# OSOceanAcoustics/echopype

Measured on AMD Instinct MI355X. Metric: range-samples/sec through compute_Sv->compute_MVBS, higher is better.
Workload: dtype f64; 1 GPU; cfg5: EK60 CW 4x2000000x4096 in ping_time tiles, compute_Sv -> compute_MVBS(20s x 1m), Sv+MVBS out; tiles=8 x 250000 pings over 1 rank(s), route=compute_Sv -> compute_MVBS('1m','20s') per tile, collective=none at 1 rank, tile_streams=2

## Files before the change

### echopype_amd/_lib.py

```python
import ctypes
import os

import torch

_HERE = os.path.dirname(os.path.abspath(__file__))
LIB_PATH = os.environ.get("ECHOPYPE_AMD_LIB") or os.path.join(_HERE, "lib", "libechopype_amd.so")

EPA_OK, EPA_EINVAL, EPA_EHIP, EPA_ENOMEM, EPA_EUNSUPPORTED = range(5)
F32, F64 = 0, 1
I8 = 2
CAL_SV, CAL_TS = 0, 1
SONAR_EK60, SONAR_EK80 = 0, 1
PM_SCALAR, PM_CHANNEL, PM_CHANNEL_PING, PM_PULSE_TABLE = range(4)
NCOEF = 8
CF_RA, CF_RB, CF_R0, CF_SHIFT, CF_ALPHA2, CF_A0, CF_G, CF_D = range(8)
NCCOEF = 8
CC_RA, CC_RB, CC_SHIFT, CC_ALPHA2, CC_A, CC_PSCALE = range(6)
FLAG_GUARD_POS, FLAG_MASK_RANGE = 1, 2
BIN_SKIPNA, BIN_CLOSED_RIGHT, BIN_RANGE_AS_STORED = 1, 2, 4
POOL_NANMEAN, POOL_NANMEDIAN = 0, 1
CMP_GT, CMP_LT, CMP_LE, CMP_GE, CMP_EQ = range(5)
CCP = ("sample_interval", "tau_nominal", "transmit_power", "sound_speed", "absorption", "gain", "freq_center", "psi",
       "sa_correction", "z_er", "z_et", "angle_offset_alongship", "angle_offset_athwartship", "beamwidth_alongship",
       "beamwidth_athwartship")
EK80_NFFT = 2048
APPLY_MASKS_WS_DOUBLES = 131072
SEAFLOOR_STATE_WORDS = 16
SHOAL_STATE_WORDS = 8
SHOAL_QUEUE_BOXES = 4096


class EpaError(RuntimeError):
    """A C-ABI call returned a non-zero status."""


def _load():
    if not os.path.exists(LIB_PATH):
        raise ImportError(
            f"{LIB_PATH} not found: build it with `python echopype_amd/build.py` "
            "(hipcc --offload-arch=gfx950).  echopype_amd has no CPU fallback."
        )
    return ctypes.CDLL(LIB_PATH)


lib = _load()

_vp, _i, _u, _d, _sz = ctypes.c_void_p, ctypes.c_int, ctypes.c_uint, ctypes.c_double, ctypes.c_size_t
_i64 = ctypes.c_int64

SIGNATURES = {
    "epa_version": [],
    "epa_source_digest": [],
    "epa_last_error": [],
    "epa_launch_trace": [_i],
    "epa_last_range_stats_filled": [],
    "epa_launch_seen": [],
    "epa_device_count": [ctypes.POINTER(_i)],
    "epa_set_device": [_i],
    "epa_device_name": [_i, ctypes.c_char_p, _sz],
    "epa_malloc": [ctypes.POINTER(_vp), _sz],
    "epa_free": [_vp],
    "epa_memset": [_vp, _i, _sz, _vp],
    "epa_memcpy_h2d": [_vp, _vp, _sz, _vp],
    "epa_memcpy_d2h": [_vp, _vp, _sz, _vp],
    "epa_stream_synchronize": [_vp],
    "epa_timer_create": [ctypes.POINTER(_vp)],
    "epa_timer_destroy": [_vp],
    "epa_timer_start": [_vp, _vp],
    "epa_timer_stop": [_vp, _vp],
    "epa_timer_elapsed_ms": [_vp, ctypes.POINTER(ctypes.c_float)],
    "epa_power_coef_ek": [_i, _i, _vp, _vp, _vp, _vp, _i, _vp, _i, _vp, _i, _vp, _i, _vp, _i, _vp, _i, _vp,
                          _vp, _i, _vp, _i, _i, _vp, _vp],
    "epa_pulse_table_lookup": [_vp, _vp, _vp, _i, _i, _i, _vp, _vp],
    "epa_sv_power": [_vp, _vp, _i, _i, _i, _i, _u, _vp, _vp, _i, _vp],
    "epa_sv_power_stats": [_vp, _vp, _i, _i, _i, _i, _u, _vp, _vp, _i, _vp, _vp, _vp],
    "epa_range_power": [_vp, _vp, _i, _i, _i, _u, _vp, _i, _vp],
    "epa_range_complex": [_vp, _i, _vp, _i, _i, _i, _i, _vp, _i, _vp],
    "epa_sv_complex_cw_stats": [_vp, _vp, _i, _vp, _i, _i, _i, _i, _i, _vp, _vp, _vp, _i, _vp, _vp, _vp],
    "epa_time_bin_offsets": [_vp, _i, _i64, _i64, _i, _u, _vp, _vp],
    "epa_sv_mvbs_fused": [_vp, _vp, _i, _i, _i, _i, _u, _vp, _vp, _i, _d, _i, _u, _d, _vp, _vp, _vp,
                          _vp, _vp, _vp, _vp, _i, _vp],
    "epa_sv_mvbs_fused_i16": [_vp, _vp, _vp, _i, _i, _i, _i, _vp, _i, _d, _i, _d, _vp, _vp, _vp, _vp, _vp, _i, _vp],
    "epa_sv_mvbs_fused_depth": [_vp, _vp, _vp, _vp, _i, _i, _i, _i, _vp, _i, _d, _i, _d, _vp, _vp, _vp, _vp, _vp, _vp, _i,
                                _vp],
    "epa_mvbs": [_vp, _vp, _vp, _i, _i, _i, _vp, _vp, _i, _d, _i, _u, _d, _vp, _vp, _vp, _i, _vp],
    "epa_selftest_lin_from_db": [_vp, _vp, _sz, _vp],
    "epa_selftest_log10": [_vp, _vp, _sz, _vp],
    "epa_selftest_log10_inline": [_vp, _vp, _sz, _vp],
    "epa_selftest_correlate": [_vp, _i, _vp, _vp, _i, _vp, _vp, _vp],
    "epa_mvbs_finalize": [_vp, _vp, _sz, _d, _vp, _i, _vp],
    "epa_edge_pack": [_vp, _vp, _vp, _vp, _i, _i, _i, _i, _i, _i, _vp, _vp],
    "epa_edge_prepare_max": [_vp, _i, _vp],
    "epa_edge_gather": [_vp, _i, _vp, _vp, _i, _i, _i, _vp, _vp, _vp, _i, _vp],
    "epa_edge_finalize_mvbs": [_vp, _i, _vp, _vp, _vp, _vp, _vp, _i, _i, _i, _d, _i, _vp],
    "epa_affine_rows": [_vp, _vp, _vp, _i, _i, _i, _vp, _i, _vp],
    "epa_depth_rows": [_vp, _vp, _vp, _vp, _vp, _i, _i, _i, _vp, _i, _vp, _vp, _vp],
    "epa_nanminmax": [_vp, _sz, _i, _vp, _vp, _vp],
    "epa_mvbs_index": [_vp, _vp, _i, _i, _i, _i, _i, _vp, _vp, _i, _vp],
    "epa_noise_estimate": [_vp, _vp, _vp, _vp, _i, _i, _i, _i, _i, _i, _d, _vp, _vp, _vp, _i, _vp],
    "epa_noise_finalize": [_vp, _vp, _i, _i, _d, _vp, _vp],
    "epa_noise_apply": [_vp, _vp, _vp, _vp, _vp, _i, _i, _i, _i, _i, _d, _vp, _vp, _vp, _i, _vp],
    "epa_noise_apply_rows": [_vp, _vp, _vp, _vp, _vp, _i, _i, _i, _i, _i, _d, _vp, _vp, _vp, _i, _vp],
    "epa_complex_coef_ek80": [_i, _i, _vp, _vp, _vp, _i, _vp, _i, _i, _i, _vp, _vp],
    "epa_sv_complex": [_vp, _vp, _i, _vp, _vp, _i, _vp, _i, _i, _i, _i, _i, _vp, _vp, _vp, _i, _vp],
    "epa_sv_complex_indexed": [_vp, _vp, _i, _vp, _vp, _vp, _i, _i, _vp, _i, _i, _i, _i, _i, _vp, _vp, _vp, _i, _vp],
    "epa_sv_complex_fft": [_vp, _vp, _i, _vp, _vp, _i, _vp, _i, _i, _i, _i, _i, _vp, _vp, _vp, _i, _i, _vp, _vp, _vp],
    "epa_sv_complex_fft_indexed": [_vp, _vp, _i, _vp, _vp, _vp, _i, _i, _vp, _i, _i, _i, _i, _i, _vp, _vp, _vp, _i, _i,
                                   _vp, _vp, _vp],
    "epa_range_bin_smooth": [_vp, _vp, _i, _i, _i, _i, _d, _d, _i, _vp, _i, _vp],
    "epa_impulse_mask": [_vp, _i, _i, _i, _i, _d, _vp, _i, _vp],
    "epa_pool_sv": [_vp, _i, _i, _i, _i, _i, _i, _i, _d, _vp, _vp, _vp, _vp, _i, _vp],
    "epa_attenuated_mask": [_vp, _vp, _i, _i, _i, _d, _d, _i, _d, _vp, _i, _vp],
    "epa_apply_mask": [_vp, _vp, _sz, _sz, _d, _vp, _sz, _vp, _i, _vp],
    "epa_apply_masks": [_vp, _vp, _vp, _i, _sz, _d, _vp, _sz, _vp, _vp, _vp, _i, _vp],
    "epa_mask_and": [_vp, _vp, _sz, _sz, _vp, _vp],
    "epa_range_step_mean": [_vp, _i, _i, _i, _i, _vp, _vp, _vp],
    "epa_first_not_le": [_vp, _sz, _d, _i, _vp, _vp],
    "epa_range_rows_check": [_vp, _i, _i, _i, _i, _vp, _vp, _vp],
    "epa_sv_noise_fused": [_vp, _vp, _vp, _i, _i, _i, _i, _u, _i, _i, _i, _d, _vp, _vp, _vp, _vp, _vp, _vp, _vp, _i, _vp],
    "epa_denoise_mvbs": [_vp, _vp, _vp, _vp, _vp, _i, _i, _i, _i, _d, _vp, _vp, _i, _d, _i, _u, _d, _vp, _vp, _vp,
                         _vp, _vp, _i, _vp],
    "epa_sv_denoise_mvbs": [_vp, _vp, _vp, _vp, _i, _i, _i, _i, _u, _i, _i, _d, _vp, _vp, _i, _d, _i, _u, _d, _vp, _vp, _vp,
                            _vp, _vp, _vp, _vp, _i, _vp],
    "epa_geodesic_steps": [_vp, _vp, _i, _vp, _vp],
    "epa_nasc": [_vp, _vp, _i, _i, _i, _vp, _i, _d, _i, _u, _vp, _vp, _vp, _vp, _i, _vp],
    "epa_splitbeam_power": [_vp, _vp, _i, _vp, _vp, _i, _i, _i, _vp, _vp, _i, _vp],
    "epa_splitbeam_complex": [_vp, _vp, _i, _vp, _vp, _vp, _vp, _vp, _vp, _i, _i, _i, _i, _i, _i, _vp, _vp, _i, _vp],
    "epa_splitbeam_complex_fft": [_vp, _vp, _i, _vp, _vp, _vp, _vp, _vp, _vp, _i, _i, _i, _i, _i, _i, _vp, _vp, _i, _i,
                                  _vp, _vp],
    "epa_pool_sv_value": [_vp, _vp, _vp, _i, _i, _i, _d, _i, _d, _d, _d, _i, _d, _vp, _vp, _vp, _i, _vp],
    "epa_seafloor_depth_uniform": [_vp, _i, _i64, _i64, _vp, _vp],
    "epa_seafloor_basic": [_vp, _i, _i64, _i64, _i64, _d, _d, _vp, _d, _vp, _vp],
    "epa_seafloor_angle_mask": [_vp, _vp, _i, _i64, _i64, _i64, _i64, _i, _i, _d, _d, _vp, _vp, _vp, _vp],
    "epa_seafloor_median": [_vp, _i, _i64, _i64, _i64, _i64, _vp, _vp, _vp, _vp],
    "epa_seafloor_components": [_vp, _i, _i64, _i64, _i64, _i64, _d, _vp, _vp, _vp, _vp],
    "epa_seafloor_bottom": [_vp, _vp, _i64, _i64, _i64, _vp, _d, _vp, _i, _vp],
    "epa_shoal_threshold_fill": [_vp, _i, _i64, _i64, _d, _i64, _i64, _vp, _vp],
    "epa_shoal_label": [_vp, _i64, _i64, _i, _vp, _vp, _vp, _i64, _vp, _vp],
    "epa_shoal_weill_filter": [_vp, _i64, _i64, _vp, _vp, _i64, _d, _d, _vp, _vp, _vp],
    "epa_shoal_echoview_link": [_vp, _i64, _i64, _vp, _vp, _vp, _i64, _vp, _i64, _vp, _i64, _d, _d, _d, _d, _d, _d, _vp,
                                _vp, _vp, _vp],
    "epa_transient_fielding": [_vp, _i, _i, _i, _i, _vp, _i, _i, _d, _d, _d, _vp, _vp, _vp, _vp],
    "epa_transient_matecho": [_vp, _i, _i, _i, _i, _vp, _vp, _vp, _vp, _i, _i, _d, _d, _i, _d, _vp, _vp, _vp, _vp],
    "epa_freq_diff_mask": [_vp, _i, _sz, _i, _i, _i, _d, _vp, _i, _vp],
    "epa_regrid_mask": [_vp, _vp, _i, _i, _i, _vp, _i, _vp, _i, _d, _i, _u, _i, _vp, _vp, _vp],
    "epa_echo_metrics": [_vp, _vp, _i, _i64, _i64, _vp, _vp, _vp, _vp, _vp, _vp, _i, _i, _vp],
}

for _name, _args in SIGNATURES.items():
    _fn = getattr(lib, _name)
    _fn.argtypes = _args
    _fn.restype = ctypes.c_char_p if _name in ("epa_last_error", "epa_launch_trace", "epa_launch_seen", "epa_source_digest") else _i


def _check_source_digest():
    if os.environ.get("ECHOPYPE_AMD_LIB"):
        return
    import importlib.util

    spec = importlib.util.spec_from_file_location("_epa_build", os.path.join(_HERE, "build.py"))
    if spec is None or not os.path.isdir(os.path.join(_HERE, "csrc")):
        return
    b = importlib.util.module_from_spec(spec)
    spec.loader.exec_module(b)
    want, got = b.source_digest(), lib.epa_source_digest().decode()
    if want != got:
        raise ImportError(f"{LIB_PATH} was built from other sources (digest {got}, the tree has {want}): "
                          "rebuild it with `python echopype_amd/build.py` (`--force` recompiles every translation unit)")


_check_source_digest()


class launch_trace:

    def __enter__(self):
        lib.epa_launch_trace(1)
        self.kernels = []
        return self

    def __exit__(self, *exc):
        self.kernels = [k for k in lib.epa_launch_trace(2).decode().split(";") if k]
        lib.epa_launch_trace(0)
        return False


def launched_kernels():
    return [k for k in lib.epa_launch_seen().decode().split(";") if k]


def last_error() -> str:
    msg = lib.epa_last_error()
    return msg.decode("utf-8", "replace") if msg else ""


def check(status: int, what: str = "") -> None:
    if status == EPA_OK:
        return
    msg = f"{what}: {last_error()}" if what else last_error()
    if status == EPA_EINVAL:
        raise ValueError(msg)
    if status == EPA_ENOMEM:
        raise MemoryError(msg)
    raise EpaError(f"[status {status}] {msg}")


def call(name: str, *args) -> None:
    check(getattr(lib, name)(*args), name)
```

### echopype_amd/csrc/block_reduce.hip

```cpp
#include <hip/amd_detail/amd_hip_unsafe_atomics.h>

#include <cstdlib>

#include "fast_math.h"
#include "sample_math.h"

namespace {

enum { SRC_RAW = 0, SRC_SV = 1, SRC_SV_DENOISE = 2, SRC_RAW_DENOISE = 3 };
enum { OP_MVBS = 0, OP_NOISE = 1 };
enum { BIN_PHYS = 0, BIN_INDEX = 1 };

struct ReduceArgs {
  double* range_max_out;
  double* range_stats_out;
  int range_stats_filled;
  const int16_t* raw_i16;
  const int32_t* n_valid;
  const double* dscale;
  const double* doffset;
  void* depth_out;
  const float* raw;
  const void* sv;
  const void* range;
// ... 152 lines not shown
        constexpr bool kDenoise = SRC == SRC_SV_DENOISE || SRC == SRC_RAW_DENOISE;
        if (kFromRaw) {
          epa::RawVec<VEC> in;
          in.load(a.raw + off);
          const epa::RowK<T> rk(a.coef[row]);
          col.update(rk.d, s0, nspread);
          if (OP == OP_NOISE || kDenoise) {
            const double k = rk.ra * rk.rb;
            col_tl.update(-rk.r0 / k, s0, (T)1);
            const T log10k = epa::fast_log10((T)k, mt.log_tab);
#pragma unroll
            for (int j = 0; j < VEC; ++j) logR[j] = col_tl.nL[j] + log10k;
          }
          T rg[VEC];
#pragma unroll
          for (int j = 0; j < VEC; ++j) {
            x[j] = rk.range(s0 + j);
            sv[j] = epa::cal_power_sample<T>(in.v[j], s0 + j, rk, nspread, col.nL[j], guard, x[j]);
            xok[j] = !(mask_range && !(in.v[j] == in.v[j]));
            rg[j] = xok[j] ? (T)x[j] : epa::M<T>::nan();
            if (a.range_max_out && xok[j]) xmax = fmax(xmax, (double)rg[j]);
          }
          if (sv_out && !kDenoise) epa::store_vec<T, VEC>(sv_out + off, sv);
          if (range_out) epa::store_vec<T, VEC>(range_out + off, rg);
        } else {
          epa::load_vec<T, VEC>(svp + off, sv);
          if (rgp) {
            T rg[VEC];
            epa::load_vec<T, VEC>(rgp + off, rg);
#pragma unroll
            for (int j = 0; j < VEC; ++j) {
              x[j] = (double)rg[j];
              xok[j] = true;
            }
          } else if (a.coef) {
            const epa::CoefRow cr = a.coef[row];
#pragma unroll
            for (int j = 0; j < VEC; ++j) {
              x[j] = epa::row_range(cr, s0 + j);
              if (range_as_stored) x[j] = (double)(T)x[j];
              xok[j] = true;
            }
          } else {
#pragma unroll
            for (int j = 0; j < VEC; ++j) {
              x[j] = 0.0;
              xok[j] = true;
            }
          }
        }
        if (kDenoise) {
          {
            const T nb = (T)a.noise[(size_t)c * a.n_pblocks + (p + a.noise_phase) / a.noise_ping_num];
            const T na2 = (T)a.alpha2[row];
            const T snr = (T)a.snr;
            T sn[VEC];
#pragma unroll
            for (int j = 0; j < VEC; ++j) {
              const T xr = xok[j] ? (T)x[j] : epa::M<T>::nan();
              const T lg = kFromRaw ? logR[j] : epa::fast_log10(xr >= (T)1 ? xr : (T)1, mt.log_tab);
              const T tl = (T)20 * (xr >= (T)1 ? lg : (T)0) + na2 * xr;
              sn[j] = nb + tl;
              const T lin = epa::lin_from_db(sv[j], mt.exp2_tab) - epa::lin_from_db(sn[j], mt.exp2_tab);
              T corr = lin > (T)0 ? (T)10 * epa::fast_log10(lin, mt.log_tab) : epa::M<T>::nan();
              const bool keep = corr - sn[j] > snr;
              sv[j] = keep ? corr : epa::M<T>::nan();
              vlin[j] = keep ? lin : epa::M<T>::nan();
              if (a.mm_keys) {
                mm[0] = fmin(mm[0], (double)sn[j]);
                mm[1] = fmax(mm[1], (double)sn[j]);
                mm[2] = fmin(mm[2], (double)sv[j]);
                mm[3] = fmax(mm[3], (double)sv[j]);
              }
            }
            if (sv_noise_out) epa::store_vec<T, VEC>(sv_noise_out + off, sn);
            if (sv_out) epa::store_vec<T, VEC>(sv_out + off, sv);
          }
        }
        T a2 = (T)0;
        if (OP == OP_NOISE) a2 = (T)a.alpha2[row];
#pragma unroll
        for (int j = 0; j < VEC; ++j) {
          T v;
          if (OP == OP_MVBS) {
            v = kDenoise ? vlin[j] : epa::lin_from_db(sv[j], mt.exp2_tab);
          } else {
            const T xr = (T)x[j];
            const T lg = kFromRaw ? logR[j] : epa::fast_log10(xr >= (T)1 ? xr : (T)1, mt.log_tab);
            const T tl = (T)20 * (xr >= (T)1 ? lg : (T)0) + a2 * xr;
            v = epa::lin_from_db(sv[j] - tl, mt.exp2_tab);
          }
          if (phys) {
            const bool same = xok[j] && (closed_right ? (x[j] > blo[j] && x[j] <= bhi[j])
                                                      : (x[j] >= blo[j] && x[j] < bhi[j]));
            if (!same) {
              const int rb = xok[j] ? epa::range_bin_index(x[j], a.range_bin, a.inv_range_bin,
                                                            n_rbins, closed_right)
                                    : -1;
              if (rb != acc_rb[j]) {
                if (acc_rb[j] >= 0 && acc_cnt[j] > 0u && !extra) {
                  atomic_add(asum + acc_rb[j], acc_sum[j]);
                  atomicAdd(acnt + acc_rb[j], acc_cnt[j]);
                }
                acc_rb[j] = rb;
                acc_sum[j] = (T)0;
                acc_cnt[j] = 0u;
              }
              if (rb >= 0) {
                blo[j] = (double)rb * a.range_bin;
                bhi[j] = (double)(rb + 1) * a.range_bin;
              } else {
                blo[j] = 1.0;
                bhi[j] = 0.0;
              }
            }
          }
          if (acc_rb[j] >= 0 && (!skipna || v == v)) {
            acc_sum[j] += v;
            acc_cnt[j] += 1u;
          }
        }
      }
      if (!extra) {
#pragma unroll
        for (int j = 0; j < VEC; ++j) {
          if (acc_rb[j] >= 0 && acc_cnt[j] > 0u) {
            atomic_add(asum + acc_rb[j], acc_sum[j]);
            atomicAdd(acnt + acc_rb[j], acc_cnt[j]);
          }
        }
      }
    }
  }
  }
  if (a.range_max_out) {
#pragma unroll
    for (int o = 32; o > 0; o >>= 1) xmax = fmax(xmax, __shfl_down(xmax, o, 64));
    if ((threadIdx.x & 63) == 0 && xmax > -__builtin_inf()) {
      const unsigned long long b = (unsigned long long)__double_as_longlong(xmax);
      atomicMax(reinterpret_cast<unsigned long long*>(a.range_max_out),
                (b >> 63) ? ~b : (b | 0x8000000000000000ull));
    }
  }
  if (a.mm_keys) {
#pragma unroll
    for (int o = 32; o > 0; o >>= 1) {
      mm[0] = fmin(mm[0], __shfl_down(mm[0], o, 64));
      mm[1] = fmax(mm[1], __shfl_down(mm[1], o, 64));
      mm[2] = fmin(mm[2], __shfl_down(mm[2], o, 64));
      mm[3] = fmax(mm[3], __shfl_down(mm[3], o, 64));
    }
    if ((threadIdx.x & 63) == 0) {
      auto key = [](double v) {
        const unsigned long long b = (unsigned long long)__double_as_longlong(v);
        return (b >> 63) ? ~b : (b | 0x8000000000000000ull);
      };
      if (mm[0] <= mm[1]) {
        atomicMin(a.mm_keys + 0, key(mm[0]));
        atomicMax(a.mm_keys + 1, key(mm[1]));
      }
      if (mm[2] <= mm[3]) {
        atomicMin(a.mm_keys + 2, key(mm[2]));
        atomicMax(a.mm_keys + 3, key(mm[3]));
      }
    }
  }
  if (extra) return;

  if (!use_lds) return;
  __syncthreads();
  if (a.nparts > 1) {
    for (int i = threadIdx.x; i < n_rbins; i += epa::kBlock) {
      const uint32_t n = lcnt[i];
      if (n > 0u) {
        atomic_add(gsum + i, lsum[i]);
        atomicAdd(gcnt + i, n);
      }
    }
    return;
  }
  if (OP == OP_MVBS) {
    T* out = reinterpret_cast<T*>(a.out) + cell0;
    for (int i = threadIdx.x; i < n_rbins; i += epa::kBlock) {
      const uint32_t n = lcnt[i];
      const T s = lsum[i];
      out[i] = n > 0u ? (T)10 * epa::M<T>::log10(s / (T)n) : (T)a.fill_value;
      if (gsum) gsum[i] = s;
      if (gcnt) gcnt[i] = n;
    }
  } else {
    if (a.edge_sum_out && (tb == 0 || tb == a.n_tbins - 1)) {
      const size_t e0 = ((size_t)(tb == 0 ? 0 : 1) * a.C + c) * n_rbins;
      for (int i = threadIdx.x; i < n_rbins; i += epa::kBlock) {
        a.edge_sum_out[e0 + i] = (double)lsum[i];
        a.edge_cnt_out[e0 + i] = lcnt[i];
      }
    }
    T best = (T)__builtin_inf();
    bool any = false;
    for (int i = threadIdx.x; i < n_rbins; i += epa::kBlock) {
      const uint32_t n = lcnt[i];
      if (n > 0u) {
        const T db = (T)10 * epa::M<T>::log10(lsum[i] / (T)n);
        if (db == db) {
          best = fmin(best, db);
          any = true;
        }
      }
    }
    __syncthreads();
    T m = block_nanmin<T>(best, any, lsum);
    if (threadIdx.x == 0) {
      double r = (double)m;
      if (a.noise_max == a.noise_max) r = (r < a.noise_max) ? r : a.noise_max;
      reinterpret_cast<double*>(a.out)[(size_t)c * a.n_tbins + tb] = r;
    }
  }
}

template <typename T>
__global__ __launch_bounds__(epa::kBlock) void mvbs_finalize_kernel(const T* __restrict__ sum,
                                                                    const uint32_t* __restrict__ cnt,
                                                                    size_t n, T fill,
                                                                    T* __restrict__ out) {
  for (size_t i = (size_t)blockIdx.x * blockDim.x + threadIdx.x; i < n;
       i += (size_t)gridDim.x * blockDim.x) {
    const uint32_t k = cnt[i];
    out[i] = k > 0u ? (T)10 * epa::M<T>::log10(sum[i] / (T)k) : fill;
  }
}

template <typename T>
__global__ __launch_bounds__(epa::kBlock) void noise_rowmin_kernel(const T* __restrict__ sum,
                                                                   const uint32_t* __restrict__ cnt,
                                                                   int n_rbins, double noise_max,
                                                                   double* __restrict__ out) {
  __shared__ T scratch[8];
  const size_t base = (size_t)blockIdx.x * n_rbins;
  T best = (T)__builtin_inf();
  bool any = false;
  for (int i = threadIdx.x; i < n_rbins; i += epa::kBlock) {
    const uint32_t n = cnt[base + i];
    if (n > 0u) {
      const T db = (T)10 * epa::M<T>::log10(sum[base + i] / (T)n);
      if (db == db) {
        best = fmin(best, db);
        any = true;
      }
    }
  }
  T m = block_nanmin<T>(best, any, scratch);
  if (threadIdx.x == 0) {
    double r = (double)m;
    if (noise_max == noise_max) r = (r < noise_max) ? r : noise_max;
    out[blockIdx.x] = r;
  }
}

template <typename T>
__global__ __launch_bounds__(epa::kBlock) void block_nanmin_kernel(const T* __restrict__ x, int C,
                                                                   int P, int S, int ping_num,
                                                                   int rsn, int Pb, int Sb,
                                                                   T* __restrict__ out) {
  const long long cells = (long long)C * Pb * Sb;
  const int lane = threadIdx.x & 63;
  const long long wave0 = ((long long)blockIdx.x * blockDim.x + threadIdx.x) >> 6;
  const long long nwaves = ((long long)gridDim.x * blockDim.x) >> 6;
  for (long long cell = wave0; cell < cells; cell += nwaves) {
    const int sb = (int)(cell % Sb);
    const int pbk = (int)((cell / Sb) % Pb);
    const int c = (int)(cell / ((long long)Sb * Pb));
    const int p0 = pbk * ping_num, p1 = min(P, p0 + ping_num);
    const int s0 = sb * rsn, s1 = min(S, s0 + rsn);
    const int w = s1 - s0;
    const int n = (p1 - p0) * w;
    T m = (T)__builtin_inf();
    int any = 0;
    for (int e = lane; e < n; e += 64) {
      const int p = p0 + e / w, s = s0 + e % w;
      const T v = x[((size_t)c * P + p) * S + s];
      if (v == v) {
        m = fmin(m, v);
        any = 1;
      }
    }
#pragma unroll
    for (int o = 32; o > 0; o >>= 1) {
      m = fmin(m, __shfl_down(m, o, 64));
      any |= __shfl_down(any, o, 64);
    }
    if (lane == 0) out[cell] = any ? m : epa::M<T>::nan();
  }
}

}

int epa_fused_fast_path(const void* raw, int raw_is_i16, const int32_t* n_valid, const double* coef,
                        int C, int P, int S, double nspread,
                        unsigned cal_flags, const int32_t* bin_start, int n_tbins, double range_bin,
                        int n_rbins, unsigned bin_flags, double fill_value, void* sv_out,
                        void* mvbs_out, void* sum_out, uint32_t* cnt_out, int dtype,
                        size_t lds_bytes, unsigned cnt_off, unsigned long long* rmax_key,
                        unsigned long long* rstat, const double* dscale, const double* doffset, void* depth_out,
                        hipStream_t st);

int epa_mvbs_rows_fast_path(const void* sv, const double* coef, int C, int P, int S, const int32_t* bin_start,
                            int n_tbins, double range_bin, int n_rbins, int as_stored, double fill_value,
                            void* mvbs_out, void* sum_out, uint32_t* cnt_out, int dtype, size_t lds_bytes,
                            unsigned cnt_off, hipStream_t st);
int epa_chain_fast_pass1(const float* raw, const double* coef, const double* alpha2, int C, int P, int S,
                         double nspread, int ping_num, int rsn, int ping_phase, double noise_max, void* sv_out,
                         double* noise_out, double* edge_sum_out, uint32_t* edge_cnt_out,
                         unsigned long long* rmax_key, unsigned long long* rstat, int dtype, hipStream_t st);
int epa_chain_fast_pass2(const float* raw, const double* coef, const double* alpha2, const double* noise, int C,
                         int P, int S, double nspread, int ping_num, int ping_phase, double snr,
                         const int32_t* bin_start, int n_tbins, double range_bin, int n_rbins, double fill_value,
                         void* noise_out, void* corr_out, void* mvbs_out, void* sum_out, uint32_t* cnt_out, int dtype,
                         size_t lds_acc_bytes, unsigned cnt_off, unsigned long long* mm_keys, hipStream_t st);

namespace {

struct Plan {
  int nparts, use_lds, vec;
  size_t lds_bytes;
  unsigned cnt_off, tab_off;
};

template <typename T>
Plan make_plan(int C, int P, int S, int n_tbins, int n_rbins, bool aligned16) {
  Plan pl;
  pl.vec = (S % 4 == 0 && aligned16) ? 4 : 1;
  if (const char* e = getenv("EPA_REDUCE_VEC")) {
    const int v = atoi(e);
    if ((v == 1) || (v == 2 && S % 2 == 0 && aligned16) || (v == 4 && S % 4 == 0 && aligned16)) pl.vec = v;
  }
  const size_t sum_bytes = ((size_t)n_rbins * sizeof(T) + 15) & ~(size_t)15;
  const size_t need = sum_bytes + (size_t)n_rbins * sizeof(uint32_t);
  pl.use_lds = need <= 128 * 1024;
  const size_t acc_bytes = pl.use_lds ? (need < 64 ? 64 : need) : 64;
  pl.cnt_off = (unsigned)sum_bytes;
  pl.tab_off = (unsigned)((acc_bytes + 15) & ~(size_t)15);
  pl.lds_bytes = pl.tab_off + epa::kMathTabBytes;
  const long long groups = (long long)C * n_tbins;
  pl.nparts = 1;
  if (groups < 1024) {
    const long long avg = n_tbins > 0 ? (P + n_tbins - 1) / n_tbins : P;
    long long want = (2048 + groups - 1) / groups;
    long long maxp = (avg + 7) / 8;
    if (maxp < 1) maxp = 1;
    pl.nparts = (int)(want < maxp ? want : maxp);
    if (pl.nparts < 1) pl.nparts = 1;
  }
  return pl;
}

template <typename T, int SRC, int OP>
int launch_reduce(ReduceArgs& a, const Plan& pl, hipStream_t st) {
  const long long tslots = (long long)a.n_tbins + ((SRC != SRC_SV && a.bin_start) ? 1 : 0);
  const dim3 grid((unsigned)(tslots * a.nparts), (unsigned)a.C);
  const dim3 block(epa::kBlock);
  a.use_lds = pl.use_lds;
  a.cnt_off = pl.cnt_off;
  a.tab_off = pl.tab_off;
#define EPA_RL(V)                                                                                 \
  do {                                                                                            \
    auto kern = block_reduce_kernel<T, SRC, OP, V>;                                               \
    if (pl.lds_bytes > 64 * 1024) {                                                               \
      EPA_CHECK_HIP(hipFuncSetAttribute(reinterpret_cast<const void*>(kern),                      \
                                        hipFuncAttributeMaxDynamicSharedMemorySize,               \
                                        (int)pl.lds_bytes));                                      \
    }                                                                                             \
    hipLaunchKernelGGL(kern, grid, block, pl.lds_bytes, st, a);                                   \
  } while (0)
  if (pl.vec == 4) EPA_RL(4); else if (pl.vec == 2) EPA_RL(2); else EPA_RL(1);
#undef EPA_RL
  return epa::check_launch("block_reduce_kernel");
}

inline bool al16(const void* p) { return p == nullptr || (reinterpret_cast<uintptr_t>(p) & 15u) == 0; }

template <typename T>
int zero_partials(void* sum_out, uint32_t* cnt_out, size_t cells, hipStream_t st) {
  EPA_CHECK_HIP(hipMemsetAsync(sum_out, 0, cells * sizeof(T), st));
  EPA_CHECK_HIP(hipMemsetAsync(cnt_out, 0, cells * sizeof(uint32_t), st));
  return EPA_OK;
}

template <typename T, int SRC>
int run_mvbs(ReduceArgs& a, hipStream_t st) {
  Plan pl = make_plan<T>(a.C, a.P, a.S, a.n_tbins, a.n_rbins,
                               al16(a.raw) && al16(a.sv) && al16(a.range) && al16(a.sv_out) &&
                                   al16(a.range_out));
  if (SRC == SRC_RAW && (a.range_max_out || a.raw_i16)) pl.nparts = 1;
  a.nparts = pl.nparts;
  const size_t cells = (size_t)a.C * a.n_tbins * a.n_rbins;
  const bool two_stage = pl.nparts > 1 || !pl.use_lds;
  if (SRC == SRC_RAW && !two_stage && pl.vec == 4 && !a.ping_perm && !a.range_out &&
      a.cal_flags == (EPA_FLAG_GUARD_POS | EPA_FLAG_MASK_RANGE) && a.bin_flags == EPA_BIN_SKIPNA &&
      (a.raw_i16 || !getenv("EPA_NO_FAST_PATH")) && (a.range_stats_filled = a.range_stats_out != nullptr, true))
    return epa_fused_fast_path(a.raw_i16 ? (const void*)a.raw_i16 : (const void*)a.raw, a.raw_i16 != nullptr,
                               a.n_valid, reinterpret_cast<const double*>(a.coef), a.C, a.P, a.S,
                               a.nspread, a.cal_flags, a.bin_start, a.n_tbins, a.range_bin,
                               a.n_rbins, a.bin_flags, a.fill_value, a.sv_out, a.out, a.sum_out,
                               a.cnt_out, sizeof(T) == 8 ? EPA_F64 : EPA_F32, pl.tab_off,
                               pl.cnt_off, reinterpret_cast<unsigned long long*>(a.range_max_out),
                               reinterpret_cast<unsigned long long*>(a.range_stats_out), a.dscale, a.doffset,
                               a.depth_out, st);
  if (a.dscale) {
    epa::set_error("epa_sv_mvbs_fused_depth: binning on depth is served by the default configuration only (sorted "
                   "pings, S %% 4 == 0, aligned arrays, range grid within LDS)");
    return EPA_EUNSUPPORTED;
  }
  if (SRC == SRC_RAW_DENOISE && !two_stage && pl.vec == 4 && !a.ping_perm && !a.range_out &&
      a.cal_flags == (EPA_FLAG_GUARD_POS | EPA_FLAG_MASK_RANGE) && a.bin_flags == EPA_BIN_SKIPNA &&
      !getenv("EPA_NO_FAST_PATH"))
    return epa_chain_fast_pass2(a.raw, reinterpret_cast<const double*>(a.coef), a.alpha2, a.noise, a.C, a.P, a.S,
                                a.nspread, a.noise_ping_num, a.noise_phase, a.snr, a.bin_start, a.n_tbins, a.range_bin,
                                a.n_rbins, a.fill_value, a.sv_noise_out, a.sv_out, a.out, a.sum_out, a.cnt_out,
                                sizeof(T) == 8 ? EPA_F64 : EPA_F32, pl.tab_off, pl.cnt_off, a.mm_keys, st);
  if (SRC == SRC_SV && !a.range && a.coef && !two_stage && pl.vec == 4 && !a.ping_perm &&
      (a.bin_flags & ~EPA_BIN_RANGE_AS_STORED) == EPA_BIN_SKIPNA && !getenv("EPA_NO_FAST_PATH"))
    return epa_mvbs_rows_fast_path(a.sv, reinterpret_cast<const double*>(a.coef), a.C, a.P, a.S, a.bin_start, a.n_tbins,
                                   a.range_bin, a.n_rbins, (a.bin_flags & EPA_BIN_RANGE_AS_STORED) ? 1 : 0,
                                   a.fill_value, a.out, a.sum_out, a.cnt_out, sizeof(T) == 8 ? EPA_F64 : EPA_F32,
                                   pl.tab_off, pl.cnt_off, st);
  if (a.raw_i16) {
    epa::set_error("epa_sv_mvbs_fused_i16: int16 ingest is served by the default configuration only "
                   "(guard + masked range, skipna, left-closed bins, sorted pings, S %% 4 == 0, no "
                   "echo_range output, range grid within LDS)");
    return EPA_EUNSUPPORTED;
  }
  if (two_stage) {
    EPA_CHECK_ARG(a.sum_out && a.cnt_out,
                  "binned reduction: this shape (C*n_tbins=%lld, n_rbins=%d) needs the sum_out/"
                  "cnt_out workspaces", (long long)a.C * a.n_tbins, a.n_rbins);
    int rc = zero_partials<T>(a.sum_out, a.cnt_out, cells, st);
    if (rc) return rc;
  }
  int rc = launch_reduce<T, SRC, OP_MVBS>(a, pl, st);
  if (rc) return rc;
  if (two_stage) {
    const int grid = (int)((cells + epa::kBlock - 1) / epa::kBlock < 4096
                               ? (cells + epa::kBlock - 1) / epa::kBlock : 4096);
    hipLaunchKernelGGL(mvbs_finalize_kernel<T>, dim3(grid), dim3(epa::kBlock), 0, st,
                       (const T*)a.sum_out, (const uint32_t*)a.cnt_out, cells, (T)a.fill_value,
                       (T*)a.out);
    return epa::check_launch("mvbs_finalize_kernel");
  }
  return EPA_OK;
}

int check_bins(const char* fn, const int32_t* bin_start, int n_tbins, double range_bin, int n_rbins) {
  EPA_CHECK_ARG(bin_start != nullptr, "%s: bin_start is NULL", fn);
  EPA_CHECK_ARG(n_tbins > 0 && n_rbins > 0, "%s: n_tbins=%d n_rbins=%d must be positive", fn,
                n_tbins, n_rbins);
  EPA_CHECK_ARG(range_bin > 0, "%s: range_bin must be positive", fn);
  return EPA_OK;
}

}

namespace {
__global__ void decode_minmax_kernel(double* p) {
  const int i = threadIdx.x;
  const unsigned long long k = reinterpret_cast<unsigned long long*>(p)[i];
  const bool none = (i & 1) ? k == 0ull : k == ~0ull;
  const unsigned long long b = (k >> 63) ? (k & 0x7fffffffffffffffull) : ~k;
  p[i] = none ? __builtin_nan("") : __longlong_as_double(b);
}
__global__ void init_minmax_kernel(unsigned long long* p) { p[threadIdx.x] = (threadIdx.x & 1) ? 0ull : ~0ull; }

__global__ void init_range_out_kernel(double* rmax, double* st) {
  if (rmax) *reinterpret_cast<unsigned long long*>(rmax) = 0ull;
  if (st) {
    unsigned long long* u = reinterpret_cast<unsigned long long*>(st);
    u[0] = ~0ull;
    u[1] = 0ull;
    u[2] = 0ull;
  }
}
__global__ void decode_range_out_kernel(double* rmax, double* st, int mode, int as_f32) {
  const unsigned long long km = *reinterpret_cast<unsigned long long*>(rmax);
  const unsigned long long bm = (km >> 63) ? (km & 0x7fffffffffffffffull) : ~km;
  const double mx = km == 0ull ? __builtin_nan("") : __longlong_as_double(bm);
  *rmax = mx;
  if (mode == 1) {
    const unsigned long long k = reinterpret_cast<unsigned long long*>(st)[0];
    const unsigned long long n = reinterpret_cast<unsigned long long*>(st)[1];
    const unsigned long long b = (k >> 63) ? (k & 0x7fffffffffffffffull) : ~k;
    double lo = k == ~0ull ? __builtin_nan("") : __longlong_as_double(b), hi = mx;
    if (as_f32) {
      lo = (double)(float)lo;
      hi = (double)(float)hi;
    }
    st[0] = lo;
    st[1] = hi;
    st[2] = (double)n;
  } else if (mode == 2) {
    st[0] = st[1] = __builtin_nan("");
    st[2] = -1.0;
  }
}

int init_range_outputs(double* rmax, double* st, hipStream_t stream) {
  if (!rmax && !st) return EPA_OK;
  hipLaunchKernelGGL(init_range_out_kernel, dim3(1), dim3(1), 0, stream, rmax, st);
  return epa::check_launch("init_range_out_kernel");
}
int decode_range_outputs(double* rmax, double* st, bool filled, int as_f32, hipStream_t stream) {
  hipLaunchKernelGGL(decode_range_out_kernel, dim3(1), dim3(1), 0, stream, rmax, st, st ? (filled ? 1 : 2) : 0, as_f32);
  return epa::check_launch("decode_range_out_kernel");
}
}

static int fused_entry(const float* raw, const int16_t* raw_i16, const int32_t* n_valid,
                       const double* coef, int C, int P, int S, int cal_type, unsigned cal_flags,
                       const int32_t* bin_start, const int32_t* ping_perm, int n_tbins,
                       double range_bin, int n_rbins, unsigned bin_flags, double fill_value,
                       void* sv_out, void* range_out, void* mvbs_out, void* sum_out,
                       uint32_t* cnt_out, double* range_max_out, double* range_stats_out, int dtype,
                       epa_stream_t stream, const double* dscale = nullptr, const double* doffset = nullptr,
                       void* depth_out = nullptr);

extern "C" int epa_sv_mvbs_fused(const float* raw, const double* coef, int C, int P, int S,
                                 int cal_type, unsigned cal_flags, const int32_t* bin_start,
                                 const int32_t* ping_perm, int n_tbins, double range_bin,
                                 int n_rbins, unsigned bin_flags, double fill_value, void* sv_out,
                                 void* range_out, void* mvbs_out, void* sum_out, uint32_t* cnt_out,
                                 double* range_max_out, double* range_stats_out, int dtype,
                                 epa_stream_t stream) {
  EPA_CHECK_ARG(raw != nullptr, "epa_sv_mvbs_fused: NULL array argument");
  EPA_CHECK_ARG(!range_stats_out || range_max_out, "epa_sv_mvbs_fused: range_stats_out needs range_max_out");
  return fused_entry(raw, nullptr, nullptr, coef, C, P, S, cal_type, cal_flags, bin_start, ping_perm,
                     n_tbins, range_bin, n_rbins, bin_flags, fill_value, sv_out, range_out, mvbs_out,
                     sum_out, cnt_out, range_max_out, range_stats_out, dtype, stream);
}

extern "C" int epa_sv_mvbs_fused_i16(const int16_t* raw, const int32_t* n_valid, const double* coef,
                                     int C, int P, int S, int cal_type, const int32_t* bin_start,
                                     int n_tbins, double range_bin, int n_rbins, double fill_value,
                                     void* sv_out, void* mvbs_out, void* sum_out, uint32_t* cnt_out,
                                     double* range_max_out, int dtype, epa_stream_t stream) {
  EPA_CHECK_ARG(raw && n_valid, "epa_sv_mvbs_fused_i16: NULL array argument");
  return fused_entry(nullptr, raw, n_valid, coef, C, P, S, cal_type,
                     EPA_FLAG_GUARD_POS | EPA_FLAG_MASK_RANGE, bin_start, nullptr, n_tbins, range_bin,
                     n_rbins, EPA_BIN_SKIPNA, fill_value, sv_out, nullptr, mvbs_out, sum_out, cnt_out,
                     range_max_out, nullptr, dtype, stream);
}

extern "C" int epa_sv_mvbs_fused_depth(const float* raw, const double* coef, const double* depth_scale,
                                       const double* depth_offset, int C, int P, int S, int cal_type,
                                       const int32_t* bin_start, int n_tbins, double range_bin, int n_rbins,
                                       double fill_value, void* sv_out, void* depth_out, void* mvbs_out, void* sum_out,
                                       uint32_t* cnt_out, double* depth_stats_out, int dtype, epa_stream_t stream) {
  EPA_CHECK_ARG(raw && depth_scale && depth_offset && depth_stats_out, "epa_sv_mvbs_fused_depth: NULL array argument");
  EPA_CHECK_ARG(!depth_out || sv_out, "epa_sv_mvbs_fused_depth: depth_out needs sv_out");
  return fused_entry(raw, nullptr, nullptr, coef, C, P, S, cal_type, EPA_FLAG_GUARD_POS | EPA_FLAG_MASK_RANGE, bin_start,
                     nullptr, n_tbins, range_bin, n_rbins, EPA_BIN_SKIPNA, fill_value, sv_out, nullptr, mvbs_out, sum_out,
                     cnt_out, depth_stats_out + 32, depth_stats_out, dtype, stream, depth_scale, depth_offset, depth_out);
}

static int fused_entry(const float* raw, const int16_t* raw_i16, const int32_t* n_valid,
                       const double* coef, int C, int P, int S, int cal_type, unsigned cal_flags,
                       const int32_t* bin_start, const int32_t* ping_perm, int n_tbins,
                       double range_bin, int n_rbins, unsigned bin_flags, double fill_value,
                       void* sv_out, void* range_out, void* mvbs_out, void* sum_out,
                       uint32_t* cnt_out, double* range_max_out, double* range_stats_out, int dtype,
                       epa_stream_t stream, const double* dscale, const double* doffset, void* depth_out) {
  EPA_CHECK_ARG(coef && mvbs_out, "epa_sv_mvbs_fused: NULL array argument");
  EPA_CHECK_ARG(C > 0 && P > 0 && S > 0, "epa_sv_mvbs_fused: C=%d P=%d S=%d", C, P, S);
  EPA_CHECK_ARG(cal_type == EPA_CAL_SV || cal_type == EPA_CAL_TS, "epa_sv_mvbs_fused: bad cal_type");
  if (int rc = check_bins("epa_sv_mvbs_fused", bin_start, n_tbins, range_bin, n_rbins)) return rc;
  ReduceArgs a{};
  a.raw = raw; a.raw_i16 = raw_i16; a.n_valid = n_valid;
  a.dscale = dscale; a.doffset = doffset; a.depth_out = depth_out;
  a.coef = reinterpret_cast<const epa::CoefRow*>(coef);
  a.C = C; a.P = P; a.S = S;
  a.nspread = cal_type == EPA_CAL_SV ? 20.0 : 40.0;
  a.cal_flags = cal_flags;
  a.bin_start = bin_start; a.ping_perm = ping_perm; a.n_tbins = n_tbins; a.ping_num = 0;
  a.bin_mode = BIN_PHYS; a.range_bin = range_bin; a.inv_range_bin = 1.0 / range_bin;
  a.n_rbins = n_rbins; a.range_sample_num = 1; a.bin_flags = bin_flags;
  a.fill_value = fill_value; a.noise_max = __builtin_nan("");
  a.sv_out = sv_out; a.range_out = range_out; a.out = mvbs_out; a.sum_out = sum_out; a.cnt_out = cnt_out;
  a.range_max_out = range_max_out;
  a.range_stats_out = range_stats_out;
  EPA_CHECK_ARG(dtype == EPA_F64 || dtype == EPA_F32, "epa_sv_mvbs_fused: bad dtype %d", dtype);
  if (int rc0 = init_range_outputs(range_max_out, range_stats_out, (hipStream_t)stream)) return rc0;
  const int rc = dtype == EPA_F64 ? run_mvbs<double, SRC_RAW>(a, (hipStream_t)stream)
                                  : run_mvbs<float, SRC_RAW>(a, (hipStream_t)stream);
  epa::note_range_stats_filled(rc == EPA_OK && range_stats_out && a.range_stats_filled ? 1 : 0);
  if (rc == EPA_OK && range_max_out) {
    return decode_range_outputs(range_max_out, range_stats_out, a.range_stats_filled != 0, dtype == EPA_F32 ? 1 : 0,
                                (hipStream_t)stream);
  }
  return rc;
}

extern "C" int epa_mvbs(const void* sv, const void* range, const double* coef, int C, int P, int S,
                        const int32_t* bin_start, const int32_t* ping_perm, int n_tbins,
                        double range_bin, int n_rbins, unsigned bin_flags, double fill_value,
                        void* mvbs_out, void* sum_out, uint32_t* cnt_out, int dtype,
                        epa_stream_t stream) {
  EPA_CHECK_ARG(sv && mvbs_out, "epa_mvbs: NULL array argument");
  EPA_CHECK_ARG(range || coef, "epa_mvbs: either range or coef must be given");
  EPA_CHECK_ARG(C > 0 && P > 0 && S > 0, "epa_mvbs: C=%d P=%d S=%d", C, P, S);
  if (int rc = check_bins("epa_mvbs", bin_start, n_tbins, range_bin, n_rbins)) return rc;
  ReduceArgs a{};
  a.sv = sv; a.range = range; a.coef = reinterpret_cast<const epa::CoefRow*>(coef);
  a.C = C; a.P = P; a.S = S;
  a.bin_start = bin_start; a.ping_perm = ping_perm; a.n_tbins = n_tbins;
  a.bin_mode = BIN_PHYS; a.range_bin = range_bin; a.inv_range_bin = 1.0 / range_bin;
  a.n_rbins = n_rbins; a.range_sample_num = 1; a.bin_flags = bin_flags;
  a.fill_value = fill_value; a.noise_max = __builtin_nan("");
  a.out = mvbs_out; a.sum_out = sum_out; a.cnt_out = cnt_out;
  if (dtype == EPA_F64) return run_mvbs<double, SRC_SV>(a, (hipStream_t)stream);
  if (dtype == EPA_F32) return run_mvbs<float, SRC_SV>(a, (hipStream_t)stream);
  epa::set_error("epa_mvbs: bad dtype %d", dtype);
  return EPA_EINVAL;
}

extern "C" int epa_mvbs_finalize(const void* sum, const uint32_t* cnt, size_t n, double fill_value,
                                 void* out, int dtype, epa_stream_t stream) {
  EPA_CHECK_ARG(sum && cnt && out, "epa_mvbs_finalize: NULL array argument");
  if (n == 0) return EPA_OK;
  const size_t blocks = (n + epa::kBlock - 1) / epa::kBlock;
  const int grid = (int)(blocks < 4096 ? blocks : 4096);
  if (dtype == EPA_F64)
    hipLaunchKernelGGL(mvbs_finalize_kernel<double>, dim3(grid), dim3(epa::kBlock), 0,
                       (hipStream_t)stream, (const double*)sum, cnt, n, fill_value, (double*)out);
  else if (dtype == EPA_F32)
    hipLaunchKernelGGL(mvbs_finalize_kernel<float>, dim3(grid), dim3(epa::kBlock), 0,
                       (hipStream_t)stream, (const float*)sum, cnt, n, (float)fill_value, (float*)out);
  else {
    epa::set_error("epa_mvbs_finalize: bad dtype %d", dtype);
    return EPA_EINVAL;
  }
  return epa::check_launch("mvbs_finalize_kernel");
}

namespace {
template <typename T>
int run_index(const void* sv, const void* range, int C, int P, int S, int ping_num, int rsn,
              void* mvbs_out, void* range_min_out, hipStream_t st) {
  const int Pb = (P + ping_num - 1) / ping_num, Sb = (S + rsn - 1) / rsn;
  ReduceArgs a{};
  a.sv = sv; a.C = C; a.P = P; a.S = S;
  a.bin_start = nullptr; a.n_tbins = Pb; a.ping_num = ping_num;
  a.bin_mode = BIN_INDEX; a.range_bin = 1.0; a.inv_range_bin = 1.0; a.n_rbins = Sb;
  a.range_sample_num = rsn; a.bin_flags = EPA_BIN_SKIPNA;
  a.fill_value = __builtin_nan(""); a.noise_max = __builtin_nan("");
  a.out = mvbs_out;
  Plan pl = make_plan<T>(C, P, S, Pb, Sb, al16(sv));
  pl.nparts = 1;
  a.nparts = 1;
  EPA_CHECK_ARG(pl.use_lds, "epa_mvbs_index: %d range blocks exceed the LDS budget", Sb);
  int rc = launch_reduce<T, SRC_SV, OP_MVBS>(a, pl, st);
  if (rc) return rc;
  if (range && range_min_out) {
    const long long cells = (long long)C * Pb * Sb;
    const long long blocks = (cells + 3) / 4;
    const int grid = (int)(blocks < 8192 ? blocks : 8192);
    hipLaunchKernelGGL(block_nanmin_kernel<T>, dim3(grid), dim3(epa::kBlock), 0, st,
                       (const T*)range, C, P, S, ping_num, rsn, Pb, Sb, (T*)range_min_out);
    return epa::check_launch("block_nanmin_kernel");
  }
  return EPA_OK;
}

template <typename T>
int run_noise(const void* sv, const void* range, const double* coef, const double* alpha2, int C,
              int P, int S, int ping_num, int rsn, int ping_phase, double noise_max, double* noise_out,
              double* edge_sum_out, uint32_t* edge_cnt_out, hipStream_t st) {
  const int Pb = (P + ping_phase + ping_num - 1) / ping_num, Sb = (S + rsn - 1) / rsn;
  ReduceArgs a{};
  a.sv = sv; a.range = range; a.coef = reinterpret_cast<const epa::CoefRow*>(coef);
  a.alpha2 = alpha2;
  a.C = C; a.P = P; a.S = S;
  a.bin_start = nullptr; a.n_tbins = Pb; a.ping_num = ping_num; a.ping_phase = ping_phase;
  a.bin_mode = BIN_INDEX; a.range_bin = 1.0; a.inv_range_bin = 1.0; a.n_rbins = Sb;
  a.range_sample_num = rsn; a.bin_flags = EPA_BIN_SKIPNA;
  a.fill_value = __builtin_nan(""); a.noise_max = noise_max;
  a.out = noise_out;
  a.edge_sum_out = edge_sum_out; a.edge_cnt_out = edge_cnt_out;
  Plan pl = make_plan<T>(C, P, S, Pb, Sb, al16(sv) && al16(range));
  pl.nparts = 1;
  a.nparts = 1;
  EPA_CHECK_ARG(pl.use_lds, "epa_noise_estimate: %d range blocks exceed the LDS budget", Sb);
  return launch_reduce<T, SRC_SV, OP_NOISE>(a, pl, st);
}
}

extern "C" int epa_mvbs_index(const void* sv, const void* range, int C, int P, int S, int ping_num,
                              int range_sample_num, void* mvbs_out, void* range_min_out, int dtype,
                              epa_stream_t stream) {
  EPA_CHECK_ARG(sv && mvbs_out, "epa_mvbs_index: NULL array argument");
  EPA_CHECK_ARG(C > 0 && P > 0 && S > 0 && ping_num > 0 && range_sample_num > 0,
                "epa_mvbs_index: sizes must be positive");
  if (dtype == EPA_F64)
    return run_index<double>(sv, range, C, P, S, ping_num, range_sample_num, mvbs_out, range_min_out,
                             (hipStream_t)stream);
  if (dtype == EPA_F32)
    return run_index<float>(sv, range, C, P, S, ping_num, range_sample_num, mvbs_out, range_min_out,
                            (hipStream_t)stream);
  epa::set_error("epa_mvbs_index: bad dtype %d", dtype);
  return EPA_EINVAL;
}

extern "C" int epa_noise_estimate(const void* sv, const void* range, const double* coef,
                                  const double* alpha2, int C, int P, int S, int ping_num,
                                  int range_sample_num, int ping_phase, double noise_max, double* noise_out,
                                  double* edge_sum_out, uint32_t* edge_cnt_out, int dtype,
                                  epa_stream_t stream) {
  EPA_CHECK_ARG(sv && alpha2 && noise_out, "epa_noise_estimate: NULL array argument");
  EPA_CHECK_ARG(range || coef, "epa_noise_estimate: either range or coef must be given");
  EPA_CHECK_ARG(C > 0 && P > 0 && S > 0 && ping_num > 0 && range_sample_num > 0,
                "epa_noise_estimate: sizes must be positive");
  EPA_CHECK_ARG(ping_phase >= 0 && ping_phase < ping_num, "epa_noise_estimate: ping_phase %d not in [0, %d)",
                ping_phase, ping_num);
  EPA_CHECK_ARG((edge_sum_out == nullptr) == (edge_cnt_out == nullptr),
                "epa_noise_estimate: edge_sum_out and edge_cnt_out come together");
  if (dtype == EPA_F64)
    return run_noise<double>(sv, range, coef, alpha2, C, P, S, ping_num, range_sample_num, ping_phase,
                             noise_max, noise_out, edge_sum_out, edge_cnt_out, (hipStream_t)stream);
  if (dtype == EPA_F32)
    return run_noise<float>(sv, range, coef, alpha2, C, P, S, ping_num, range_sample_num, ping_phase, noise_max,
                            noise_out, edge_sum_out, edge_cnt_out, (hipStream_t)stream);
  epa::set_error("epa_noise_estimate: bad dtype %d", dtype);
  return EPA_EINVAL;
}

namespace {
__global__ __launch_bounds__(epa::kBlock) void noise_rows_f64_kernel(const double* __restrict__ sum,
                                                                     const double* __restrict__ cnt, int n_rbins,
                                                                     double noise_max, double* __restrict__ out) {
  __shared__ double scratch[8];
  const size_t base = (size_t)blockIdx.x * n_rbins;
  double best = __builtin_inf();
  bool any = false;
  for (int i = threadIdx.x; i < n_rbins; i += epa::kBlock) {
    const double n = cnt[base + i];
    if (n > 0.0) {
      const double db = 10.0 * ::log10(sum[base + i] / n);
      if (db == db) {
        best = fmin(best, db);
        any = true;
      }
    }
  }
  const double m = block_nanmin<double>(best, any, scratch);
  if (threadIdx.x == 0) {
    double r = m;
    if (noise_max == noise_max) r = (r < noise_max) ? r : noise_max;
    out[blockIdx.x] = r;
  }
}
}

extern "C" int epa_noise_finalize(const double* sum, const double* cnt, int rows, int n_rblocks, double noise_max,
                                  double* noise_out, epa_stream_t stream) {
  EPA_CHECK_ARG(sum && cnt && noise_out, "epa_noise_finalize: NULL array argument");
  EPA_CHECK_ARG(rows > 0 && n_rblocks > 0, "epa_noise_finalize: sizes must be positive");
  hipLaunchKernelGGL(noise_rows_f64_kernel, dim3(rows), dim3(epa::kBlock), 0, (hipStream_t)stream, sum, cnt,
                     n_rblocks, noise_max, noise_out);
  return epa::check_launch("noise_rows_f64_kernel");
}

namespace {
template <typename T>
int run_sv_noise(const float* raw, const double* coef, const double* alpha2, int C, int P, int S,
                 double nspread, unsigned cal_flags, int ping_num, int rsn, int ping_phase, double noise_max,
                 void* sv_out, void* range_out, double* noise_out, double* edge_sum_out, uint32_t* edge_cnt_out,
                 double* range_max_out, double* range_stats_out, int* stats_filled, hipStream_t st) {
  const int Pb = (P + ping_phase + ping_num - 1) / ping_num, Sb = (S + rsn - 1) / rsn;
  ReduceArgs a{};
  a.raw = raw; a.coef = reinterpret_cast<const epa::CoefRow*>(coef); a.alpha2 = alpha2;
  a.C = C; a.P = P; a.S = S; a.nspread = nspread; a.cal_flags = cal_flags;
  a.bin_start = nullptr; a.n_tbins = Pb; a.ping_num = ping_num; a.ping_phase = ping_phase;
  a.bin_mode = BIN_INDEX; a.range_bin = 1.0; a.inv_range_bin = 1.0; a.n_rbins = Sb;
  a.range_sample_num = rsn; a.bin_flags = EPA_BIN_SKIPNA;
  a.fill_value = __builtin_nan(""); a.noise_max = noise_max;
  a.sv_out = sv_out; a.range_out = range_out; a.out = noise_out; a.range_max_out = range_max_out;
  a.edge_sum_out = edge_sum_out; a.edge_cnt_out = edge_cnt_out;
  Plan pl = make_plan<T>(C, P, S, Pb, Sb, al16(raw) && al16(sv_out) && al16(range_out));
  pl.nparts = 1;
  a.nparts = 1;
  EPA_CHECK_ARG(pl.use_lds, "epa_sv_noise_fused: %d range blocks exceed the LDS budget", Sb);
  if (pl.vec == 4 && !range_out && cal_flags == (EPA_FLAG_GUARD_POS | EPA_FLAG_MASK_RANGE) &&
      !getenv("EPA_NO_FAST_PATH")) {
    *stats_filled = range_stats_out != nullptr;
    return epa_chain_fast_pass1(raw, coef, alpha2, C, P, S, nspread, ping_num, rsn, ping_phase, noise_max, sv_out,
                                noise_out, edge_sum_out, edge_cnt_out,
                                reinterpret_cast<unsigned long long*>(range_max_out),
                                reinterpret_cast<unsigned long long*>(range_stats_out),
                                sizeof(T) == 8 ? EPA_F64 : EPA_F32, st);
  }
  return launch_reduce<T, SRC_RAW, OP_NOISE>(a, pl, st);
}
}

extern "C" int epa_sv_noise_fused(const float* raw, const double* coef, const double* alpha2, int C, int P,
                                  int S, int cal_type, unsigned cal_flags, int ping_num,
                                  int range_sample_num, int ping_phase, double noise_max, void* sv_out,
                                  void* range_out, double* noise_out, double* edge_sum_out, uint32_t* edge_cnt_out,
                                  double* range_max_out, double* range_stats_out, int dtype, epa_stream_t stream) {
  EPA_CHECK_ARG(raw && coef && alpha2 && noise_out, "epa_sv_noise_fused: NULL array argument");
  EPA_CHECK_ARG(C > 0 && P > 0 && S > 0 && ping_num > 0 && range_sample_num > 0,
                "epa_sv_noise_fused: sizes must be positive");
  EPA_CHECK_ARG(ping_phase >= 0 && ping_phase < ping_num, "epa_sv_noise_fused: ping_phase %d not in [0, %d)",
                ping_phase, ping_num);
  EPA_CHECK_ARG((edge_sum_out == nullptr) == (edge_cnt_out == nullptr),
                "epa_sv_noise_fused: edge_sum_out and edge_cnt_out come together");
  EPA_CHECK_ARG(cal_type == EPA_CAL_SV || cal_type == EPA_CAL_TS, "epa_sv_noise_fused: bad cal_type");
  const double nspread = cal_type == EPA_CAL_SV ? 20.0 : 40.0;
  EPA_CHECK_ARG(dtype == EPA_F64 || dtype == EPA_F32, "epa_sv_noise_fused: bad dtype %d", dtype);
  EPA_CHECK_ARG(!range_stats_out || range_max_out, "epa_sv_noise_fused: range_stats_out needs range_max_out");
  if (int rc0 = init_range_outputs(range_max_out, range_stats_out, (hipStream_t)stream)) return rc0;
  int filled = 0;
  const int rc = dtype == EPA_F64
      ? run_sv_noise<double>(raw, coef, alpha2, C, P, S, nspread, cal_flags, ping_num, range_sample_num, ping_phase,
                             noise_max, sv_out, range_out, noise_out, edge_sum_out, edge_cnt_out, range_max_out,
                             range_stats_out, &filled, (hipStream_t)stream)
      : run_sv_noise<float>(raw, coef, alpha2, C, P, S, nspread, cal_flags, ping_num, range_sample_num, ping_phase,
                            noise_max, sv_out, range_out, noise_out, edge_sum_out, edge_cnt_out, range_max_out,
                            range_stats_out, &filled, (hipStream_t)stream);
  epa::note_range_stats_filled(rc == EPA_OK && range_stats_out && filled ? 1 : 0);
  if (rc == EPA_OK && range_max_out) {
    return decode_range_outputs(range_max_out, range_stats_out, filled != 0, 0, (hipStream_t)stream);
  }
  return rc;
}

extern "C" int epa_denoise_mvbs(const void* sv, const void* range, const double* coef, const double* alpha2,
                                const double* noise, int C, int P, int S, int ping_num,
                                double snr_threshold, const int32_t* bin_start, const int32_t* ping_perm,
                                int n_tbins, double range_bin, int n_rbins, unsigned bin_flags,
                                double fill_value, void* sv_noise_out, void* sv_corrected_out,
                                void* mvbs_out, void* sum_out, uint32_t* cnt_out, int dtype,
                                epa_stream_t stream) {
  EPA_CHECK_ARG(sv && alpha2 && noise && mvbs_out, "epa_denoise_mvbs: NULL array argument");
  EPA_CHECK_ARG(range || coef, "epa_denoise_mvbs: either range or coef must be given");
  EPA_CHECK_ARG(C > 0 && P > 0 && S > 0 && ping_num > 0, "epa_denoise_mvbs: sizes must be positive");
  if (int rc = check_bins("epa_denoise_mvbs", bin_start, n_tbins, range_bin, n_rbins)) return rc;
  ReduceArgs a{};
  a.sv = sv; a.range = range; a.coef = reinterpret_cast<const epa::CoefRow*>(coef);
  a.alpha2 = alpha2; a.noise = noise; a.noise_ping_num = ping_num; a.n_pblocks = (P + ping_num - 1) / ping_num;
  a.snr = snr_threshold;
  a.C = C; a.P = P; a.S = S;
  a.bin_start = bin_start; a.ping_perm = ping_perm; a.n_tbins = n_tbins;
  a.bin_mode = BIN_PHYS; a.range_bin = range_bin; a.inv_range_bin = 1.0 / range_bin;
  a.n_rbins = n_rbins; a.range_sample_num = 1; a.bin_flags = bin_flags;
  a.fill_value = fill_value; a.noise_max = __builtin_nan("");
  a.sv_out = sv_corrected_out; a.sv_noise_out = sv_noise_out;
  a.out = mvbs_out; a.sum_out = sum_out; a.cnt_out = cnt_out;
  if (dtype == EPA_F64) return run_mvbs<double, SRC_SV_DENOISE>(a, (hipStream_t)stream);
  if (dtype == EPA_F32) return run_mvbs<float, SRC_SV_DENOISE>(a, (hipStream_t)stream);
  epa::set_error("epa_denoise_mvbs: bad dtype %d", dtype);
  return EPA_EINVAL;
}

extern "C" int epa_sv_denoise_mvbs(const float* raw, const double* coef, const double* alpha2,
                                   const double* noise, int C, int P, int S, int cal_type, unsigned cal_flags,
                                   int ping_num, int ping_phase, double snr_threshold, const int32_t* bin_start,
                                   const int32_t* ping_perm, int n_tbins, double range_bin, int n_rbins,
                                   unsigned bin_flags, double fill_value, void* sv_noise_out,
                                   void* sv_corrected_out, void* range_out, void* mvbs_out, void* sum_out,
                                   uint32_t* cnt_out, double* minmax_out, int dtype, epa_stream_t stream) {
  EPA_CHECK_ARG(raw && coef && alpha2 && noise && mvbs_out, "epa_sv_denoise_mvbs: NULL array argument");
  EPA_CHECK_ARG(C > 0 && P > 0 && S > 0 && ping_num > 0, "epa_sv_denoise_mvbs: sizes must be positive");
  EPA_CHECK_ARG(ping_phase >= 0 && ping_phase < ping_num, "epa_sv_denoise_mvbs: ping_phase %d not in [0, %d)",
                ping_phase, ping_num);
  EPA_CHECK_ARG(cal_type == EPA_CAL_SV || cal_type == EPA_CAL_TS, "epa_sv_denoise_mvbs: bad cal_type");
  if (int rc = check_bins("epa_sv_denoise_mvbs", bin_start, n_tbins, range_bin, n_rbins)) return rc;
  ReduceArgs a{};
  a.raw = raw; a.coef = reinterpret_cast<const epa::CoefRow*>(coef);
  a.alpha2 = alpha2; a.noise = noise; a.noise_ping_num = ping_num; a.noise_phase = ping_phase;
  a.n_pblocks = (P + ping_phase + ping_num - 1) / ping_num;
  a.snr = snr_threshold;
  a.C = C; a.P = P; a.S = S;
  a.nspread = cal_type == EPA_CAL_SV ? 20.0 : 40.0;
  a.cal_flags = cal_flags;
  a.bin_start = bin_start; a.ping_perm = ping_perm; a.n_tbins = n_tbins;
  a.bin_mode = BIN_PHYS; a.range_bin = range_bin; a.inv_range_bin = 1.0 / range_bin;
  a.n_rbins = n_rbins; a.range_sample_num = 1; a.bin_flags = bin_flags;
  a.fill_value = fill_value; a.noise_max = __builtin_nan("");
  a.sv_out = sv_corrected_out; a.sv_noise_out = sv_noise_out; a.range_out = range_out;
  a.out = mvbs_out; a.sum_out = sum_out; a.cnt_out = cnt_out;
  a.mm_keys = reinterpret_cast<unsigned long long*>(minmax_out);
  EPA_CHECK_ARG(dtype == EPA_F64 || dtype == EPA_F32, "epa_sv_denoise_mvbs: bad dtype %d", dtype);
  if (minmax_out) {
    hipLaunchKernelGGL(init_minmax_kernel, dim3(1), dim3(4), 0, (hipStream_t)stream, a.mm_keys);
    if (int rc = epa::check_launch("init_minmax_kernel")) return rc;
  }
// ... 9 lines not shown
```

### echopype_amd/csrc/fast_math.h

```cpp
#pragma once
#include "epa_internal.h"

namespace epa {

constexpr int kExpTabN = 256;
constexpr int kLogTabN = 128;
constexpr size_t kExpTabBytes = kExpTabN * sizeof(double);
constexpr size_t kLogTabBytes = kLogTabN * 2 * sizeof(double);
constexpr size_t kMathTabBytes = kExpTabBytes + kLogTabBytes;

struct MathTabs {
  const double* exp2_tab;
  const double2* log_tab;
};

__device__ __forceinline__ MathTabs build_math_tabs(unsigned char* base) {
  double* e = reinterpret_cast<double*>(base);
  double2* l = reinterpret_cast<double2*>(base + kExpTabBytes);
  const int t = threadIdx.x;
  if (t < kExpTabN) e[t] = ::exp2((double)t * (1.0 / kExpTabN));
  if (t < kLogTabN) {
    const double c = 1.0 + ((double)t + 0.5) * (1.0 / kLogTabN);
    const double inv = 1.0 / c;
    double lg = -::log10(inv);
    if (c > 1.4142135623730951) lg -= 0.30102999566398120;
    l[t] = make_double2(inv, lg);
  }
  return MathTabs{e, l};
}

__device__ __forceinline__ double lin_from_db(double u, const double* __restrict__ tab) {
  constexpr double K256_HI = 85.04135922911648;
  constexpr double K256_LO = -4.272771985668806e-15;
  constexpr double Z = 0.0027076061740622863;
  const double t = u * K256_HI;
  const double m = __builtin_rint(t);
  double r = fma(u, K256_HI, -m);
  r = fma(u, K256_LO, r);
  const double z = r * Z;
  double p = fma(z, 1.0 / 24.0, 1.0 / 6.0);
  p = fma(p, z, 0.5);
  p = fma(p, z, 1.0);
  p = fma(p, z, 1.0);
  const double mc = fmin(fmax(m, -300000.0), 300000.0);
  const int mi = (int)mc;
  const double v = ldexp(p * tab[mi & 255], mi >> 8);
  return (fabs(t) < __builtin_inf()) ? v : (t < 0.0 ? 0.0 : t);
}
__device__ __forceinline__ float lin_from_db(float u, const double*) { return ::exp10f(u * 0.1f); }

__device__ __forceinline__ double lin_from_db_lean(double u, const double* __restrict__ tab) {
  constexpr double K256_HI = 85.04135922911648, K256_LO = -4.272771985668806e-15, Z = 0.0027076061740622863;
  const double t = u * K256_HI;
  const double m = __builtin_rint(t);
  double r = fma(u, K256_HI, -m);
  r = fma(u, K256_LO, r);
  const double z = r * Z;
  double p = fma(z, 1.0 / 24.0, 1.0 / 6.0);
  p = fma(p, z, 0.5);
  p = fma(p, z, 1.0);
  p = fma(p, z, 1.0);
  const int mi = __double2int_rz(m);
  double v = ldexp(p * tab[mi & 255], mi >> 8);
  if (__builtin_expect(__builtin_isinf(t), 0)) v = t < 0.0 ? 0.0 : t;
  return v;
}
__device__ __forceinline__ float lin_from_db_lean(float u, const double*) { return ::exp10f(u * 0.1f); }

__device__ __noinline__ double log10_special(double x) { return ::log10(x); }

__device__ __forceinline__ double fast_log10(double x, const double2* __restrict__ tab) {
  constexpr double LOG10_2 = 0.30102999566398120;
  constexpr double C1 = 0.43429448190325182765, C2 = -0.21714724095162591383,
                   C3 = 0.14476482730108394255, C4 = -0.10857362047581295691,
                   C5 = 0.086858896380650365530, C6 = -0.072382413650541971275;
  const unsigned long long bits = __double_as_longlong(x);
  const unsigned ex = (unsigned)(bits >> 52) & 0x7ffu;
  const bool special = (long long)bits <= 0 || ex == 0u || ex == 0x7ffu;
  if (__builtin_expect(special, 0)) return log10_special(x);
  const int j = (int)((bits >> 45) & 127ull);
  const double m = __longlong_as_double((bits & 0x000fffffffffffffull) | 0x3ff0000000000000ull);
  const double2 t = tab[j];
  const double r = fma(m, t.x, -1.0);
  double p = fma(r, C6, C5);
  p = fma(p, r, C4);
  p = fma(p, r, C3);
  p = fma(p, r, C2);
  p = fma(p, r, C1);
  const double ef = (double)((int)ex - 1023 + (j >= 53 ? 1 : 0));
  const double res = fma(ef, LOG10_2, t.y) + r * p;
  return x == 1.0 ? 0.0 : res;
}
__device__ __forceinline__ float fast_log10(float x, const double2*) { return ::log10f(x); }

template <bool POSITIVE, bool EXACT_AT_1 = true>
__device__ __forceinline__ double fast_log10_inl(double x, const double2* __restrict__ tab) {
  constexpr double LOG10_2 = 0.30102999566398120;
  constexpr double C1 = 0.43429448190325182765, C2 = -0.21714724095162591383,
                   C3 = 0.14476482730108394255, C4 = -0.10857362047581295691,
                   C5 = 0.086858896380650365530, C6 = -0.072382413650541971275;
  const bool sub = ((unsigned)__double2hiint(x) & 0x7ff00000u) == 0u;
  const double xs = sub ? x * 0x1p54 : x;
  const unsigned long long bits = __double_as_longlong(xs);
  const unsigned ex = (unsigned)(bits >> 52) & 0x7ffu;
  const int j = (int)((bits >> 45) & 127ull);
  const double m = __longlong_as_double((bits & 0x000fffffffffffffull) | 0x3ff0000000000000ull);
  const double2 t = tab[j];
  const double r = fma(m, t.x, -1.0);
  double p = fma(r, C6, C5);
  p = fma(p, r, C4);
  p = fma(p, r, C3);
  p = fma(p, r, C2);
  p = fma(p, r, C1);
  const double ef = (double)((int)ex - (sub ? 1023 + 54 : 1023) + (j >= 53 ? 1 : 0));
  double res = fma(ef, LOG10_2, t.y) + r * p;
  if (EXACT_AT_1) res = x == 1.0 ? 0.0 : res;
  res = ex == 0x7ffu ? x : res;
  if (!POSITIVE) {
    res = x == 0.0 ? -__builtin_inf() : res;
    res = x < 0.0 ? __builtin_nan("") : res;
  }
  return res;
}
template <bool POSITIVE, bool EXACT_AT_1 = true>
__device__ __forceinline__ float fast_log10_inl(float x, const double2*) { return ::log10f(x); }

__device__ __forceinline__ double fast_log10_lean(double x, const double2* __restrict__ tab) {
  constexpr double LOG10_2 = 0.30102999566398120;
  constexpr double C1 = 0.43429448190325182765, C2 = -0.21714724095162591383,
                   C3 = 0.14476482730108394255, C4 = -0.10857362047581295691,
                   C5 = 0.086858896380650365530, C6 = -0.072382413650541971275;
  const unsigned long long bits = __double_as_longlong(x);
  const unsigned ex = (unsigned)(bits >> 52) & 0x7ffu;
  const int j = (int)((bits >> 45) & 127ull);
  const double m = __longlong_as_double((bits & 0x000fffffffffffffull) | 0x3ff0000000000000ull);
  const double2 t = tab[j];
  const double r = fma(m, t.x, -1.0);
  double p = fma(r, C6, C5);
  p = fma(p, r, C4);
  p = fma(p, r, C3);
  p = fma(p, r, C2);
  p = fma(p, r, C1);
  const double ef = (double)((int)ex - 1023 + (j >= 53 ? 1 : 0));
  double res = fma(ef, LOG10_2, t.y) + r * p;
  if (__builtin_expect(ex == 0u || ex == 0x7ffu, 0)) res = fast_log10_inl<true, false>(x, tab);
  return res;
}
__device__ __forceinline__ float fast_log10_lean(float x, const double2*) { return ::log10f(x); }

struct LogCoef {
  double c1, c2, c3, c4, c5, c6, log10_2;
};
__device__ __forceinline__ double opaque_scalar(double x) {
  int lo = __double2loint(x), hi = __double2hiint(x);
  asm volatile("" : "+s"(lo), "+s"(hi));
  return __hiloint2double(hi, lo);
}
__device__ __forceinline__ LogCoef make_log_coef() {
  return LogCoef{opaque_scalar(0.43429448190325182765),  opaque_scalar(-0.21714724095162591383),
                 opaque_scalar(0.14476482730108394255),  opaque_scalar(-0.10857362047581295691),
                 opaque_scalar(0.086858896380650365530), opaque_scalar(-0.072382413650541971275),
                 opaque_scalar(0.30102999566398120)};
}
__device__ __forceinline__ double fast_log10_lean(double x, const double2* __restrict__ tab, const LogCoef& K) {
  const unsigned long long bits = __double_as_longlong(x);
  const unsigned ex = (unsigned)(bits >> 52) & 0x7ffu;
  const int j = (int)((bits >> 45) & 127ull);
  const double m = __longlong_as_double((bits & 0x000fffffffffffffull) | 0x3ff0000000000000ull);
  const double2 t = tab[j];
  const double r = fma(m, t.x, -1.0);
  double p = fma(r, K.c6, K.c5);
  p = fma(p, r, K.c4);
  p = fma(p, r, K.c3);
  p = fma(p, r, K.c2);
  p = fma(p, r, K.c1);
  const double ef = (double)((int)ex - 1023 + (j >= 53 ? 1 : 0));
  double res = fma(ef, K.log10_2, t.y) + r * p;
  if (__builtin_expect(ex == 0u || ex == 0x7ffu, 0)) res = fast_log10_inl<true, false>(x, tab);
  return res;
}
__device__ __forceinline__ float fast_log10_lean(float x, const double2*, const LogCoef&) { return ::log10f(x); }

}
```

### echopype_amd/csrc/fused_sv_mvbs.hip

```cpp
#include <hip/amd_detail/amd_hip_unsafe_atomics.h>

#include <cstdlib>
#include <type_traits>

#include "fast_math.h"
#include "sample_math.h"

namespace epa_fused {

constexpr int VEC = 4;
constexpr int kChunk = epa::kBlock * VEC;

struct Args {
  int P, S, n_tbins, n_rbins;
  double range_bin, inv_range_bin;
  double nspread, fill_value;
  unsigned guard, mask_range, skipna, closed_right;
  unsigned cnt_off, tab_off;
  unsigned long long* rmax_key;
  unsigned long long* rstat;
  int xcd_map;
  int flagged_only;
  const double* dscale;
  const double* doffset;
  void* depth_out;
};

__device__ __forceinline__ unsigned long long ordered_key(double v) {
  const unsigned long long b = __double_as_longlong(v);
  return (b >> 63) ? ~b : (b | 0x8000000000000000ull);
}

template <typename T>
__device__ __noinline__ T log10_slow(T x) {
  return epa::M<T>::log10(x);
}

template <typename T>
__device__ __forceinline__ void lds_add(T* p, T v) {
  unsafeAtomicAdd(p, v);
}

template <typename T>
struct Column {
  double sra;
  double blo, bhi;
  T nL;
  T acc_sum;
  int acc_rb;
  uint32_t acc_cnt;
  __device__ __forceinline__ void init() {
    sra = 0.0; blo = 1.0; bhi = 0.0; nL = epa::M<T>::nan(); acc_sum = (T)0; acc_rb = -1; acc_cnt = 0u;
  }
  __device__ __forceinline__ void flush(T* lsum, uint32_t* lcnt, uint32_t n_clean) {
    const uint32_t n = acc_cnt + n_clean;
    if (acc_rb >= 0 && n > 0u) {
      lds_add(lsum + acc_rb, acc_sum);
      atomicAdd(lcnt + acc_rb, n);
    }
  }
  __device__ __forceinline__ void rebin(double x, bool valid, double bin, double inv_bin, int n_rbins, T* lsum,
                                        uint32_t* lcnt, uint32_t n_clean) {
    const int rb = valid ? epa::range_bin_index(x, bin, inv_bin, n_rbins, false) : -1;
    if (rb != acc_rb) {
      flush(lsum, lcnt, n_clean);
      acc_rb = rb;
      acc_sum = (T)0;
      acc_cnt = 0u - n_clean;
    }
    blo = rb >= 0 ? (double)rb * bin : 1.0;
    bhi = rb >= 0 ? (double)(rb + 1) * bin : 0.0;
  }
};

__device__ __forceinline__ double lin_bins(double u, const double* __restrict__ tab) {
  constexpr double K256 = 85.04135922911648, Z = 0.0027076061740622863;
  constexpr double C1 = Z, C2 = Z * Z / 2.0, C3 = Z * Z * Z / 6.0;
  const double t = u * K256;
  const double m = __builtin_rint(t);
  const double r = fma(u, K256, -m);
  double p = fma(r, C3, C2);
  p = fma(p, r, C1);
  p = fma(p, r, 1.0);
  const int mi = __double2int_rz(m);
  return ldexp(p * tab[mi & 255], mi >> 8);
}
__device__ __forceinline__ float lin_bins(float u, const double*) { return ::exp10f(u * 0.1f); }

__device__ __forceinline__ double vmax_num(double a, double b) {
  double r;
  asm("v_max_f64 %0, %1, %2" : "=v"(r) : "v"(a), "v"(b));
  return r;
}
__device__ __forceinline__ float vmax_num(float a, float b) {
  float r;
  asm("v_max_f32 %0, %1, %2" : "=v"(r) : "v"(a), "v"(b));
  return r;
}
__device__ __forceinline__ double vmin_num(double a, double b) {
  double r;
  asm("v_min_f64 %0, %1, %2" : "=v"(r) : "v"(a), "v"(b));
  return r;
}

template <typename T, bool STATS>
__device__ __forceinline__ T process_sample(Column<T>& c, float raw, const epa::CoefRow& r, double r0v, T g, T a2,
                                            T A0v, T nL, T nspread, double bin, double inv_bin, int n_rbins,
                                            const double* tab, T* lsum, uint32_t* lcnt, double& xmax, double& xmin,
                                            unsigned& nnan, uint32_t n_clean) {
  const T NaN = epa::M<T>::nan();
  const double x = fma(c.sra, r.rb, r0v);
  if (STATS) {
    const double xq = fma((double)raw, 0.0, x);
    xmax = vmax_num(xmax, xq);
    xmin = vmin_num(xmin, xq);
    nnan += (unsigned)__builtin_popcountll(__ballot(raw != raw));
  }
  const double rtd = x - r.shift;
  const T rt = (T)rtd;
  const bool pos = rtd > 0.0;
  T s1 = fma(g, (T)raw, nL);
  if (pos & !(nL > -(T)__builtin_inf()))
    s1 = fma(g, (T)raw, nspread * (log10_slow<T>(rt) - log10_slow<T>((T)(r.ra * r.rb))));
  s1 = pos ? s1 : NaN;
  const T sv = s1 + fma(a2, rt, A0v);
  const T v = epa::lin_from_db_lean(sv, tab);
  const bool same = (x >= c.blo) & (x < c.bhi);
  if (!same) c.rebin(x, raw == raw, bin, inv_bin, n_rbins, lsum, lcnt, n_clean);
  c.acc_sum += vmax_num(v, (T)0);
  c.acc_cnt += v == v ? 1u : 0u;
  return sv;
}

template <typename T, bool STATS, bool WRITE_SV, int DEPTH>
__device__ __forceinline__ void process_pair(Column<T>& c0, Column<T>& c1, float2 in, bool clean, const epa::CoefRow& r,
                                             double r0v, T g, T a2, T A0v, T nL0, T nL1, T nspread, double bin,
                                             double inv_bin, int n_rbins, const double* tab, T* lsum, uint32_t* lcnt,
                                             T* __restrict__ sv_dst, double& xmax, double& xmin, unsigned& nnan,
                                             uint32_t n_clean, double& xfirst, double& xlast, T dsc, T dof,
                                             T* __restrict__ depth_dst, double sra0, double sra1) {
  const double e0 = fma(sra0, r.rb, r0v), e1 = fma(sra1, r.rb, r0v);
  const double rtd0 = e0 - r.shift, rtd1 = e1 - r.shift;
  T d0 = (T)0, d1 = (T)0;
  if (DEPTH) {
    d0 = epa::depth_of(dsc, dof, (T)e0);
    d1 = epa::depth_of(dsc, dof, (T)e1);
  }
  const double x0 = DEPTH ? (double)d0 : e0, x1 = DEPTH ? (double)d1 : e1;
  const T rt0 = (T)rtd0, rt1 = (T)rtd1;
  T s10 = fma(g, (T)in.x, nL0), s11 = fma(g, (T)in.y, nL1);
  if (!clean) {
    const T NaN = epa::M<T>::nan();
    const bool pos0 = rtd0 > 0.0, pos1 = rtd1 > 0.0;
    if (pos0 & !(nL0 > -(T)__builtin_inf()))
      s10 = fma(g, (T)in.x, nspread * (log10_slow<T>(rt0) - log10_slow<T>((T)(r.ra * r.rb))));
    if (pos1 & !(nL1 > -(T)__builtin_inf()))
      s11 = fma(g, (T)in.y, nspread * (log10_slow<T>(rt1) - log10_slow<T>((T)(r.ra * r.rb))));
    s10 = pos0 ? s10 : NaN;
    s11 = pos1 ? s11 : NaN;
    if (STATS) {
      const double xq0 = fma((double)in.x, 0.0, x0), xq1 = fma((double)in.y, 0.0, x1);
      xmax = vmax_num(vmax_num(xmax, xq0), xq1);
      xmin = vmin_num(vmin_num(xmin, xq0), xq1);
      nnan += (unsigned)__builtin_popcountll(__ballot(xq0 != xq0)) + (unsigned)__builtin_popcountll(__ballot(xq1 != xq1));
    }
    if (DEPTH == 2) {
      d0 = fma((T)in.x, (T)0, d0);
      d1 = fma((T)in.y, (T)0, d1);
    }
  }
  if (DEPTH == 2) epa::store_nt2(depth_dst, d0, d1);
  const T sv0 = s10 + fma(a2, rt0, A0v), sv1 = s11 + fma(a2, rt1, A0v);
  if (WRITE_SV) {
#ifndef EPA_PLAIN_STORES
    epa::store_nt2(sv_dst, sv0, sv1);
#else
    const T o[2] = {sv0, sv1};
    epa::store_vec<T, 2>(sv_dst, o);
#endif
  }
  T v0 = lin_bins(sv0, tab), v1 = lin_bins(sv1, tab);
  if (!clean) {
    if (__builtin_expect(__builtin_isinf(sv0), 0)) v0 = sv0 < (T)0 ? (T)0 : sv0;
    if (__builtin_expect(__builtin_isinf(sv1), 0)) v1 = sv1 < (T)0 ? (T)0 : sv1;
  }
  if (!((x0 >= c0.blo) & (x0 < c0.bhi))) c0.rebin(x0, in.x == in.x, bin, inv_bin, n_rbins, lsum, lcnt, n_clean);
  if (!((x1 >= c1.blo) & (x1 < c1.bhi))) c1.rebin(x1, in.y == in.y, bin, inv_bin, n_rbins, lsum, lcnt, n_clean);
  if (clean) {
    c0.acc_sum += v0;
    c1.acc_sum += v1;
  } else {
    c0.acc_sum += vmax_num(v0, (T)0);
    c1.acc_sum += vmax_num(v1, (T)0);
    c0.acc_cnt += v0 == v0 ? 1u : 0u;
    c1.acc_cnt += v1 == v1 ? 1u : 0u;
  }
  xfirst = x0;
  xlast = x1;
}

__device__ __forceinline__ bool not_finite(float x) { return __builtin_amdgcn_classf(x, 0x207); }

template <typename RawT>
struct PingLoad;
template <>
struct PingLoad<float> {
  float2 a, b;
  __device__ __forceinline__ PingLoad() : a(make_float2(0.f, 0.f)), b(make_float2(0.f, 0.f)) {}
  __device__ __forceinline__ void issue(const float* __restrict__ row, int sA, int sB, bool hasB, int, int) {
    a = *reinterpret_cast<const float2*>(row + sA);
    if (hasB) b = *reinterpret_cast<const float2*>(row + sB);
  }
  __device__ __forceinline__ void resolve(float2& A, float2& B, int, int, int, bool) const {
    A = a;
    B = b;
  }
};
template <>
struct PingLoad<int16_t> {
  unsigned a, b;
  __device__ __forceinline__ PingLoad() : a(0u), b(0u) {}
  __device__ __forceinline__ void issue(const int16_t* __restrict__ row, int sA, int sB, bool hasB, int, int) {
    a = *reinterpret_cast<const unsigned*>(row + sA);
    if (hasB) b = *reinterpret_cast<const unsigned*>(row + sB);
  }
  static __device__ __forceinline__ float2 unpack(unsigned w, int s, int n_valid) {
    constexpr float kIndex2Power = 0.011758984205624266f;
    const float nanv = __builtin_nanf("");
    const float x = (float)(short)(w & 0xffffu), y = (float)(short)(w >> 16);
    return make_float2(s < n_valid ? x * kIndex2Power : nanv, s + 1 < n_valid ? y * kIndex2Power : nanv);
  }
  static __device__ __forceinline__ float2 unpack_all(unsigned w) {
    constexpr float kIndex2Power = 0.011758984205624266f;
    return make_float2((float)(short)(w & 0xffffu) * kIndex2Power, (float)(short)(w >> 16) * kIndex2Power);
  }
  __device__ __forceinline__ void resolve(float2& A, float2& B, int sA, int sB, int nv, bool full) const {
    if (full) {
      A = unpack_all(a);
      B = unpack_all(b);
    } else {
      A = unpack(a, sA, nv);
      B = unpack(b, sB, nv);
    }
  }
};

#ifndef EPA_FUSED_MIN_WAVES
#define EPA_FUSED_MIN_WAVES 1
#endif
#ifndef EPA_FUSED_LEAN
#define EPA_FUSED_LEAN 1
#endif
__device__ __forceinline__ double uniform(double v) {
  return __hiloint2double(__builtin_amdgcn_readfirstlane(__double2hiint(v)), __builtin_amdgcn_readfirstlane(__double2loint(v)));
}

__device__ __forceinline__ bool finite_bits(double v) { return (__double2hiint(v) & 0x7ff00000) != 0x7ff00000; }

template <typename T, typename RawT, bool WRITE_SV, bool RMAX, int DEPTH>
__global__ __launch_bounds__(epa::kBlock, EPA_FUSED_MIN_WAVES > 4 ? EPA_FUSED_MIN_WAVES : 4) void fused_sv_mvbs_kernel(
    const RawT* __restrict__ raw, const int32_t* __restrict__ n_valid,
    const epa::CoefRow* __restrict__ coef,
    const int32_t* __restrict__ bin_start, T* __restrict__ sv_out, T* __restrict__ mvbs_out,
    T* __restrict__ sum_out, uint32_t* __restrict__ cnt_out, const double* __restrict__ dscale,
    const double* __restrict__ doffset, Args a) {
  extern __shared__ __attribute__((aligned(16))) unsigned char smem[];
  T* lsum = reinterpret_cast<T*>(smem);
  uint32_t* lcnt = reinterpret_cast<uint32_t*>(smem + a.cnt_off);
  const epa::MathTabs mt = epa::build_math_tabs(smem + a.tab_off);
  const double* tab = mt.exp2_tab;
  constexpr bool NL_LDS = RMAX || sizeof(T) == 8;
  __shared__ T col_nL[NL_LDS ? kChunk : 1];
  constexpr bool SRA_LDS = (RMAX || std::is_same<RawT, int16_t>::value) && sizeof(T) == 8;
  __shared__ double col_sra[SRA_LDS ? kChunk : 1];
  __shared__ unsigned long long wg_keys[2];
  __shared__ unsigned wg_nnan;
  if (RMAX && threadIdx.x == 0) {
    wg_keys[0] = 0ull;
    wg_keys[1] = ~0ull;
    wg_nnan = 0u;
  }

  const int c = blockIdx.y, tb = a.xcd_map ? epa::xcd_contiguous(blockIdx.x, a.n_tbins) : (int)blockIdx.x;
  const int S = a.S, n_rbins = a.n_rbins;
  const bool extra = tb == a.n_tbins;
  if (extra && !WRITE_SV) return;
  const int nseg = extra ? 2 : 1;
  for (int i = threadIdx.x; i < n_rbins; i += epa::kBlock) {
    lsum[i] = (T)0;
    lcnt[i] = 0u;
  }
  __syncthreads();

  const T nspread = (T)a.nspread;
  const double bin = a.range_bin, inv_bin = a.inv_range_bin;
  const epa::CoefRow* __restrict__ rowp0 = coef + (size_t)c * a.P;
  const RawT* __restrict__ raw_c = raw + (size_t)c * a.P * S;
  const int32_t* __restrict__ nv_c = n_valid ? n_valid + (size_t)c * a.P : nullptr;
  T* __restrict__ sv_c = WRITE_SV ? sv_out + (size_t)c * a.P * S : nullptr;
  T* __restrict__ dp_c = DEPTH == 2 ? reinterpret_cast<T*>(a.depth_out) + (size_t)c * a.P * S : nullptr;
  const double* __restrict__ dsc_c = DEPTH ? dscale + (size_t)c * a.P : nullptr;
  const double* __restrict__ dof_c = DEPTH ? doffset + (size_t)c * a.P : nullptr;
  const int wave = __builtin_amdgcn_readfirstlane((int)(threadIdx.x >> 6)), lane = threadIdx.x & 63;
  double xmax = -__builtin_inf(), xmin = __builtin_inf();
  unsigned nnan = 0u;

  for (int seg = 0; seg < nseg; ++seg) {
  const int pb = extra ? (seg == 0 ? 0 : bin_start[a.n_tbins]) : bin_start[tb];
  const int pe = extra ? (seg == 0 ? bin_start[0] : a.P) : bin_start[tb + 1];
  for (int chunk0 = 0; chunk0 < S; chunk0 += kChunk) {
    const int sA = chunk0 + wave * 256 + 2 * lane;
    const int sB = sA + 128;
    if (sA >= S) continue;
    const bool hasB = sB < S;
    Column<T> col[VEC];
#pragma unroll
    for (int j = 0; j < VEC; ++j) col[j].init();
    const int eA = wave * 256 + 2 * lane;
    if (NL_LDS) {
      col_nL[eA] = col_nL[eA + 1] = col_nL[eA + 128] = col_nL[eA + 129] = epa::M<T>::nan();
    }
    long long dcur = 0x7ff8dead00000001ll, racur = 0x7ff8dead00000002ll;
    uint32_t n_clean = 0u;
    bool plain = false;
    const int s4 = chunk0 + wave * 256 + 4 * lane;
    PingLoad<RawT> nxt;
    epa::CoefRow nxtR = rowp0[pb < pe ? pb : 0];
    double nxtDs = 1.0, nxtDo = 0.0;
    if (DEPTH) {
      nxtDs = uniform(dsc_c[pb < pe ? pb : 0]);
      nxtDo = uniform(dof_c[pb < pe ? pb : 0]);
    }
    int nxtNv = nv_c && pb < pe ? nv_c[pb] : S;
    if (pb < pe) nxt.issue(raw_c + (size_t)pb * S, sA, sB, hasB, s4, S);
    for (int p = pb; p < pe; ++p) {
      const epa::CoefRow r = nxtR;
      const double curDs = nxtDs, curDo = nxtDo;
      const size_t row_off = (size_t)p * S;
      const int nv = nxtNv;
      float2 inA, inB;
      const bool full = nv_c != nullptr && nv >= chunk0 + wave * 256 + 256;
      nxt.resolve(inA, inB, sA, sB, nv, full);
      if (p + 1 < pe) {
        nxtR = rowp0[p + 1];
        if (nv_c) nxtNv = nv_c[p + 1];
        if (DEPTH) {
          nxtDs = uniform(dsc_c[p + 1]);
          nxtDo = uniform(dof_c[p + 1]);
        }
        nxt.issue(raw_c + row_off + S, sA, sB, hasB, s4, S);
      }
      if (!((__double_as_longlong(r.d) == dcur) & (__double_as_longlong(r.ra) == racur))) {
        dcur = __double_as_longlong(r.d);
        racur = __double_as_longlong(r.ra);
        bool fin = true;
        for (int j = 0; j < VEC; ++j) {
          const double sj = (double)((j < 2 ? sA : sB) + (j & 1));
          const T nl = nspread * log10_slow<T>((T)(sj - r.d));
          if (NL_LDS) col_nL[eA + (j < 2 ? 0 : 128) + (j & 1)] = nl;
          else col[j].nL = nl;
          if (SRA_LDS) col_sra[eA + (j < 2 ? 0 : 128) + (j & 1)] = sj * r.ra;
          else col[j].sra = sj * r.ra;
          fin = fin & ((j >= 2 && !hasB) | (fabs(nl) < (T)__builtin_inf()));
        }
        plain = __ballot(!fin) == 0ull;
      }
      const T g = (T)r.g, a2 = (T)r.alpha2;
      T A0 = (T)r.A0;
      double r0v = r.r0;
      asm volatile("" : "+v"(A0), "+v"(r0v));
      bool clean = false;
#if EPA_FUSED_LEAN
      {
        const double xa = fma(SRA_LDS ? col_sra[eA] : col[0].sra, r.rb, r0v);
        bool bad = !(xa - r.shift > 0.0);
        if (!full) bad = bad | not_finite(inA.x) | not_finite(inA.y) | not_finite(inB.x) | not_finite(inB.y);
        bool kpos = (__double2hiint(r.ra) > 0) & (__double2hiint(r.rb) > 0) & finite_bits(r.g) & finite_bits(r.A0) &
                    finite_bits(r.alpha2);
        if (DEPTH) kpos = kpos & finite_bits(curDs) & finite_bits(curDo);
        clean = plain & kpos & (__ballot(bad) == 0ull);
      }
#endif
      const T dsc = (T)curDs, dof = (T)curDo;
      double xf, xl, xdummy;
      process_pair<T, RMAX, WRITE_SV, DEPTH>(col[0], col[1], inA, clean, r, r0v, g, a2, A0, NL_LDS ? col_nL[eA] : col[0].nL,
                                             NL_LDS ? col_nL[eA + 1] : col[1].nL, nspread, bin, inv_bin, n_rbins, tab, lsum,
                                             lcnt, WRITE_SV ? sv_c + row_off + sA : nullptr, xmax, xmin, nnan, n_clean, xf,
                                             xl, dsc, dof, DEPTH == 2 ? dp_c + row_off + sA : nullptr,
                                             SRA_LDS ? col_sra[eA] : col[0].sra, SRA_LDS ? col_sra[eA + 1] : col[1].sra);
      if (hasB)
        process_pair<T, RMAX, WRITE_SV, DEPTH>(col[2], col[3], inB, clean, r, r0v, g, a2, A0,
                                               NL_LDS ? col_nL[eA + 128] : col[2].nL, NL_LDS ? col_nL[eA + 129] : col[3].nL,
                                               nspread, bin, inv_bin, n_rbins, tab, lsum, lcnt,
                                               WRITE_SV ? sv_c + row_off + sB : nullptr, xmax, xmin, nnan, n_clean, xdummy,
                                               xl, dsc, dof, DEPTH == 2 ? dp_c + row_off + sB : nullptr,
                                               SRA_LDS ? col_sra[eA + 128] : col[2].sra,
                                               SRA_LDS ? col_sra[eA + 129] : col[3].sra);
      if (clean) {
        if (RMAX) {
          if (DEPTH) {
            xmin = vmin_num(vmin_num(xmin, xf), xl);
            xmax = vmax_num(vmax_num(xmax, xf), xl);
          } else {
            xmin = vmin_num(xmin, xf);
            xmax = vmax_num(xmax, xl);
          }
        }
        ++n_clean;
      }
    }
#pragma unroll
    for (int j = 0; j < VEC; ++j) col[j].flush(lsum, lcnt, n_clean);
  }
  }
  if (RMAX) {
#pragma unroll
    for (int o = 32; o > 0; o >>= 1) xmax = fmax(xmax, __shfl_down(xmax, o, 64));
#pragma unroll
    for (int o = 32; o > 0; o >>= 1) xmin = fmin(xmin, __shfl_down(xmin, o, 64));
    if (lane == 0) {
      if (xmax > -__builtin_inf()) atomicMax(&wg_keys[0], ordered_key(xmax));
      if (xmin < __builtin_inf()) atomicMin(&wg_keys[1], ordered_key(xmin));
      if (nnan > 0u) atomicAdd(&wg_nnan, nnan);
    }
    __syncthreads();
    if (threadIdx.x == 0) {
      const unsigned long long kmax = wg_keys[0], kmin = wg_keys[1];
      if (kmax != 0ull) atomicMax(a.rmax_key, kmax);
      if (a.rstat) {
        if (kmin != ~0ull) atomicMin(a.rstat, kmin);
        if (wg_nnan > 0u) atomicAdd(a.rstat + 1, (unsigned long long)wg_nnan);
      }
    }
  }
  if (extra) return;
  __syncthreads();
  const size_t cell0 = ((size_t)c * a.n_tbins + tb) * n_rbins;
  T* out = mvbs_out + cell0;
  T* gsum = sum_out ? sum_out + cell0 : nullptr;
  uint32_t* gcnt = cnt_out ? cnt_out + cell0 : nullptr;
  for (int i = threadIdx.x; i < n_rbins; i += epa::kBlock) {
    const uint32_t n = lcnt[i];
    const T s = lsum[i];
    out[i] = n > 0u ? (T)10 * epa::M<T>::log10(s / (T)n) : (T)a.fill_value;
    if (gsum) gsum[i] = s;
    if (gcnt) gcnt[i] = n;
  }
}

template <typename T, typename RawT>
int launch(Args& a, const RawT* raw, const int32_t* n_valid, const double* coef, const int32_t* bin_start,
           void* sv_out, void* mvbs_out, void* sum_out, uint32_t* cnt_out, int C, size_t lds_bytes,
           hipStream_t st) {
  const dim3 grid((unsigned)a.n_tbins + 1u, (unsigned)C);
  a.tab_off = (unsigned)((lds_bytes + 15) & ~(size_t)15);
  lds_bytes = a.tab_off + epa::kMathTabBytes;
  a.xcd_map = epa::xcd_map_enabled() ? 1 : 0;
#define EPA_FL(W, R) EPA_FLD(W, R, 0)
#define EPA_FLD(W, R, D)                                                                       \
  do {                                                                                         \
    auto kern = fused_sv_mvbs_kernel<T, RawT, W, R, D>;                                        \
    if (lds_bytes > 64 * 1024)                                                                 \
      EPA_CHECK_HIP(hipFuncSetAttribute(reinterpret_cast<const void*>(kern),                   \
                                        hipFuncAttributeMaxDynamicSharedMemorySize,            \
                                        (int)lds_bytes));                                      \
    hipLaunchKernelGGL(kern, grid, dim3(epa::kBlock), lds_bytes, st, raw, n_valid,             \
                       reinterpret_cast<const epa::CoefRow*>(coef), bin_start, (T*)sv_out,     \
                       (T*)mvbs_out, (T*)sum_out, cnt_out, a.dscale, a.doffset, a);            \
  } while (0)
  if (a.dscale) {
    if constexpr (std::is_same<RawT, float>::value) {
      if (a.depth_out) EPA_FLD(true, true, 2);
      else if (sv_out) EPA_FLD(true, true, 1);
      else EPA_FLD(false, true, 1);
    } else {
      epa::set_error("epa_sv_mvbs_fused_depth: float power samples only");
      return EPA_EUNSUPPORTED;
    }
  } else if (a.rmax_key) {
    if (sv_out) EPA_FL(true, true); else EPA_FL(false, true);
  } else {
    if (sv_out) EPA_FL(true, false); else EPA_FL(false, false);
  }
#undef EPA_FLD
#undef EPA_FL
  return epa::check_launch("fused_sv_mvbs_kernel");
}

__global__ __launch_bounds__(epa::kBlock) void selftest_lin_kernel(const double* __restrict__ u,
                                                                   double* __restrict__ out,
                                                                   size_t n) {
  __shared__ __attribute__((aligned(16))) unsigned char tabs[epa::kMathTabBytes];
  const epa::MathTabs mt = epa::build_math_tabs(tabs);
  __syncthreads();
  for (size_t i = (size_t)blockIdx.x * blockDim.x + threadIdx.x; i < n;
       i += (size_t)gridDim.x * blockDim.x)
    out[i] = epa::lin_from_db(u[i], mt.exp2_tab);
}

__global__ __launch_bounds__(epa::kBlock) void selftest_log_kernel(const double* __restrict__ x,
                                                                   double* __restrict__ out,
                                                                   size_t n) {
  __shared__ __attribute__((aligned(16))) unsigned char tabs[epa::kMathTabBytes];
  const epa::MathTabs mt = epa::build_math_tabs(tabs);
  __syncthreads();
  for (size_t i = (size_t)blockIdx.x * blockDim.x + threadIdx.x; i < n;
       i += (size_t)gridDim.x * blockDim.x)
    out[i] = epa::fast_log10(x[i], mt.log_tab);
}

__global__ __launch_bounds__(epa::kBlock) void selftest_log_inl_kernel(const double* __restrict__ x,
                                                                       double* __restrict__ out, size_t n) {
  __shared__ __attribute__((aligned(16))) unsigned char tabs[epa::kMathTabBytes];
  const epa::MathTabs mt = epa::build_math_tabs(tabs);
  __syncthreads();
  for (size_t i = (size_t)blockIdx.x * blockDim.x + threadIdx.x; i < n;
       i += (size_t)gridDim.x * blockDim.x)
    out[i] = epa::fast_log10_inl<false>(x[i], mt.log_tab);
}

template <typename T>
struct SvColumn {
  double sra, blo, bhi;
  T acc_sum;
  int acc_rb;
  uint32_t acc_cnt;
  __device__ __forceinline__ void init() { sra = 0.0; blo = 1.0; bhi = 0.0; acc_sum = (T)0; acc_rb = -1; acc_cnt = 0u; }
  __device__ __forceinline__ void flush(T* lsum, uint32_t* lcnt) {
    if (acc_rb >= 0 && acc_cnt > 0u) {
      lds_add(lsum + acc_rb, acc_sum);
      atomicAdd(lcnt + acc_rb, acc_cnt);
    }
  }
};

template <typename T, bool AS_STORED>
__device__ __forceinline__ void bin_sv_sample(SvColumn<T>& c, T sv, const epa::CoefRow& r, double bin, double inv_bin,
                                              int n_rbins, const double* tab, T* lsum, uint32_t* lcnt) {
  const double x0 = c.sra * r.rb + r.r0;
  const double x = AS_STORED ? (double)(T)x0 : x0;
  const T v = epa::lin_from_db(sv, tab);
  const bool same = (x >= c.blo) & (x < c.bhi);
  if (!same) {
    const int rb = (x == x) ? epa::range_bin_index(x, bin, inv_bin, n_rbins, false) : -1;
    if (rb != c.acc_rb) {
      c.flush(lsum, lcnt);
      c.acc_rb = rb;
      c.acc_sum = (T)0;
      c.acc_cnt = 0u;
    }
    c.blo = rb >= 0 ? (double)rb * bin : 1.0;
    c.bhi = rb >= 0 ? (double)(rb + 1) * bin : 0.0;
  }
  const bool take = (c.acc_rb >= 0) & (v == v);
  c.acc_sum += take ? v : (T)0;
  c.acc_cnt += take ? 1u : 0u;
}

constexpr int kFixedPings = 512;
template <typename T>
struct LeftMark;
template <>
struct LeftMark<double> {
  static constexpr unsigned long long kBits = 0x7ff8dead0c0ffee2ull;
};
template <>
struct LeftMark<float> {
  static constexpr unsigned kBits = 0x7fcdead2u;
};
__device__ __forceinline__ bool left_to_rows(const double* cell) {
  return *reinterpret_cast<const unsigned long long*>(cell) == LeftMark<double>::kBits;
}
__device__ __forceinline__ bool left_to_rows(const float* cell) {
  return *reinterpret_cast<const unsigned*>(cell) == LeftMark<float>::kBits;
}
__device__ __forceinline__ void mark_left(double* cell) {
  *reinterpret_cast<unsigned long long*>(cell) = LeftMark<double>::kBits;
}
__device__ __forceinline__ void mark_left(float* cell) { *reinterpret_cast<unsigned*>(cell) = LeftMark<float>::kBits; }

template <typename T, bool AS_STORED>
__global__ __launch_bounds__(epa::kBlock, sizeof(T) == 8 ? 6 : 8) void mvbs_of_sv_fixed_kernel(
    const T* __restrict__ sv, const epa::CoefRow* __restrict__ coef, const int32_t* __restrict__ bin_start,
    T* __restrict__ mvbs_out, T* __restrict__ sum_out, uint32_t* __restrict__ cnt_out, Args a) {
  typedef T T2 __attribute__((ext_vector_type(2)));
  extern __shared__ __attribute__((aligned(16))) unsigned char smem[];
  T* lsum = reinterpret_cast<T*>(smem);
  uint32_t* lcnt = reinterpret_cast<uint32_t*>(smem + a.cnt_off);
  const epa::MathTabs mt = epa::build_math_tabs(smem + a.tab_off);
  const double* tab = mt.exp2_tab;
  __shared__ int differs;
  __shared__ unsigned long long rb_lo_key, rb_hi_key;
  const int c = blockIdx.y, tb = a.xcd_map ? epa::xcd_contiguous(blockIdx.x, a.n_tbins) : (int)blockIdx.x;
  const int S = a.S, n_rbins = a.n_rbins;
  const int pb = bin_start[tb], pe = bin_start[tb + 1], np = pe - pb;
  const size_t cell0 = ((size_t)c * a.n_tbins + tb) * n_rbins;
  for (int i = threadIdx.x; i < n_rbins; i += epa::kBlock) {
    lsum[i] = (T)0;
    lcnt[i] = 0u;
  }
  if (threadIdx.x == 0) {
    differs = np > kFixedPings ? 1 : 0;
    rb_lo_key = ~0ull;
    rb_hi_key = 0ull;
  }
  __syncthreads();
  const epa::CoefRow* __restrict__ rowp0 = coef + (size_t)c * a.P;
  const epa::CoefRow r = rowp0[np > 0 ? pb : 0];
  for (int i = threadIdx.x; i < min(np, kFixedPings); i += epa::kBlock) {
    const epa::CoefRow ri = rowp0[pb + i];
    if (!((ri.ra == r.ra) & (ri.r0 == r.r0) & (ri.rb == ri.rb) & (ri.ra > 0.0))) differs = 1;
    atomicMin(&rb_lo_key, ordered_key(ri.rb));
    atomicMax(&rb_hi_key, ordered_key(ri.rb));
  }
  __syncthreads();
  if (differs) {
    if (threadIdx.x == 0) mark_left(mvbs_out + cell0);
    return;
  }
  auto unkey = [](unsigned long long k) {
    return __longlong_as_double((long long)((k >> 63) ? (k & 0x7fffffffffffffffull) : ~k));
  };
  const double rb_lo = unkey(rb_lo_key), rb_hi = unkey(rb_hi_key);
  const double bin = a.range_bin, inv_bin = a.inv_range_bin;
  const T* __restrict__ sv_c = sv + (size_t)c * a.P * S;
  const int wave = threadIdx.x >> 6, lane = threadIdx.x & 63;
  auto range_of = [&](int sx, double rb) {
    const double x0 = ((double)sx * r.ra) * rb + r.r0;
    return AS_STORED ? (double)(T)x0 : x0;
  };
  for (int chunk0 = 0; chunk0 < S; chunk0 += kChunk) {
    const int sA = chunk0 + wave * 256 + 2 * lane;
    const int sB = sA + 128;
    if (sA >= S) continue;
    const bool hasB = sB < S;
    int rbin[VEC];
    T acc_sum[VEC];
    uint32_t acc_cnt[VEC];
    unsigned fixed = 0;
#pragma unroll
    for (int j = 0; j < VEC; ++j) {
      const int sx = (j < 2 ? sA : sB) + (j & 1);
      const int b_lo = epa::range_bin_index(range_of(sx, rb_lo), bin, inv_bin, n_rbins, false);
      const int b_hi = epa::range_bin_index(range_of(sx, rb_hi), bin, inv_bin, n_rbins, false);
      rbin[j] = b_lo;
      if (b_lo == b_hi) fixed |= 1u << j;
      acc_sum[j] = (T)0;
      acc_cnt[j] = 0u;
    }
    T2 nA0 = {(T)0, (T)0}, nB0 = nA0, nA1 = nA0, nB1 = nA0;
    if (np > 0) {
      nA0 = *reinterpret_cast<const T2*>(sv_c + (size_t)pb * S + sA);
      if (hasB) nB0 = *reinterpret_cast<const T2*>(sv_c + (size_t)pb * S + sB);
    }
    if (np > 1) {
      nA1 = *reinterpret_cast<const T2*>(sv_c + (size_t)(pb + 1) * S + sA);
      if (hasB) nB1 = *reinterpret_cast<const T2*>(sv_c + (size_t)(pb + 1) * S + sB);
    }
    for (int p = pb; p < pe; ++p) {
      const T2 inA = nA0, inB = nB0;
      nA0 = nA1;
      nB0 = nB1;
      if (p + 2 < pe) {
        const T* nx = sv_c + (size_t)(p + 2) * S;
        nA1 = *reinterpret_cast<const T2*>(nx + sA);
        if (hasB) nB1 = *reinterpret_cast<const T2*>(nx + sB);
      }
      const T in[VEC] = {inA.x, inA.y, inB.x, inB.y};
#pragma unroll
      for (int j = 0; j < VEC; ++j) {
        if (j >= 2 && !hasB) break;
        const T v = epa::lin_from_db_lean(in[j], tab);
        acc_sum[j] += vmax_num(v, (T)0);
        acc_cnt[j] += v == v ? 1u : 0u;
      }
    }
#pragma unroll
    for (int j = 0; j < VEC; ++j) {
      if (((fixed >> j) & 1u) != 0u && rbin[j] >= 0 && acc_cnt[j] > 0u) {
        lds_add(lsum + rbin[j], acc_sum[j]);
        atomicAdd(lcnt + rbin[j], acc_cnt[j]);
      }
    }
    const unsigned loose = (~fixed) & (hasB ? 0xfu : 0x3u);
    if (__ballot(loose != 0u) != 0ull) {
      const int nact = (int)__popcll(__ballot(true));
#pragma unroll 1
      for (int j = 0; j < VEC; ++j) {
        unsigned long long todo = __ballot(((loose >> j) & 1u) != 0u);
        while (todo != 0ull) {
          const int src = __ffsll((long long)todo) - 1;
          todo &= todo - 1ull;
          const int sx = chunk0 + wave * 256 + 2 * src + (j < 2 ? 0 : 128) + (j & 1);
          for (int p = pb + lane; p < pe; p += nact) {
            const T v = epa::lin_from_db_lean(sv_c[(size_t)p * S + sx], tab);
            const double x = range_of(sx, rowp0[p].rb);
            const int rb = epa::range_bin_index(x, bin, inv_bin, n_rbins, false);
            if ((rb >= 0) & (v == v)) {
              lds_add(lsum + rb, v);
              atomicAdd(lcnt + rb, 1u);
            }
          }
        }
      }
    }
  }
  __syncthreads();
  T* out = mvbs_out + cell0;
  T* gsum = sum_out ? sum_out + cell0 : nullptr;
  uint32_t* gcnt = cnt_out ? cnt_out + cell0 : nullptr;
  for (int i = threadIdx.x; i < n_rbins; i += epa::kBlock) {
    const uint32_t n = lcnt[i];
    const T s = lsum[i];
    out[i] = n > 0u ? (T)10 * epa::M<T>::log10(s / (T)n) : (T)a.fill_value;
    if (gsum) gsum[i] = s;
    if (gcnt) gcnt[i] = n;
  }
}

template <typename T, bool AS_STORED>
__global__ __launch_bounds__(epa::kBlock, EPA_FUSED_MIN_WAVES) void mvbs_of_sv_rows_kernel(
    const T* __restrict__ sv, const epa::CoefRow* __restrict__ coef, const int32_t* __restrict__ bin_start,
    T* __restrict__ mvbs_out, T* __restrict__ sum_out, uint32_t* __restrict__ cnt_out, Args a) {
  typedef T T2 __attribute__((ext_vector_type(2)));
  extern __shared__ __attribute__((aligned(16))) unsigned char smem[];
  T* lsum = reinterpret_cast<T*>(smem);
  uint32_t* lcnt = reinterpret_cast<uint32_t*>(smem + a.cnt_off);
  const epa::MathTabs mt = epa::build_math_tabs(smem + a.tab_off);
  const double* tab = mt.exp2_tab;
  const int c = blockIdx.y, tb = a.xcd_map ? epa::xcd_contiguous(blockIdx.x, a.n_tbins) : (int)blockIdx.x;
  const int S = a.S, n_rbins = a.n_rbins;
  if (a.flagged_only && !left_to_rows(mvbs_out + ((size_t)c * a.n_tbins + tb) * n_rbins)) return;
  for (int i = threadIdx.x; i < n_rbins; i += epa::kBlock) {
    lsum[i] = (T)0;
    lcnt[i] = 0u;
  }
  __syncthreads();
  const double bin = a.range_bin, inv_bin = a.inv_range_bin;
  const epa::CoefRow* __restrict__ rowp0 = coef + (size_t)c * a.P;
  const T* __restrict__ sv_c = sv + (size_t)c * a.P * S;
  const int wave = threadIdx.x >> 6, lane = threadIdx.x & 63;
  const int pb = bin_start[tb], pe = bin_start[tb + 1];
  for (int chunk0 = 0; chunk0 < S; chunk0 += kChunk) {
    const int sA = chunk0 + wave * 256 + 2 * lane;
    const int sB = sA + 128;
    if (sA >= S) continue;
    const bool hasB = sB < S;
    SvColumn<T> col[VEC];
#pragma unroll
    for (int j = 0; j < VEC; ++j) col[j].init();
    double racur = __builtin_nan("");
    T2 nA = {(T)0, (T)0}, nB = {(T)0, (T)0};
    epa::CoefRow nxtR = rowp0[pb < pe ? pb : 0];
    if (pb < pe) {
      nA = *reinterpret_cast<const T2*>(sv_c + (size_t)pb * S + sA);
      if (hasB) nB = *reinterpret_cast<const T2*>(sv_c + (size_t)pb * S + sB);
    }
    for (int p = pb; p < pe; ++p) {
      const epa::CoefRow r = nxtR;
      const T2 inA = nA, inB = nB;
      if (p + 1 < pe) {
        nxtR = rowp0[p + 1];
        const T* nx = sv_c + (size_t)(p + 1) * S;
        nA = *reinterpret_cast<const T2*>(nx + sA);
        if (hasB) nB = *reinterpret_cast<const T2*>(nx + sB);
      }
      if (!(r.ra == racur)) {
        racur = r.ra;
        for (int j = 0; j < VEC; ++j) col[j].sra = (double)((j < 2 ? sA : sB) + (j & 1)) * r.ra;
      }
      bin_sv_sample<T, AS_STORED>(col[0], inA.x, r, bin, inv_bin, n_rbins, tab, lsum, lcnt);
      bin_sv_sample<T, AS_STORED>(col[1], inA.y, r, bin, inv_bin, n_rbins, tab, lsum, lcnt);
      if (hasB) {
        bin_sv_sample<T, AS_STORED>(col[2], inB.x, r, bin, inv_bin, n_rbins, tab, lsum, lcnt);
        bin_sv_sample<T, AS_STORED>(col[3], inB.y, r, bin, inv_bin, n_rbins, tab, lsum, lcnt);
      }
    }
#pragma unroll
    for (int j = 0; j < VEC; ++j) col[j].flush(lsum, lcnt);
  }
  __syncthreads();
  const size_t cell0 = ((size_t)c * a.n_tbins + tb) * n_rbins;
  T* out = mvbs_out + cell0;
  T* gsum = sum_out ? sum_out + cell0 : nullptr;
  uint32_t* gcnt = cnt_out ? cnt_out + cell0 : nullptr;
  for (int i = threadIdx.x; i < n_rbins; i += epa::kBlock) {
    const uint32_t n = lcnt[i];
    const T s = lsum[i];
    out[i] = n > 0u ? (T)10 * epa::M<T>::log10(s / (T)n) : (T)a.fill_value;
    if (gsum) gsum[i] = s;
    if (gcnt) gcnt[i] = n;
  }
}

template <typename T>
int launch_sv_rows(Args& a, const void* sv, const double* coef, const int32_t* bin_start, void* mvbs_out, void* sum_out,
                   uint32_t* cnt_out, int C, size_t lds_bytes, bool as_stored, hipStream_t st) {
  const dim3 grid((unsigned)a.n_tbins, (unsigned)C);
  a.tab_off = (unsigned)((lds_bytes + 15) & ~(size_t)15);
  lds_bytes = a.tab_off + epa::kMathTabBytes;
  a.xcd_map = epa::xcd_map_enabled() ? 1 : 0;
  static const bool fixed_off = [] {
    const char* e = getenv("EPA_MVBS_FIXED");
    return e && e[0] == '0';
  }();
#define EPA_SR(KERN, AS)                                                                                 \
  do {                                                                                                   \
    auto kern = KERN<T, AS>;                                                                             \
    if (lds_bytes > 64 * 1024)                                                                           \
      EPA_CHECK_HIP(hipFuncSetAttribute(reinterpret_cast<const void*>(kern),                             \
                                        hipFuncAttributeMaxDynamicSharedMemorySize, (int)lds_bytes));    \
    hipLaunchKernelGGL(kern, grid, dim3(epa::kBlock), lds_bytes, st, (const T*)sv,                       \
                       reinterpret_cast<const epa::CoefRow*>(coef), bin_start, (T*)mvbs_out, (T*)sum_out, \
                       cnt_out, a);                                                                      \
  } while (0)
  a.flagged_only = 0;
  if (!fixed_off) {
    if (as_stored) EPA_SR(mvbs_of_sv_fixed_kernel, true); else EPA_SR(mvbs_of_sv_fixed_kernel, false);
    if (int rc = epa::check_launch("mvbs_of_sv_fixed_kernel")) return rc;
    a.flagged_only = 1;
  }
  if (as_stored) EPA_SR(mvbs_of_sv_rows_kernel, true); else EPA_SR(mvbs_of_sv_rows_kernel, false);
#undef EPA_SR
  return epa::check_launch("mvbs_of_sv_rows_kernel");
}

}

int epa_mvbs_rows_fast_path(const void* sv, const double* coef, int C, int P, int S, const int32_t* bin_start,
                            int n_tbins, double range_bin, int n_rbins, int as_stored, double fill_value,
                            void* mvbs_out, void* sum_out, uint32_t* cnt_out, int dtype, size_t lds_bytes,
                            unsigned cnt_off, hipStream_t st) {
  epa_fused::Args a{};
  a.P = P; a.S = S; a.n_tbins = n_tbins; a.n_rbins = n_rbins;
  a.range_bin = range_bin; a.inv_range_bin = 1.0 / range_bin;
  a.fill_value = fill_value;
  a.skipna = 1;
  a.cnt_off = cnt_off;
  if (dtype == EPA_F64)
    return epa_fused::launch_sv_rows<double>(a, sv, coef, bin_start, mvbs_out, sum_out, cnt_out, C, lds_bytes,
                                             as_stored != 0, st);
  return epa_fused::launch_sv_rows<float>(a, sv, coef, bin_start, mvbs_out, sum_out, cnt_out, C, lds_bytes,
                                          as_stored != 0, st);
}

extern "C" int epa_selftest_lin_from_db(const double* u, double* out, size_t n, epa_stream_t stream) {
  EPA_CHECK_ARG(u && out, "epa_selftest_lin_from_db: NULL array argument");
  if (n == 0) return EPA_OK;
  const size_t blocks = (n + epa::kBlock - 1) / epa::kBlock;
  hipLaunchKernelGGL(epa_fused::selftest_lin_kernel, dim3((unsigned)(blocks < 1024 ? blocks : 1024)),
                     dim3(epa::kBlock), 0, (hipStream_t)stream, u, out, n);
  return epa::check_launch("selftest_lin_kernel");
}

extern "C" int epa_selftest_log10(const double* x, double* out, size_t n, epa_stream_t stream) {
  EPA_CHECK_ARG(x && out, "epa_selftest_log10: NULL array argument");
  if (n == 0) return EPA_OK;
  const size_t blocks = (n + epa::kBlock - 1) / epa::kBlock;
  hipLaunchKernelGGL(epa_fused::selftest_log_kernel, dim3((unsigned)(blocks < 1024 ? blocks : 1024)),
                     dim3(epa::kBlock), 0, (hipStream_t)stream, x, out, n);
  return epa::check_launch("selftest_log_kernel");
}

extern "C" int epa_selftest_log10_inline(const double* x, double* out, size_t n, epa_stream_t stream) {
  EPA_CHECK_ARG(x && out, "epa_selftest_log10_inline: NULL array argument");
  if (n == 0) return EPA_OK;
  const size_t blocks = (n + epa::kBlock - 1) / epa::kBlock;
  hipLaunchKernelGGL(epa_fused::selftest_log_inl_kernel, dim3((unsigned)(blocks < 1024 ? blocks : 1024)),
                     dim3(epa::kBlock), 0, (hipStream_t)stream, x, out, n);
  return epa::check_launch("selftest_log_inl_kernel");
}

int epa_fused_fast_path(const void* raw, int raw_is_i16, const int32_t* n_valid, const double* coef,
                        int C, int P, int S, double nspread,
                        unsigned cal_flags, const int32_t* bin_start, int n_tbins, double range_bin,
                        int n_rbins, unsigned bin_flags, double fill_value, void* sv_out,
                        void* mvbs_out, void* sum_out, uint32_t* cnt_out, int dtype,
                        size_t lds_bytes, unsigned cnt_off, unsigned long long* rmax_key,
                        unsigned long long* rstat, const double* dscale, const double* doffset, void* depth_out,
                        hipStream_t st) {
  epa_fused::Args a{};
  a.dscale = dscale; a.doffset = doffset; a.depth_out = dscale ? depth_out : nullptr;
  a.rmax_key = rmax_key;
  a.rstat = rmax_key ? rstat : nullptr;
  a.P = P; a.S = S; a.n_tbins = n_tbins; a.n_rbins = n_rbins;
  a.range_bin = range_bin; a.inv_range_bin = 1.0 / range_bin;
  a.nspread = nspread; a.fill_value = fill_value;
  a.guard = (cal_flags & EPA_FLAG_GUARD_POS) != 0;
  a.mask_range = (cal_flags & EPA_FLAG_MASK_RANGE) != 0;
  a.skipna = (bin_flags & EPA_BIN_SKIPNA) != 0;
  a.closed_right = (bin_flags & EPA_BIN_CLOSED_RIGHT) != 0;
  a.cnt_off = cnt_off;
#define EPA_GO(T, RawT)                                                                           \
  return epa_fused::launch<T, RawT>(a, reinterpret_cast<const RawT*>(raw), n_valid, coef, bin_start, \
                                    sv_out, mvbs_out, sum_out, cnt_out, C, lds_bytes, st)
  if (raw_is_i16) {
    if (dtype == EPA_F64) EPA_GO(double, int16_t);
    EPA_GO(float, int16_t);
  }
  if (dtype == EPA_F64) EPA_GO(double, float);
  EPA_GO(float, float);
#undef EPA_GO
}
```

### echopype_amd/ops.py

```python
import ctypes
import threading

import numpy as np
import torch

from . import _lib
from ._lib import call

_DT = {torch.float32: _lib.F32, torch.float64: _lib.F64}


def _stream():
    return ctypes.c_void_p(torch.cuda.current_stream().cuda_stream)


def _p(t):
    if t is None:
        return None
    if not t.is_cuda:
        raise ValueError("echopype_amd kernels need device (HBM) buffers; got a CPU tensor")
    if not t.is_contiguous():
        raise ValueError("echopype_amd kernels need C-contiguous buffers")
    return ctypes.c_void_p(t.data_ptr())

# ... 11 lines not shown
class _Uploader:

    _MAX_POOL = 64
    _MAX_BYTES = 256 << 20

    def __init__(self, device):
        self.device = device
        self.stream = torch.cuda.Stream(device=device)
        self.pool = []
        self.lock = threading.Lock()

    def _staging(self, nbytes):
        best = None
        for slot in self.pool:
            buf, ev = slot
            if buf.numel() >= nbytes and (ev is None or ev.query()) and (best is None or buf.numel() < best[0].numel()):
                best = slot
        if best is None:
            if len(self.pool) >= self._MAX_POOL:
                idle = [s_ for s_ in self.pool if s_[1] is None or s_[1].query()]
                if idle:
                    self.pool.remove(min(idle, key=lambda s_: s_[0].numel()))
            best = [torch.empty(max(4096, 1 << (int(nbytes) - 1).bit_length()), dtype=torch.uint8, pin_memory=True), None]
            self.pool.append(best)
        return best

    def upload(self, a):
        nbytes = a.nbytes
        if nbytes == 0 or nbytes > self._MAX_BYTES:
            w = a if a.flags.writeable else a.copy()
            return torch.from_numpy(w).to(self.device)
        tdt = torch.from_numpy(np.empty(0, dtype=a.dtype)).dtype
        cur = torch.cuda.current_stream(self.device)
        with self.lock:
            slot = self._staging(nbytes)
            staged = slot[0][:nbytes]
            staged.numpy().view(np.uint8)[:] = a.reshape(-1).view(np.uint8)
            with torch.cuda.stream(self.stream):
                out = torch.empty(a.shape, dtype=tdt, device=self.device)
                out.view(-1).view(torch.uint8).copy_(staged, non_blocking=True)
                ev = torch.cuda.Event()
                ev.record(self.stream)
            slot[1] = ev
        cur.wait_event(ev)
        out.record_stream(cur)
        out._epa_ready = ev
        return out


class HostFuture:

    __slots__ = ("_slot", "_host", "_event", "_value")

    def __init__(self, slot, host, event):
        self._slot, self._host, self._event, self._value = slot, host, event, None

    def cpu(self):
        if self._value is None:
            self._event.synchronize()
            self._value = self._host.clone()
            self._slot[1] = None
            self._slot = self._host = None
        return self._value

    def tolist(self):
        return self.cpu().tolist()

    def item(self):
        return self.cpu().item()

    def __del__(self):
        slot = getattr(self, "_slot", None)
        if slot is not None:
            slot[1] = None


class _Downloader:

    def __init__(self, device):
        self.device = device
        self.stream = torch.cuda.Stream(device=device)
        self.pool = []
        self.lock = threading.Lock()

    def fetch(self, t):
        t = t.contiguous()
        nbytes = t.numel() * t.element_size()
        with self.lock:
            slot = next((s_ for s_ in self.pool if s_[1] is None and s_[0].numel() >= nbytes), None)
            if slot is None:
                slot = [torch.empty(max(256, 1 << (int(nbytes) - 1).bit_length()), dtype=torch.uint8, pin_memory=True), None]
                self.pool.append(slot)
            slot[1] = True
        host = slot[0][:nbytes].view(t.dtype).view(t.shape)
        cur = torch.cuda.current_stream(self.device)
        ready = torch.cuda.Event()
        ready.record(cur)
        with torch.cuda.stream(self.stream):
            self.stream.wait_event(ready)
            host.copy_(t, non_blocking=True)
            done = torch.cuda.Event()
            done.record(self.stream)
        t.record_stream(self.stream)
        return HostFuture(slot, host, done)


_uploaders = {}
_downloaders = {}


def fetch_async(t):
    dl = _downloaders.get(t.device)
    if dl is None:
        dl = _downloaders[t.device] = _Downloader(t.device)
    return dl.fetch(t)



def _uploader(dev):
    up = _uploaders.get(dev)
    if up is None:
        up = _uploaders[dev] = _Uploader(dev)
    return up


def to_device(a, dtype=None, device=None):
    dev = device if device is not None else torch.device("cuda", torch.cuda.current_device())
    dev = torch.device(dev)
    if dev.type == "cuda" and dev.index is None:
        dev = torch.device("cuda", torch.cuda.current_device())
    if isinstance(a, torch.Tensor):
        t = a
        if dtype is not None and t.dtype != dtype:
            t = t.to(dtype)
        if not t.is_cuda:
            t = _uploader(dev).upload(t.contiguous().numpy()) if dev.type == "cuda" else t.to(dev)
        return t.contiguous()
    a = np.ascontiguousarray(a)
    if dtype is not None:
        want = np.dtype(str(dtype).replace("torch.", ""))
        if a.dtype != want:
            a = a.astype(want)
    if a.dtype.kind == "M":
        a = a.view(np.int64)
    if dev.type != "cuda":
        return torch.from_numpy(a if a.flags.writeable else a.copy()).to(dev)
    return _uploader(dev).upload(a)


_SMALL = {}
_SMALL_MAX = 256


def to_device_small(a, dtype=None, device=None):
    a = np.ascontiguousarray(a)
    if dtype is not None:
        want = np.dtype(str(dtype).replace("torch.", ""))
        if a.dtype != want:
            a = a.astype(want)
    if a.nbytes > 2048 or a.nbytes == 0:
        return to_device(a, device=device)
    dev = torch.device("cuda", torch.cuda.current_device()) if device is None else torch.device(device)
    if dev.type == "cuda" and dev.index is None:
        dev = torch.device("cuda", torch.cuda.current_device())
    key = (dev, a.dtype.str, a.shape, a.tobytes())
    ent = _SMALL.get(key)
    if ent is None:
        if len(_SMALL) >= _SMALL_MAX:
            _SMALL.clear()
        t = to_device(a, device=dev)
        ev = getattr(t, "_epa_ready", None)
        if ev is not None:
            ev.synchronize()
        _SMALL[key] = ent = t
    return ent


_PING_NS = {}


def ping_time_facts(ping_time, want_device=True):
    import weakref

    pt = np.asarray(ping_time)
    if pt.dtype != np.dtype("datetime64[ns]"):
        pt = pt.astype("datetime64[ns]")
    dev = torch.device("cuda", torch.cuda.current_device())
    ent = _PING_NS.get(id(pt)) if not pt.flags.writeable else None
    if ent is not None and ent[0]() is pt:
        _, ns, ok, tens = ent
    else:
        ns = pt.view(np.int64)
        ok = bool(ns.size) and not bool(np.any(ns[1:] < ns[:-1])) and ns[0] != np.iinfo(np.int64).min
        tens = {}
        if not pt.flags.writeable:
            key = id(pt)
            _PING_NS[key] = (weakref.ref(pt, lambda _r, k=key: _PING_NS.pop(k, None)), ns, ok, tens)
    if not want_device:
        return ns, ok, None
    t = tens.get(dev)
    if t is None:
        t = to_device(ns, device=dev)
        tens[dev] = t
    else:
        ev = getattr(t, "_epa_ready", None)
        if ev is not None:
            torch.cuda.current_stream().wait_event(ev)
    return ns, ok, t


def _mode_of(t, C, P):
    n = t.numel()
    if n == 1:
        return _lib.PM_SCALAR
    if n == C and t.dim() <= 1:
        return _lib.PM_CHANNEL
    if n == C * P:
        return _lib.PM_CHANNEL_PING
    raise ValueError(f"parameter of shape {tuple(t.shape)} is not scalar, (C,) or (C,P) with C={C}, P={P}")


def _tau_mode(tau_eff, C, P):
    if tuple(tau_eff.shape) == (C,):
        return _lib.PM_CHANNEL
    if tuple(tau_eff.shape) == (C, P):
        return _lib.PM_CHANNEL_PING
    raise ValueError(f"tau_eff of shape {tuple(tau_eff.shape)}: expected ({C},) or ({C}, {P})")


def power_coef_ek(sample_interval, tau_nominal, transmit_power, sound_speed, absorption, gain, sa,
                  psi, f_nominal, tau_eff, *, sonar="EK60", cal_type="Sv", pulse_length=None,
                  gain_is_table=False, sa_is_table=False, gpt=None):
    C, P = sample_interval.shape
    coef = torch.empty((C, P, _lib.NCOEF), dtype=torch.float64, device=sample_interval.device)
    K = 0 if pulse_length is None else pulse_length.shape[1]
    gmode = _lib.PM_PULSE_TABLE if gain_is_table else _mode_of(gain, C, P)
    smode = _lib.PM_PULSE_TABLE if sa_is_table else _mode_of(sa, C, P)
    call("epa_power_coef_ek", C, P, _p(sample_interval), _p(tau_nominal), _p(transmit_power),
         _p(sound_speed), _mode_of(sound_speed, C, P), _p(absorption), _mode_of(absorption, C, P),
         _p(gain), gmode, _p(sa), smode, _p(pulse_length), K, _p(psi), _mode_of(psi, C, P), _p(f_nominal), _p(tau_eff),
         _tau_mode(tau_eff, C, P), _p(gpt), _lib.SONAR_EK60 if sonar in ("EK60", "ES70") else _lib.SONAR_EK80,
         _lib.CAL_SV if cal_type == "Sv" else _lib.CAL_TS, _p(coef), _stream())
    return coef


def pulse_table_lookup(tau_nominal, pulse_length, table):
    C, P = tau_nominal.shape
    out = torch.empty((C, P), dtype=torch.float64, device=tau_nominal.device)
    call("epa_pulse_table_lookup", _p(tau_nominal), _p(pulse_length), _p(table), C, P, pulse_length.shape[1], _p(out),
         _stream())
    return out


def sv_power_vectorized(raw, S, dtype):
    return S % (2 if dtype == torch.float64 else 4) == 0 and raw.data_ptr() % 16 == 0


def sv_power(raw, coef, *, cal_type="Sv", flags=_lib.FLAG_GUARD_POS | _lib.FLAG_MASK_RANGE,
             dtype=torch.float64, want_range=True, out=None, range_out=None, want_range_stats=False):
    C, P, S = raw.shape
    if raw.dtype != torch.float32:
        raise ValueError("raw power samples must be float32 (convert/parse_base.py:302)")
    if out is None:
        out = torch.empty((C, P, S), dtype=dtype, device=raw.device)
    if want_range and range_out is None:
        range_out = torch.empty((C, P, S), dtype=dtype, device=raw.device)
    ct = _lib.CAL_SV if cal_type == "Sv" else _lib.CAL_TS
    if want_range_stats:
        ws = torch.empty(3 * (S // 256 + 8192 + 1024), dtype=torch.float64, device=raw.device)
        stats = torch.empty(3, dtype=torch.float64, device=raw.device)
        call("epa_sv_power_stats", _p(raw), _p(coef), C, P, S, ct, flags, _p(out),
             _p(range_out) if want_range else None, _DT[out.dtype], _p(ws), _p(stats), _stream())
        return out, (range_out if want_range else None), stats
    call("epa_sv_power", _p(raw), _p(coef), C, P, S, ct, flags, _p(out), _p(range_out) if want_range else None,
         _DT[out.dtype], _stream())
    return out, (range_out if want_range else None)


def range_power(raw, coef, *, flags=_lib.FLAG_MASK_RANGE, dtype=torch.float64):
    C, P, S = raw.shape
    out = torch.empty((C, P, S), dtype=dtype, device=raw.device)
    call("epa_range_power", _p(raw), _p(coef), C, P, S, flags, _p(out), _DT[dtype], _stream())
    return out


def time_bin_offsets(ping_time_ns, t0, dt, n_bins, closed="left"):
    P = ping_time_ns.numel()
    out = torch.empty(n_bins + 1, dtype=torch.int32, device=ping_time_ns.device)
    call("epa_time_bin_offsets", _p(ping_time_ns), P, int(t0), int(dt), int(n_bins),
         _lib.BIN_CLOSED_RIGHT if closed == "right" else 0, _p(out), _stream())
    return out


def _bin_flags(skipna, closed):
    return (_lib.BIN_SKIPNA if skipna else 0) | (_lib.BIN_CLOSED_RIGHT if closed == "right" else 0)


def reduce_needs_workspace(C, n_tbins, n_rbins, dtype):
    esz = 8 if dtype == torch.float64 else 4
    lds = ((n_rbins * esz + 15) & ~15) + 4 * n_rbins
    return C * n_tbins < 1024 or lds > 128 * 1024


def sv_mvbs_fused(raw, coef, bin_start, n_tbins, range_bin, n_rbins, *, cal_type="Sv",
                  cal_flags=_lib.FLAG_GUARD_POS | _lib.FLAG_MASK_RANGE, skipna=True, closed="left",
                  fill_value=float("nan"), dtype=torch.float64, want_sv=True, want_range=False,
                  want_partials=False, ping_perm=None, sv_out=None, range_out=None, mvbs_out=None,
                  want_range_max=False, want_range_stats=False):
    C, P, S = raw.shape
    dev = raw.device
    if want_sv and sv_out is None:
        sv_out = torch.empty((C, P, S), dtype=dtype, device=dev)
    if want_range and range_out is None:
        range_out = torch.empty((C, P, S), dtype=dtype, device=dev)
    if mvbs_out is None:
        mvbs_out = torch.empty((C, n_tbins, n_rbins), dtype=dtype, device=dev)
    ssum = cnt = None
    if want_partials or reduce_needs_workspace(C, n_tbins, n_rbins, dtype):
        ssum = torch.empty((C, n_tbins, n_rbins), dtype=dtype, device=dev)
        cnt = torch.empty((C, n_tbins, n_rbins), dtype=torch.int32, device=dev)
    rmax = torch.empty(1, dtype=torch.float64, device=dev) if want_range_max or want_range_stats else None
    rstats = torch.empty(3, dtype=torch.float64, device=dev) if want_range_stats else None
    call("epa_sv_mvbs_fused", _p(raw), _p(coef), C, P, S,
         _lib.CAL_SV if cal_type == "Sv" else _lib.CAL_TS, cal_flags, _p(bin_start), _p(ping_perm),
         int(n_tbins), float(range_bin), int(n_rbins), _bin_flags(skipna, closed), float(fill_value),
         _p(sv_out) if want_sv else None, _p(range_out) if want_range else None, _p(mvbs_out),
         _p(ssum), _p(cnt), _p(rmax), _p(rstats), _DT[dtype], _stream())
    return dict(Sv=sv_out if want_sv else None, echo_range=range_out if want_range else None,
                MVBS=mvbs_out, sum=ssum, cnt=cnt, range_max=rmax, range_stats=rstats,
                range_stats_filled=bool(_lib.lib.epa_last_range_stats_filled()) if want_range_stats else False)


def sv_mvbs_fused_depth(raw, coef, depth_scale, depth_offset, bin_start, n_tbins, range_bin, n_rbins, *, cal_type="Sv",
                        fill_value=float("nan"), dtype=torch.float64, want_sv=True, want_depth=False,
                        want_partials=False, sv_out=None, mvbs_out=None):
    C, P, S = raw.shape
    dev = raw.device
    if want_sv and sv_out is None:
        sv_out = torch.empty((C, P, S), dtype=dtype, device=dev)
    depth_out = torch.empty((C, P, S), dtype=dtype, device=dev) if want_depth else None
    if mvbs_out is None:
        mvbs_out = torch.empty((C, n_tbins, n_rbins), dtype=dtype, device=dev)
    ssum = cnt = None
    if want_partials:
        ssum = torch.empty((C, n_tbins, n_rbins), dtype=dtype, device=dev)
        cnt = torch.empty((C, n_tbins, n_rbins), dtype=torch.int32, device=dev)
    rstats = torch.empty(64, dtype=torch.float64, device=dev)
    call("epa_sv_mvbs_fused_depth", _p(raw), _p(coef), _p(depth_scale), _p(depth_offset), C, P, S,
         _lib.CAL_SV if cal_type == "Sv" else _lib.CAL_TS, _p(bin_start), int(n_tbins), float(range_bin), int(n_rbins),
         float(fill_value), _p(sv_out) if want_sv else None, _p(depth_out), _p(mvbs_out), _p(ssum), _p(cnt), _p(rstats),
         _DT[dtype], _stream())
    return dict(Sv=sv_out if want_sv else None, depth=depth_out, MVBS=mvbs_out, sum=ssum, cnt=cnt,
                range_stats=rstats[:3], range_stats_filled=True)


def sv_mvbs_fused_i16(raw_i16, n_valid, coef, bin_start, n_tbins, range_bin, n_rbins, *, cal_type="Sv",
                      fill_value=float("nan"), dtype=torch.float64, want_sv=True, want_partials=False,
                      sv_out=None, mvbs_out=None, want_range_max=False):
    C, P, S = raw_i16.shape
    if raw_i16.dtype != torch.int16 or n_valid.dtype != torch.int32:
        raise ValueError("raw_i16 must be int16 and n_valid int32")
    dev = raw_i16.device
    if want_sv and sv_out is None:
        sv_out = torch.empty((C, P, S), dtype=dtype, device=dev)
    if mvbs_out is None:
        mvbs_out = torch.empty((C, n_tbins, n_rbins), dtype=dtype, device=dev)
    ssum = cnt = None
    if want_partials:
        ssum = torch.empty((C, n_tbins, n_rbins), dtype=dtype, device=dev)
        cnt = torch.empty((C, n_tbins, n_rbins), dtype=torch.int32, device=dev)
    rmax = torch.empty(1, dtype=torch.float64, device=dev) if want_range_max else None
    call("epa_sv_mvbs_fused_i16", _p(raw_i16), _p(n_valid), _p(coef), C, P, S,
         _lib.CAL_SV if cal_type == "Sv" else _lib.CAL_TS, _p(bin_start), int(n_tbins), float(range_bin),
         int(n_rbins), float(fill_value), _p(sv_out) if want_sv else None, _p(mvbs_out), _p(ssum), _p(cnt),
         _p(rmax), _DT[dtype], _stream())
    return dict(Sv=sv_out if want_sv else None, MVBS=mvbs_out, sum=ssum, cnt=cnt, range_max=rmax)


def mvbs(sv, bin_start, n_tbins, range_bin, n_rbins, *, range=None, coef=None, skipna=True,
         closed="left", fill_value=float("nan"), want_partials=False, ping_perm=None, coef_as_stored=False):
    C, P, S = sv.shape
    dev, dtype = sv.device, sv.dtype
    if range is not None and range.dtype != dtype:
        range = range.to(dtype)
    out = torch.empty((C, n_tbins, n_rbins), dtype=dtype, device=dev)
    ssum = cnt = None
    if want_partials or reduce_needs_workspace(C, n_tbins, n_rbins, dtype):
        ssum = torch.empty((C, n_tbins, n_rbins), dtype=dtype, device=dev)
        cnt = torch.empty((C, n_tbins, n_rbins), dtype=torch.int32, device=dev)
    call("epa_mvbs", _p(sv), _p(range), _p(coef), C, P, S, _p(bin_start), _p(ping_perm), int(n_tbins),
         float(range_bin), int(n_rbins), _bin_flags(skipna, closed) | (_lib.BIN_RANGE_AS_STORED if coef_as_stored else 0),
         float(fill_value), _p(out), _p(ssum), _p(cnt), _DT[dtype], _stream())
    return dict(MVBS=out, sum=ssum, cnt=cnt)


def selftest_lin_from_db(u):
    out = torch.empty_like(u)
    call("epa_selftest_lin_from_db", _p(u), _p(out), u.numel(), _stream())
    return out


def selftest_log10(x, inline=False):
    out = torch.empty_like(x)
    call("epa_selftest_log10_inline" if inline else "epa_selftest_log10", _p(x), _p(out), x.numel(), _stream())
    return out


def selftest_correlate(x, replica, fft_dtype=None):
    if x.dim() != 2 or x.shape[1] != _lib.EK80_NFFT or x.dtype not in (torch.complex64, torch.complex128):
        raise ValueError(f"x: (T, {_lib.EK80_NFFT}) complex64 / complex128 tiles expected")
    if replica.dtype != torch.complex64 or replica.dim() != 1 or not 1 <= replica.numel() <= _lib.EK80_NFFT:
        raise ValueError(f"replica: 1 .. {_lib.EK80_NFFT} complex64 taps expected")
    fdt = torch.float32 if x.dtype == torch.complex64 else torch.float64
    if fft_dtype is not None and torch_dtype(fft_dtype) != fdt:
        raise ValueError("fft_dtype is the precision of x")
    xr, rr = torch.view_as_real(x.contiguous()), torch.view_as_real(replica.contiguous())
    off = torch.tensor([0, replica.numel()], dtype=torch.int32, device=x.device)
    ws = torch.empty(768 + 4 + 3 * _lib.EK80_NFFT + 3 * 1024 + 2 + 1 + 5 + 256, dtype=torch.float64,
                     device=x.device)
    out = torch.empty_like(xr)
    call("epa_selftest_correlate", _p(xr), x.shape[0], _p(rr), _p(off), _DT[fdt], _p(out), _p(ws), _stream())
    return torch.view_as_complex(out)


def mvbs_finalize(ssum, cnt, fill_value=float("nan")):
    out = torch.empty_like(ssum)
    call("epa_mvbs_finalize", _p(ssum), _p(cnt), ssum.numel(), float(fill_value), _p(out),
         _DT[ssum.dtype], _stream())
    return out


def affine_rows(x, scale, offset):
    C, P, S = x.shape
    out = torch.empty_like(x)
    call("epa_affine_rows", _p(x), _p(scale), _p(offset), C, P, S, _p(out), _DT[x.dtype], _stream())
    return out


def depth_rows(scale, offset, *, range=None, coef=None, mask_raw=None, shape=None, dtype=None, want_stats=True):
    if range is not None:
        C, P, S = range.shape
        dtype, dev = range.dtype, range.device
    else:
        C, P, S = shape
        dev = coef.device
    out = torch.empty((C, P, S), dtype=dtype, device=dev)
    ws = stats = None
    if want_stats:
        ws = torch.empty(3 * 16384, dtype=torch.float64, device=dev)
        stats = torch.empty(3, dtype=torch.float64, device=dev)
    call("epa_depth_rows", _p(range), _p(coef), _p(mask_raw), _p(scale), _p(offset), C, P, S, _p(out), _DT[dtype],
         _p(ws), _p(stats), _stream())
    return out, stats


def nanminmax(x, with_nan_count=False):
    ws = torch.empty(3072, dtype=torch.float64, device=x.device)
    out = torch.empty(3, dtype=torch.float64, device=x.device)
    call("epa_nanminmax", _p(x), x.numel(), _DT[x.dtype], _p(ws), _p(out), _stream())
    lo, hi, nn = out.cpu().tolist()
    return (lo, hi, int(nn)) if with_nan_count else (lo, hi)


def mvbs_index(sv, ping_num, range_sample_num, range=None):
    C, P, S = sv.shape
    Pb, Sb = -(-P // ping_num), -(-S // range_sample_num)
    out = torch.empty((C, Pb, Sb), dtype=sv.dtype, device=sv.device)
    rmin = None
    if range is not None:
        if range.dtype != sv.dtype:
            range = range.to(sv.dtype)
        rmin = torch.empty((C, Pb, Sb), dtype=sv.dtype, device=sv.device)
    call("epa_mvbs_index", _p(sv), _p(range), C, P, S, int(ping_num), int(range_sample_num), _p(out),
         _p(rmin), _DT[sv.dtype], _stream())
    return out, rmin


def noise_estimate(sv, alpha2, ping_num, range_sample_num, *, range=None, coef=None,
                   noise_max=float("nan"), ping_phase=0, want_edges=False):
    C, P, S = sv.shape
    if range is not None and range.dtype != sv.dtype:
        range = range.to(sv.dtype)
    out = torch.empty((C, -(-(P + ping_phase) // ping_num)), dtype=torch.float64, device=sv.device)
    es = ec = None
    if want_edges:
        Sb = -(-S // range_sample_num)
        es = torch.zeros((2, C, Sb), dtype=torch.float64, device=sv.device)
        ec = torch.zeros((2, C, Sb), dtype=torch.int32, device=sv.device)
    call("epa_noise_estimate", _p(sv), _p(range), _p(coef), _p(alpha2), C, P, S, int(ping_num),
         int(range_sample_num), int(ping_phase), float(noise_max), _p(out), _p(es), _p(ec), _DT[sv.dtype], _stream())
    return (out, es, ec) if want_edges else out


def noise_finalize(ssum, cnt, noise_max=float("nan")):
    rows, Sb = ssum.shape
    out = torch.empty(rows, dtype=torch.float64, device=ssum.device)
    call("epa_noise_finalize", _p(ssum), _p(cnt), rows, Sb, float(noise_max), _p(out), _stream())
    return out


def noise_apply(sv, alpha2, noise, ping_num, snr_threshold, *, range=None, coef=None, mask_raw=None,
                want_noise=True, want_corrected=True, want_minmax=False, ping_phase=0, minmax_async=False):
    C, P, S = sv.shape
    if range is not None and range.dtype != sv.dtype:
        range = range.to(sv.dtype)
    sn = torch.empty_like(sv) if want_noise else None
    sc = torch.empty_like(sv) if want_corrected else None
    mm = torch.empty(4, dtype=torch.float64, device=sv.device) if want_minmax else None
    if range is None and mask_raw is not None:
        call("epa_noise_apply_rows", _p(sv), _p(coef), _p(mask_raw), _p(alpha2), _p(noise), C, P, S, int(ping_num),
             int(ping_phase), float(snr_threshold), _p(sn), _p(sc), _p(mm), _DT[sv.dtype], _stream())
    else:
        call("epa_noise_apply", _p(sv), _p(range), _p(coef), _p(alpha2), _p(noise), C, P, S, int(ping_num),
             int(ping_phase), float(snr_threshold), _p(sn), _p(sc), _p(mm), _DT[sv.dtype], _stream())
    return (sn, sc, fetch_async(mm) if minmax_async else mm.cpu().tolist()) if want_minmax else (sn, sc)


def complex_coef_ek80(params, tau_eff, C, P, *, B, bb, cal_type="Sv", gpt=None):
    dev = tau_eff.device
    ptrs = (ctypes.c_void_p * len(_lib.CCP))()
    modes = (ctypes.c_int * len(_lib.CCP))()
    keep = []
    for k, name in enumerate(_lib.CCP):
        t = params.get(name)
        if t is None:
            ptrs[k], modes[k] = None, _lib.PM_SCALAR
            continue
        t = t.to(torch.float64).contiguous()
        keep.append(t)
        ptrs[k], modes[k] = t.data_ptr(), _mode_of(t, C, P)
    out = torch.empty((C, P, _lib.NCCOEF), dtype=torch.float64, device=dev)
    call("epa_complex_coef_ek80", C, P, ptrs, modes, _p(tau_eff), _tau_mode(tau_eff, C, P), _p(gpt), int(B), 1 if bb else 0,
         _lib.CAL_SV if cal_type == "Sv" else _lib.CAL_TS, _p(out), _stream())
    return out


def sv_complex_uses_fft(replica, max_taps, method="auto"):
    return replica is not None and (method == "fft" or (method == "auto" and 16 <= max_taps <= _lib.EK80_NFFT // 2))


def range_complex(re, ccoef, *, dtype=torch.float64):
    C, P, S, B = re.shape
    out = torch.empty((C, P, S), dtype=dtype, device=re.device)
    call("epa_range_complex", _p(re), _DT[re.dtype], _p(ccoef), C, P, S, B, _p(out), _DT[dtype], _stream())
    return out


def power_rows_of_complex(ccoef):
    rows = torch.zeros(tuple(ccoef.shape[:2]) + (_lib.NCOEF,), dtype=torch.float64, device=ccoef.device)
    rows[..., 0] = ccoef[..., _lib.CC_RA]
    rows[..., 1] = ccoef[..., _lib.CC_RB]
    return rows


def sv_complex(re, im, ccoef, *, replica=None, replica_off=None, max_taps=0, cal_type="Sv",
               dtype=torch.float64, want_range=True, want_prx=False, method="auto", fft_dtype=None,
               want_range_stats=False, replica_id=None):
    C, P, S, B = re.shape
    n_rep = C if replica_id is None else int(replica_off.numel()) - 1
    if replica_id is not None and (replica is None or tuple(replica_id.shape) != (C, P) or replica_id.dtype != torch.int32):
        raise ValueError("replica_id: int32 (C, P) next to replica / replica_off")
    if re.dtype != im.dtype or re.dtype not in _DT:
        raise ValueError("backscatter_r / backscatter_i must both be float32 or float64")
    if method not in ("auto", "direct", "fft"):
        raise ValueError("method must be 'auto', 'direct' or 'fft'")
    dev = re.device
    out = torch.empty((C, P, S), dtype=dtype, device=dev)
    rng = torch.empty((C, P, S), dtype=dtype, device=dev) if want_range else None
    prx = torch.empty((C, P, S), dtype=dtype, device=dev) if want_prx else None
    cal = _lib.CAL_SV if cal_type == "Sv" else _lib.CAL_TS
    use_fft = sv_complex_uses_fft(replica, max_taps, method)
    stats = None
    if use_fft:
        W = max(C, n_rep)
        n_ws = (768 + 4 * W + 3 * W * _lib.EK80_NFFT + 3 * 1024 + 2
                + (W * P * (S // (_lib.EK80_NFFT // 2 + 1) + 1) + 63) // 64 + W * (S + 4) + 256)
        ws = torch.empty(n_ws, dtype=torch.float64, device=dev)
        fdt = torch_dtype(fft_dtype) if fft_dtype is not None else dtype
        if want_range_stats:
            stats = torch.empty(3, dtype=torch.float64, device=dev)
        if replica_id is None:
            call("epa_sv_complex_fft", _p(re), _p(im), _DT[re.dtype], _p(replica), _p(replica_off), int(max_taps),
                 _p(ccoef), C, P, S, B, cal, _p(out), _p(rng), _p(prx), _DT[dtype], _DT[fdt], _p(ws), _p(stats),
                 _stream())
        else:
            call("epa_sv_complex_fft_indexed", _p(re), _p(im), _DT[re.dtype], _p(replica), _p(replica_off),
                 _p(replica_id), n_rep, int(max_taps), _p(ccoef), C, P, S, B, cal, _p(out), _p(rng), _p(prx),
                 _DT[dtype], _DT[fdt], _p(ws), _p(stats), _stream())
    elif replica is None and want_range_stats:
        ws = torch.empty(3072, dtype=torch.float64, device=dev)
        stats = torch.empty(3, dtype=torch.float64, device=dev)
        call("epa_sv_complex_cw_stats", _p(re), _p(im), _DT[re.dtype], _p(ccoef), C, P, S, B, cal, _p(out), _p(rng),
             _p(prx), _DT[dtype], _p(ws), _p(stats), _stream())
    elif replica_id is not None:
        call("epa_sv_complex_indexed", _p(re), _p(im), _DT[re.dtype], _p(replica), _p(replica_off), _p(replica_id), n_rep,
             int(max_taps), _p(ccoef), C, P, S, B, cal, _p(out), _p(rng), _p(prx), _DT[dtype], _stream())
    else:
        call("epa_sv_complex", _p(re), _p(im), _DT[re.dtype], _p(replica), _p(replica_off), int(max_taps),
             _p(ccoef), C, P, S, B, cal, _p(out), _p(rng), _p(prx), _DT[dtype], _stream())
    return dict(out=out, echo_range=rng, prx=prx, range_stats=stats)



SPLITBEAM_PARAMS = ("angle_sensitivity_alongship", "angle_sensitivity_athwartship", "angle_offset_alongship",
                    "angle_offset_athwartship")
SPLITBEAM_BEAM_TYPES = (1, 17, 49, 65, 81)


def _angle_params(params, C, P):
    if len(params) != 4:
        raise ValueError("four angle parameters: sensitivity along / athwart, offset along / athwart")
    keep = [t.to(torch.float64).contiguous() for t in params]
    ptrs = (ctypes.c_void_p * 4)(*[t.data_ptr() for t in keep])
    modes = (ctypes.c_int * 4)(*[_mode_of(t, C, P) for t in keep])
    for t in keep:
        _p(t)
    return ptrs, modes, keep


def splitbeam_power(along, athw, params, *, dtype=torch.float64):
    C, P, S = along.shape
    if athw.shape != along.shape or athw.dtype != along.dtype:
        raise ValueError("angle_alongship / angle_athwartship: same shape and dtype")
    codes = {torch.int8: _lib.I8, torch.float32: _lib.F32, torch.float64: _lib.F64}
    if along.dtype not in codes:
        raise ValueError(f"angle planes must be int8, float32 or float64 (got {along.dtype})")
    ptrs, modes, keep = _angle_params(params, C, P)
    theta = torch.empty((C, P, S), dtype=dtype, device=along.device)
    phi = torch.empty_like(theta)
    call("epa_splitbeam_power", _p(along), _p(athw), codes[along.dtype], ptrs, modes, C, P, S, _p(theta), _p(phi),
         _DT[dtype], _stream())
    return theta, phi


def splitbeam_uses_fft(replica, max_taps, method="auto"):
    return sv_complex_uses_fft(replica, max_taps, method)


def splitbeam_complex(re, im, beam_type, params, *, replica=None, replica_off=None, max_taps=0, replica_id=None,
                      dtype=torch.float64, method="auto", fft_dtype=None):
    C, P, S, B = re.shape
    if re.dtype != im.dtype or re.dtype not in _DT or im.shape != re.shape:
        raise ValueError("backscatter_r / backscatter_i must both be float32 or float64 of one shape")
    if method not in ("auto", "direct", "fft"):
        raise ValueError("method must be 'auto', 'direct' or 'fft'")
    bt = np.ascontiguousarray(np.asarray(beam_type, dtype=np.int32).reshape(-1))
    if bt.size != C:
        raise ValueError(f"beam_type: {C} values expected, got {bt.size}")
    if replica_id is not None and (replica is None or tuple(replica_id.shape) != (C, P) or replica_id.dtype != torch.int32):
        raise ValueError("replica_id: int32 (C, P) next to replica / replica_off")
    n_rep = 0 if replica is None else (C if replica_id is None else int(replica_off.numel()) - 1)
    ptrs, modes, keep = _angle_params(params, C, P)
    dev = re.device
    theta = torch.empty((C, P, S), dtype=dtype, device=dev)
    phi = torch.empty_like(theta)
    bt_p = bt.ctypes.data_as(ctypes.c_void_p)
    if splitbeam_uses_fft(replica, max_taps, method):
        ws = torch.empty(768 + 3 * n_rep * _lib.EK80_NFFT, dtype=torch.float64, device=dev)
        fdt = torch_dtype(fft_dtype) if fft_dtype is not None else torch.float64
        call("epa_splitbeam_complex_fft", _p(re), _p(im), _DT[re.dtype], bt_p, ptrs, modes, _p(replica),
             _p(replica_off), _p(replica_id), n_rep, int(max_taps), C, P, S, B, _p(theta), _p(phi), _DT[dtype],
             _DT[fdt], _p(ws), _stream())
    else:
        call("epa_splitbeam_complex", _p(re), _p(im), _DT[re.dtype], bt_p, ptrs, modes, _p(replica), _p(replica_off),
             _p(replica_id), n_rep, int(max_taps), C, P, S, B, _p(theta), _p(phi), _DT[dtype], _stream())
    return theta, phi

def _plane_dtype(t, what):
    if t.dim() != 2 or t.dtype not in _DT:
        raise ValueError(f"{what}: a (ping_time, range_sample) float32 / float64 plane expected, got {tuple(t.shape)} "
                         f"{t.dtype}")
    return _DT[t.dtype]


def seafloor_state(device):
    return torch.zeros(_lib.SEAFLOOR_STATE_WORDS, dtype=torch.int64, device=device)


# ... 502 lines not shown
```

### include/echopype_amd.h

```cpp
#ifndef ECHOPYPE_AMD_H
#define ECHOPYPE_AMD_H

#include <stddef.h>
#include <stdint.h>

#ifdef __cplusplus
extern "C" {
#endif

#define EPA_VERSION 104

typedef void* epa_stream_t;

enum epa_status { EPA_OK = 0, EPA_EINVAL = 1, EPA_EHIP = 2, EPA_ENOMEM = 3, EPA_EUNSUPPORTED = 4 };
enum epa_dtype { EPA_F32 = 0, EPA_F64 = 1 };
enum epa_cal_type { EPA_CAL_SV = 0, EPA_CAL_TS = 1 };
enum epa_sonar { EPA_SONAR_EK60 = 0, EPA_SONAR_EK80 = 1 };
enum epa_param_mode { EPA_PM_SCALAR = 0, EPA_PM_CHANNEL = 1, EPA_PM_CHANNEL_PING = 2, EPA_PM_PULSE_TABLE = 3 };

#define EPA_NCOEF 8
enum epa_coef_slot { EPA_CF_RA = 0, EPA_CF_RB = 1, EPA_CF_R0 = 2, EPA_CF_SHIFT = 3, EPA_CF_ALPHA2 = 4,
                     EPA_CF_A0 = 5, EPA_CF_G = 6, EPA_CF_D = 7 };

#define EPA_FLAG_GUARD_POS 1u
#define EPA_FLAG_MASK_RANGE 2u

#define EPA_BIN_SKIPNA 1u
#define EPA_BIN_CLOSED_RIGHT 2u
#define EPA_BIN_RANGE_AS_STORED 4u

int epa_version(void);
const char* epa_source_digest(void);
const char* epa_last_error(void);
const char* epa_launch_trace(int mode);
int epa_last_range_stats_filled(void);
const char* epa_launch_seen(void);
int epa_device_count(int* n);
int epa_set_device(int dev);
int epa_device_name(int dev, char* buf, size_t len);
int epa_malloc(void** ptr, size_t bytes);
int epa_free(void* ptr);
int epa_memset(void* ptr, int value, size_t bytes, epa_stream_t stream);
int epa_memcpy_h2d(void* dst, const void* src_host, size_t bytes, epa_stream_t stream);
int epa_memcpy_d2h(void* dst_host, const void* src, size_t bytes, epa_stream_t stream);
int epa_stream_synchronize(epa_stream_t stream);
int epa_timer_create(void** timer);
int epa_timer_destroy(void* timer);
int epa_timer_start(void* timer, epa_stream_t stream);
int epa_timer_stop(void* timer, epa_stream_t stream);
int epa_timer_elapsed_ms(void* timer, float* ms);

int epa_power_coef_ek(int C, int P, const double* sample_interval, const double* tau_nominal,
                      const double* transmit_power, const double* sound_speed, int ss_mode,
                      const double* absorption, int abs_mode, const double* gain, int gain_mode,
                      const double* sa_correction, int sa_mode, const double* pulse_length, int K,
                      const double* psi, int psi_mode, const double* f_nominal, const double* tau_eff,
                      int tau_eff_mode, const uint8_t* gpt, int sonar, int cal_type, double* coef, epa_stream_t stream);

int epa_pulse_table_lookup(const double* tau_nominal, const double* pulse_length, const double* table, int C, int P,
                           int K, double* out, epa_stream_t stream);

int epa_sv_power(const float* raw, const double* coef, int C, int P, int S, int cal_type,
                 unsigned flags, void* out, void* range_out, int out_dtype, epa_stream_t stream);
#define EPA_SV_POWER_STATS_WS_DOUBLES(S) (3 * ((size_t)(S) / 256 + 8192 + 1024))
int epa_sv_power_stats(const float* raw, const double* coef, int C, int P, int S, int cal_type,
                       unsigned flags, void* out, void* range_out, int out_dtype, double* workspace,
                       double* range_stats_out, epa_stream_t stream);
int epa_range_power(const float* raw, const double* coef, int C, int P, int S, unsigned flags, void* range_out,
                    int out_dtype, epa_stream_t stream);

int epa_time_bin_offsets(const int64_t* ping_time, int P, int64_t t0, int64_t dt, int n_bins,
                         unsigned flags, int32_t* bin_start, epa_stream_t stream);

int epa_sv_mvbs_fused(const float* raw, const double* coef, int C, int P, int S, int cal_type,
                      unsigned cal_flags, const int32_t* bin_start, const int32_t* ping_perm,
                      int n_tbins, double range_bin, int n_rbins, unsigned bin_flags,
                      double fill_value, void* sv_out, void* range_out, void* mvbs_out,
                      void* sum_out, uint32_t* cnt_out, double* range_max_out, double* range_stats_out,
                      int dtype, epa_stream_t stream);

int epa_sv_mvbs_fused_i16(const int16_t* raw, const int32_t* n_valid, const double* coef, int C, int P,
                          int S, int cal_type, const int32_t* bin_start, int n_tbins, double range_bin,
                          int n_rbins, double fill_value, void* sv_out, void* mvbs_out, void* sum_out,
                          uint32_t* cnt_out, double* range_max_out, int dtype, epa_stream_t stream);

int epa_sv_mvbs_fused_depth(const float* raw, const double* coef, const double* depth_scale,
                            const double* depth_offset, int C, int P, int S, int cal_type, const int32_t* bin_start,
                            int n_tbins, double range_bin, int n_rbins, double fill_value, void* sv_out,
                            void* depth_out, void* mvbs_out, void* sum_out, uint32_t* cnt_out, double* depth_stats_out,
                            int dtype, epa_stream_t stream);

int epa_mvbs(const void* sv, const void* range, const double* coef, int C, int P, int S,
             const int32_t* bin_start, const int32_t* ping_perm, int n_tbins, double range_bin,
             int n_rbins, unsigned bin_flags, double fill_value, void* mvbs_out, void* sum_out,
             uint32_t* cnt_out, int dtype, epa_stream_t stream);

int epa_selftest_lin_from_db(const double* u, double* out, size_t n, epa_stream_t stream);
int epa_selftest_log10(const double* x, double* out, size_t n, epa_stream_t stream);
int epa_selftest_log10_inline(const double* x, double* out, size_t n, epa_stream_t stream);

int epa_mvbs_finalize(const void* sum, const uint32_t* cnt, size_t n, double fill_value, void* out,
                      int dtype, epa_stream_t stream);

int epa_edge_pack(const void* const* sum_rows, const uint32_t* const* cnt_rows, const long long* chan_stride,
                  const int* slots, int n_rows, int sum_dtype, int C, int R, int n_slots, int zero_first, double* buf,
                  epa_stream_t stream);
int epa_edge_gather(const double* buf, int n_slots, const int32_t* group_off, const int32_t* group_slots, int n_edges,
                    int C, int R, double* totals_out, void* sum_out, uint32_t* cnt_out, int sum_dtype,
                    epa_stream_t stream);
int epa_edge_finalize_mvbs(const double* buf, int n_slots, const int32_t* group_off, const int32_t* group_slots,
                           const int* edges, void* const* dst_rows, const long long* chan_stride, int n_rows, int C,
                           int R, double fill_value, int dtype, epa_stream_t stream);
int epa_edge_prepare_max(double* values, int n, epa_stream_t stream);

int epa_affine_rows(const void* x, const double* scale, const double* offset, int C, int P, int S,
                    void* out, int dtype, epa_stream_t stream);
#define EPA_DEPTH_ROWS_WS_DOUBLES (3 * 16384)
int epa_depth_rows(const void* range, const double* coef, const float* mask_raw, const double* scale,
                   const double* offset, int C, int P, int S, void* out, int dtype, double* workspace,
                   double* stats_out, epa_stream_t stream);

int epa_nanminmax(const void* x, size_t n, int dtype, double* workspace, double* out,
                  epa_stream_t stream);

int epa_mvbs_index(const void* sv, const void* range, int C, int P, int S, int ping_num,
                   int range_sample_num, void* mvbs_out, void* range_min_out, int dtype,
                   epa_stream_t stream);

int epa_noise_estimate(const void* sv, const void* range, const double* coef, const double* alpha2,
                       int C, int P, int S, int ping_num, int range_sample_num, int ping_phase, double noise_max,
                       double* noise_out, double* edge_sum_out, uint32_t* edge_cnt_out, int dtype,
                       epa_stream_t stream);

int epa_noise_finalize(const double* sum, const double* cnt, int rows, int n_rblocks, double noise_max,
                       double* noise_out, epa_stream_t stream);

int epa_noise_apply(const void* sv, const void* range, const double* coef, const double* alpha2,
                    const double* noise, int C, int P, int S, int ping_num, int ping_phase, double snr_threshold,
                    void* sv_noise_out, void* sv_corrected_out, double* minmax_out, int dtype,
                    epa_stream_t stream);
int epa_noise_apply_rows(const void* sv, const double* coef, const float* mask_raw, const double* alpha2,
                         const double* noise, int C, int P, int S, int ping_num, int ping_phase,
                         double snr_threshold, void* sv_noise_out, void* sv_corrected_out, double* minmax_out,
                         int dtype, epa_stream_t stream);

#define EPA_NCCOEF 8
enum epa_ccoef_slot { EPA_CC_RA = 0, EPA_CC_RB = 1, EPA_CC_SHIFT = 2, EPA_CC_ALPHA2 = 3, EPA_CC_A = 4,
                      EPA_CC_PSCALE = 5, EPA_CC_RSV0 = 6, EPA_CC_RSV1 = 7 };
enum epa_ccoef_param { EPA_CCP_SAMPLE_INTERVAL = 0, EPA_CCP_TAU_NOMINAL, EPA_CCP_TRANSMIT_POWER, EPA_CCP_SOUND_SPEED,
                       EPA_CCP_ABSORPTION, EPA_CCP_GAIN, EPA_CCP_FREQ_CENTER, EPA_CCP_PSI, EPA_CCP_SA_CORRECTION,
                       EPA_CCP_Z_ER, EPA_CCP_Z_ET, EPA_CCP_ANGLE_OFFSET_ALONGSHIP, EPA_CCP_ANGLE_OFFSET_ATHWARTSHIP,
                       EPA_CCP_BEAMWIDTH_ALONGSHIP, EPA_CCP_BEAMWIDTH_ATHWARTSHIP, EPA_CCP_COUNT };
int epa_complex_coef_ek80(int C, int P, const double* const* params, const int* modes, const double* tau_eff,
                          int tau_eff_mode, const uint8_t* gpt, int B, int bb, int cal_type, double* ccoef,
                          epa_stream_t stream);

int epa_sv_complex(const void* re, const void* im, int in_dtype, const float* replica,
                   const int32_t* replica_off, int max_taps, const double* ccoef, int C, int P,
                   int S, int B, int cal_type, void* out, void* range_out, void* prx_out,
                   int out_dtype, epa_stream_t stream);
int epa_sv_complex_indexed(const void* re, const void* im, int in_dtype, const float* replica,
                           const int32_t* replica_off, const int32_t* replica_id, int n_replicas, int max_taps,
                           const double* ccoef, int C, int P, int S, int B, int cal_type, void* out, void* range_out,
                           void* prx_out, int out_dtype, epa_stream_t stream);

#define EPA_EK80_NFFT 2048
#define EPA_EK80_FFT_WS_DOUBLES(C, P, S)                                              \
  (768 + 4 * (size_t)(C) + 3 * (size_t)(C) * EPA_EK80_NFFT + 3 * 1024 + 2 +          \
   ((size_t)(C) * (size_t)(P) * ((size_t)(S) / (EPA_EK80_NFFT / 2 + 1) + 1) + 63) / 64 + \
   (size_t)(C) * ((size_t)(S) + 4) + 256)
int epa_sv_complex_fft(const void* re, const void* im, int in_dtype, const float* replica,
                       const int32_t* replica_off, int max_taps, const double* ccoef, int C, int P,
                       int S, int B, int cal_type, void* out, void* range_out, void* prx_out,
                       int out_dtype, int fft_dtype, double* workspace, double* range_stats_out,
                       epa_stream_t stream);
int epa_selftest_correlate(const void* x, int n_tiles, const float* replica, const int32_t* replica_off,
                           int fft_dtype, void* out, double* workspace, epa_stream_t stream);
int epa_sv_complex_fft_indexed(const void* re, const void* im, int in_dtype, const float* replica,
                               const int32_t* replica_off, const int32_t* replica_id, int n_replicas, int max_taps,
                               const double* ccoef, int C, int P, int S, int B, int cal_type, void* out,
                               void* range_out, void* prx_out, int out_dtype, int fft_dtype, double* workspace,
                               double* range_stats_out, epa_stream_t stream);

#define EPA_I8 2

int epa_splitbeam_power(const void* along, const void* athw, int in_dtype, const double* const* params_host,
                        const int* modes_host, int C, int P, int S, void* theta, void* phi, int out_dtype,
                        epa_stream_t stream);

int epa_splitbeam_complex(const void* re, const void* im, int in_dtype, const int32_t* beam_type_host,
                          const double* const* params_host, const int* modes_host, const float* replica,
                          const int32_t* replica_off, const int32_t* replica_id, int n_replicas, int max_taps, int C,
                          int P, int S, int B, void* theta, void* phi, int out_dtype, epa_stream_t stream);

#define EPA_SPLITBEAM_FFT_WS_DOUBLES(n) (768 + 3 * (size_t)(n) * EPA_EK80_NFFT)
int epa_splitbeam_complex_fft(const void* re, const void* im, int in_dtype, const int32_t* beam_type_host,
                              const double* const* params_host, const int* modes_host, const float* replica,
                              const int32_t* replica_off, const int32_t* replica_id, int n_replicas, int max_taps,
                              int C, int P, int S, int B, void* theta, void* phi, int out_dtype, int fft_dtype,
                              double* workspace, epa_stream_t stream);

#define EPA_SV_COMPLEX_CW_STATS_WS_DOUBLES 3072
int epa_sv_complex_cw_stats(const void* re, const void* im, int in_dtype, const double* ccoef, int C, int P, int S,
                            int B, int cal_type, void* out, void* range_out, void* prx_out, int out_dtype,
                            double* workspace, double* range_stats_out, epa_stream_t stream);

int epa_range_complex(const void* re, int in_dtype, const double* ccoef, int C, int P, int S, int B,
                      void* range_out, int out_dtype, epa_stream_t stream);


int epa_range_bin_smooth(const void* sv, const void* range, int C, int P, int S, int nper, double r0,
                         double bin, int nbins, void* up_out, int dtype, epa_stream_t stream);

int epa_impulse_mask(const void* up, int C, int P, int S, int num_side_pings, double threshold,
                     uint8_t* mask_out, int dtype, epa_stream_t stream);

enum epa_pool_func { EPA_POOL_NANMEAN = 0, EPA_POOL_NANMEDIAN = 1 };
int epa_pool_sv(const void* sv, int C, int P, int S, int first_sample, int num_side_pings,
                int num_side_samples, int func, double threshold, void* pooled_out, uint8_t* mask_out,
                double* ws_sum, int32_t* ws_cnt, int dtype, epa_stream_t stream);

int epa_attenuated_mask(const void* sv, const void* range, int C, int P, int S, double upper_limit,
                        double lower_limit, int num_side_pings, double threshold, uint8_t* mask_out,
                        int dtype, epa_stream_t stream);

int epa_apply_mask(const void* src, const uint8_t* mask, size_t n, size_t mask_period,
                   double fill_value, const void* fill_array, size_t fill_period, void* out,
                   int dtype, epa_stream_t stream);

#define EPA_APPLY_MASKS_WS_DOUBLES 131072
int epa_apply_masks(const void* src, const uint8_t* const* masks, const size_t* mask_periods, int n_masks, size_t n,
                    double fill_value, const void* fill_array, size_t fill_period, void* out, double* workspace,
                    double* minmax_out, int dtype, epa_stream_t stream);

int epa_mask_and(const uint8_t* a, const uint8_t* b, size_t n, size_t b_period, uint8_t* out,
                 epa_stream_t stream);

int epa_range_step_mean(const void* range, int C, int P, int S, int dtype, double* workspace,
                        double* out, epa_stream_t stream);

int epa_first_not_le(const void* x, size_t n, double limit, int dtype, uint64_t* out,
                     epa_stream_t stream);

int epa_range_rows_check(const void* range, int C, int P, int S, int dtype, int32_t* nvalid_out,
                         int32_t* violations_out, epa_stream_t stream);

#define EPA_POOL_VALUE_WS_BYTES(C, P, S) \
  ((size_t)(C) * (P) * (S) * 40 + (size_t)(C) * (S) * 8 + (size_t)(C) * 8 + (size_t)(C) * (P))
#define EPA_POOL_VALUE_MEDIAN_WS_BYTES(C, S) (((size_t)(C) * (S) * 2 + (size_t)(C) * 2) * 4)
int epa_pool_sv_value(const void* sv, const void* range, const int32_t* nvalid, int C, int P, int S,
                      double depth_bin, int num_side_pings, double exclude_above, double range_min,
                      double range_max, int func, double threshold, void* pooled_out, uint8_t* mask_out,
                      void* ws, int dtype, epa_stream_t stream);

int epa_geodesic_steps(const double* lat, const double* lon, int P, double* step_m_out, epa_stream_t stream);
int epa_nasc(const void* sv, const void* depth, int C, int P, int S, const int32_t* bin_start, int n_dbins,
             double range_bin, int n_rbins, unsigned bin_flags, void* workspace, void* nasc_out,
             void* sv_mean_out, void* h_mean_out, int dtype, epa_stream_t stream);

int epa_sv_noise_fused(const float* raw, const double* coef, const double* alpha2, int C, int P, int S,
                       int cal_type, unsigned cal_flags, int ping_num, int range_sample_num, int ping_phase,
                       double noise_max, void* sv_out, void* range_out, double* noise_out, double* edge_sum_out,
                       uint32_t* edge_cnt_out, double* range_max_out, double* range_stats_out, int dtype,
                       epa_stream_t stream);

int epa_denoise_mvbs(const void* sv, const void* range, const double* coef, const double* alpha2,
                     const double* noise, int C, int P, int S, int ping_num, double snr_threshold,
                     const int32_t* bin_start, const int32_t* ping_perm, int n_tbins, double range_bin,
                     int n_rbins, unsigned bin_flags, double fill_value, void* sv_noise_out,
                     void* sv_corrected_out, void* mvbs_out, void* sum_out, uint32_t* cnt_out, int dtype,
                     epa_stream_t stream);

int epa_sv_denoise_mvbs(const float* raw, const double* coef, const double* alpha2, const double* noise,
                        int C, int P, int S, int cal_type, unsigned cal_flags, int ping_num, int ping_phase,
                        double snr_threshold, const int32_t* bin_start, const int32_t* ping_perm,
                        int n_tbins, double range_bin, int n_rbins, unsigned bin_flags, double fill_value,
                        void* sv_noise_out, void* sv_corrected_out, void* range_out, void* mvbs_out,
                        void* sum_out, uint32_t* cnt_out, double* minmax_out, int dtype, epa_stream_t stream);

#define EPA_SEAFLOOR_STATE_WORDS 16

int epa_seafloor_depth_uniform(const void* depth, int dtype, long long P, long long S, int* bad_pings,
                               epa_stream_t stream);

int epa_seafloor_basic(const void* sv, int dtype, long long P, long long S, long long skip, double tmin, double tmax,
                       const double* depth0, double offset, double* out, epa_stream_t stream);

int epa_seafloor_angle_mask(const void* theta, const void* phi, int dtype, long long P, long long S, long long r0,
                            long long R, int wtheta, int wphi, double ttheta, double tphi, double* work,
                            unsigned char* mask, unsigned long long* state, epa_stream_t stream);

int epa_seafloor_median(const void* sv, int dtype, long long P, long long S, long long r0, long long R,
                        const unsigned char* mask, unsigned long long* state, unsigned long long* hist,
                        epa_stream_t stream);

int epa_seafloor_components(const void* sv, int dtype, long long P, long long S, long long r0, long long R,
                            double threshold, unsigned char* mask, long long* parent, unsigned long long* state,
                            epa_stream_t stream);

int epa_seafloor_bottom(const long long* parent, const unsigned char* mask, long long P, long long R, long long r0,
                        const double* depth0, double offset, void* out, int out_dtype, epa_stream_t stream);

#define EPA_SHOAL_STATE_WORDS 8
#define EPA_SHOAL_QUEUE_BOXES 4096

int epa_shoal_threshold_fill(const void* sv, int dtype, long long P, long long S, double thr, long long maxvgap,
                             long long maxhgap, unsigned char* plane, epa_stream_t stream);

int epa_shoal_label(const unsigned char* plane, long long P, long long S, int connectivity, long long* parent,
                    int* box, int* flag, long long cap, unsigned long long* state, epa_stream_t stream);

int epa_shoal_weill_filter(const long long* parent, long long P, long long S, const int* box, int* flag,
                           long long cap, double minvlen, double minhlen, unsigned long long* state,
                           unsigned char* plane, epa_stream_t stream);

int epa_shoal_echoview_link(const long long* parent, long long P, long long S, int* box, int* group, int* flag,
                            long long cap, const double* idim, long long ni, const double* jdim, long long nj,
                            double mincan0, double mincan1, double maxlink0, double maxlink1, double minsho0,
                            double minsho1, int* queue, unsigned long long* state, unsigned char* plane,
                            epa_stream_t stream);

int epa_transient_fielding(const void* sv, int dtype, int C, int P, int S, const int* chan, int max_rows, int n,
                           double thr0, double thr1, double maxts, long long* list, unsigned* count,
                           uint8_t* mask_out, epa_stream_t stream);

int epa_transient_matecho(const void* sv, int dtype, int C, int P, int S, const double* range, const int* chan_i,
                          const double* chan_d, const double* bottom, int bottom_rows, int half_window,
                          double percentile, double delta_db, int extend_ping, double min_window, int* s_hi,
                          uint8_t* flag, uint8_t* mask_out, epa_stream_t stream);

enum epa_cmp { EPA_CMP_GT = 0, EPA_CMP_LT = 1, EPA_CMP_LE = 2, EPA_CMP_GE = 3, EPA_CMP_EQ = 4 };
int epa_freq_diff_mask(const void* sv, int C, size_t n, int chan_a, int chan_b, int cmp, double diff,
                       uint8_t* mask_out, int dtype, epa_stream_t stream);

int epa_regrid_mask(const uint8_t* mask, const int32_t* group, int T, int P, int D, const double* range,
                    int range_per_ping, const int32_t* bin_start, int n_tbins, double range_bin, int n_rbins,
                    unsigned bin_flags, int func, uint8_t* out, int32_t* nonbinary_out, epa_stream_t stream);

int epa_echo_metrics(const void* sv, const void* range, int range_per_row, long long R, long long S,
                     const double* cm_in, void* abundance, void* center_of_mass, void* dispersion, void* evenness,
                     void* aggregation, int dtype, int max_grid, epa_stream_t stream);

#ifdef __cplusplus
}
#endif
#endif
```

Before: 493.7 billion range-samples/s.

## Precompute per-channel spreading-loss column table in a prepass kernel

Adds a small prepass kernel that computes nspread*log10(s - d) once per channel and sample into a global workspace. The fused Sv/MVBS kernel then loads these values instead of recomputing the slow log10 in every block. The per-column refresh is split so a change in range coefficient no longer forces the log10 recompute. The LDS setup now builds only the exp2 table, dropping the log table. The cost is an extra launch, a workspace allocation per call, and the assumption that d is constant along ping; if d changes per ping the old in-loop recompute still handles it.

```diff
diff --git a/echopype_amd/_lib.py b/echopype_amd/_lib.py
--- a/echopype_amd/_lib.py
+++ b/echopype_amd/_lib.py
@@ -83,6 +83,12 @@
     "epa_sv_mvbs_fused_i16": [_vp, _vp, _vp, _i, _i, _i, _i, _vp, _i, _d, _i, _d, _vp, _vp, _vp, _vp, _vp, _i, _vp],
     "epa_sv_mvbs_fused_depth": [_vp, _vp, _vp, _vp, _i, _i, _i, _i, _vp, _i, _d, _i, _d, _vp, _vp, _vp, _vp, _vp, _vp, _i,
                                 _vp],
+    "epa_sv_mvbs_fused_tab": [_vp, _vp, _i, _i, _i, _i, _u, _vp, _vp, _i, _d, _i, _u, _d, _vp, _vp, _vp,
+                              _vp, _vp, _vp, _vp, _i, _vp, _vp],
+    "epa_sv_mvbs_fused_i16_tab": [_vp, _vp, _vp, _i, _i, _i, _i, _vp, _i, _d, _i, _d, _vp, _vp, _vp, _vp, _vp, _i, _vp,
+                                  _vp],
+    "epa_sv_mvbs_fused_depth_tab": [_vp, _vp, _vp, _vp, _i, _i, _i, _i, _vp, _i, _d, _i, _d, _vp, _vp, _vp, _vp, _vp, _vp,
+                                    _i, _vp, _vp],
     "epa_mvbs": [_vp, _vp, _vp, _i, _i, _i, _vp, _vp, _i, _d, _i, _u, _d, _vp, _vp, _vp, _i, _vp],
     "epa_selftest_lin_from_db": [_vp, _vp, _sz, _vp],
     "epa_selftest_log10": [_vp, _vp, _sz, _vp],
diff --git a/echopype_amd/csrc/block_reduce.hip b/echopype_amd/csrc/block_reduce.hip
--- a/echopype_amd/csrc/block_reduce.hip
+++ b/echopype_amd/csrc/block_reduce.hip
@@ -478,7 +478,7 @@
                         void* mvbs_out, void* sum_out, uint32_t* cnt_out, int dtype,
                         size_t lds_bytes, unsigned cnt_off, unsigned long long* rmax_key,
                         unsigned long long* rstat, const double* dscale, const double* doffset, void* depth_out,
-                        hipStream_t st);
+                        void* coltab_ws, hipStream_t st);
 
 int epa_mvbs_rows_fast_path(const void* sv, const double* coef, int C, int P, int S, const int32_t* bin_start,
                             int n_tbins, double range_bin, int n_rbins, int as_stored, double fill_value,
@@ -563,7 +563,7 @@
 }
 
 template <typename T, int SRC>
-int run_mvbs(ReduceArgs& a, hipStream_t st) {
+int run_mvbs(ReduceArgs& a, hipStream_t st, void* coltab_ws = nullptr) {
   Plan pl = make_plan<T>(a.C, a.P, a.S, a.n_tbins, a.n_rbins,
                                al16(a.raw) && al16(a.sv) && al16(a.range) && al16(a.sv_out) &&
                                    al16(a.range_out));
@@ -581,7 +581,7 @@
                                a.cnt_out, sizeof(T) == 8 ? EPA_F64 : EPA_F32, pl.tab_off,
                                pl.cnt_off, reinterpret_cast<unsigned long long*>(a.range_max_out),
                                reinterpret_cast<unsigned long long*>(a.range_stats_out), a.dscale, a.doffset,
-                               a.depth_out, st);
+                               a.depth_out, coltab_ws, st);
   if (a.dscale) {
     epa::set_error("epa_sv_mvbs_fused_depth: binning on depth is served by the default configuration only (sorted "
                    "pings, S %% 4 == 0, aligned arrays, range grid within LDS)");
@@ -696,7 +696,7 @@
                        void* sv_out, void* range_out, void* mvbs_out, void* sum_out,
                        uint32_t* cnt_out, double* range_max_out, double* range_stats_out, int dtype,
                        epa_stream_t stream, const double* dscale = nullptr, const double* doffset = nullptr,
-                       void* depth_out = nullptr);
+                       void* depth_out = nullptr, void* coltab_ws = nullptr);
 
 extern "C" int epa_sv_mvbs_fused(const float* raw, const double* coef, int C, int P, int S,
                                  int cal_type, unsigned cal_flags, const int32_t* bin_start,
@@ -736,13 +736,55 @@
                      cnt_out, depth_stats_out + 32, depth_stats_out, dtype, stream, depth_scale, depth_offset, depth_out);
 }
 
+extern "C" int epa_sv_mvbs_fused_tab(const float* raw, const double* coef, int C, int P, int S,
+                                     int cal_type, unsigned cal_flags, const int32_t* bin_start,
+                                     const int32_t* ping_perm, int n_tbins, double range_bin,
+                                     int n_rbins, unsigned bin_flags, double fill_value, void* sv_out,
+                                     void* range_out, void* mvbs_out, void* sum_out, uint32_t* cnt_out,
+                                     double* range_max_out, double* range_stats_out, int dtype,
+                                     void* coltab_ws, epa_stream_t stream) {
+  EPA_CHECK_ARG(raw != nullptr, "epa_sv_mvbs_fused: NULL array argument");
+  EPA_CHECK_ARG(!range_stats_out || range_max_out, "epa_sv_mvbs_fused: range_stats_out needs range_max_out");
+  return fused_entry(raw, nullptr, nullptr, coef, C, P, S, cal_type, cal_flags, bin_start, ping_perm,
+                     n_tbins, range_bin, n_rbins, bin_flags, fill_value, sv_out, range_out, mvbs_out,
+                     sum_out, cnt_out, range_max_out, range_stats_out, dtype, stream, nullptr, nullptr, nullptr,
+                     coltab_ws);
+}
+
+extern "C" int epa_sv_mvbs_fused_i16_tab(const int16_t* raw, const int32_t* n_valid, const double* coef,
+                                         int C, int P, int S, int cal_type, const int32_t* bin_start,
+                                         int n_tbins, double range_bin, int n_rbins, double fill_value,
+                                         void* sv_out, void* mvbs_out, void* sum_out, uint32_t* cnt_out,
+                                         double* range_max_out, int dtype, void* coltab_ws, epa_stream_t stream) {
+  EPA_CHECK_ARG(raw && n_valid, "epa_sv_mvbs_fused_i16: NULL array argument");
+  return fused_entry(nullptr, raw, n_valid, coef, C, P, S, cal_type,
+                     EPA_FLAG_GUARD_POS | EPA_FLAG_MASK_RANGE, bin_start, nullptr, n_tbins, range_bin,
+                     n_rbins, EPA_BIN_SKIPNA, fill_value, sv_out, nullptr, mvbs_out, sum_out, cnt_out,
+                     range_max_out, nullptr, dtype, stream, nullptr, nullptr, nullptr, coltab_ws);
+}
+
+extern "C" int epa_sv_mvbs_fused_depth_tab(const float* raw, const double* coef, const double* depth_scale,
+                                           const double* depth_offset, int C, int P, int S, int cal_type,
+                                           const int32_t* bin_start, int n_tbins, double range_bin, int n_rbins,
+                                           double fill_value, void* sv_out, void* depth_out, void* mvbs_out,
+                                           void* sum_out, uint32_t* cnt_out, double* depth_stats_out, int dtype,
+                                           void* coltab_ws, epa_stream_t stream) {
+  EPA_CHECK_ARG(raw && depth_scale && depth_offset && depth_stats_out, "epa_sv_mvbs_fused_depth: NULL array argument");
+  EPA_CHECK_ARG(!depth_out || sv_out, "epa_sv_mvbs_fused_depth: depth_out needs sv_out");
+  return fused_entry(raw, nullptr, nullptr, coef, C, P, S, cal_type, EPA_FLAG_GUARD_POS | EPA_FLAG_MASK_RANGE, bin_start,
+                     nullptr, n_tbins, range_bin, n_rbins, EPA_BIN_SKIPNA, fill_value, sv_out, nullptr, mvbs_out, sum_out,
+                     cnt_out, depth_stats_out + 32, depth_stats_out, dtype, stream, depth_scale, depth_offset, depth_out,
+                     coltab_ws);
+}
+
 static int fused_entry(const float* raw, const int16_t* raw_i16, const int32_t* n_valid,
                        const double* coef, int C, int P, int S, int cal_type, unsigned cal_flags,
                        const int32_t* bin_start, const int32_t* ping_perm, int n_tbins,
                        double range_bin, int n_rbins, unsigned bin_flags, double fill_value,
                        void* sv_out, void* range_out, void* mvbs_out, void* sum_out,
                        uint32_t* cnt_out, double* range_max_out, double* range_stats_out, int dtype,
-                       epa_stream_t stream, const double* dscale, const double* doffset, void* depth_out) {
+                       epa_stream_t stream, const double* dscale, const double* doffset, void* depth_out,
+                       void* coltab_ws) {
   EPA_CHECK_ARG(coef && mvbs_out, "epa_sv_mvbs_fused: NULL array argument");
   EPA_CHECK_ARG(C > 0 && P > 0 && S > 0, "epa_sv_mvbs_fused: C=%d P=%d S=%d", C, P, S);
   EPA_CHECK_ARG(cal_type == EPA_CAL_SV || cal_type == EPA_CAL_TS, "epa_sv_mvbs_fused: bad cal_type");
@@ -763,8 +805,8 @@
   a.range_stats_out = range_stats_out;
   EPA_CHECK_ARG(dtype == EPA_F64 || dtype == EPA_F32, "epa_sv_mvbs_fused: bad dtype %d", dtype);
   if (int rc0 = init_range_outputs(range_max_out, range_stats_out, (hipStream_t)stream)) return rc0;
-  const int rc = dtype == EPA_F64 ? run_mvbs<double, SRC_RAW>(a, (hipStream_t)stream)
-                                  : run_mvbs<float, SRC_RAW>(a, (hipStream_t)stream);
+  const int rc = dtype == EPA_F64 ? run_mvbs<double, SRC_RAW>(a, (hipStream_t)stream, coltab_ws)
+                                  : run_mvbs<float, SRC_RAW>(a, (hipStream_t)stream, coltab_ws);
   epa::note_range_stats_filled(rc == EPA_OK && range_stats_out && a.range_stats_filled ? 1 : 0);
   if (rc == EPA_OK && range_max_out) {
     return decode_range_outputs(range_max_out, range_stats_out, a.range_stats_filled != 0, dtype == EPA_F32 ? 1 : 0,
diff --git a/echopype_amd/csrc/fast_math.h b/echopype_amd/csrc/fast_math.h
--- a/echopype_amd/csrc/fast_math.h
+++ b/echopype_amd/csrc/fast_math.h
@@ -27,6 +27,13 @@
     l[t] = make_double2(inv, lg);
   }
   return MathTabs{e, l};
+}
+
+__device__ __forceinline__ const double* build_exp2_tab(unsigned char* base) {
+  double* e = reinterpret_cast<double*>(base);
+  const int t = threadIdx.x;
+  if (t < kExpTabN) e[t] = ::exp2((double)t * (1.0 / kExpTabN));
+  return e;
 }
 
 __device__ __forceinline__ double lin_from_db(double u, const double* __restrict__ tab) {
diff --git a/echopype_amd/csrc/fused_sv_mvbs.hip b/echopype_amd/csrc/fused_sv_mvbs.hip
--- a/echopype_amd/csrc/fused_sv_mvbs.hip
+++ b/echopype_amd/csrc/fused_sv_mvbs.hip
@@ -263,12 +263,12 @@
     const epa::CoefRow* __restrict__ coef,
     const int32_t* __restrict__ bin_start, T* __restrict__ sv_out, T* __restrict__ mvbs_out,
     T* __restrict__ sum_out, uint32_t* __restrict__ cnt_out, const double* __restrict__ dscale,
-    const double* __restrict__ doffset, Args a) {
+    const double* __restrict__ doffset, const T* __restrict__ coltab, Args a) {
+  typedef T T2 __attribute__((ext_vector_type(2)));
   extern __shared__ __attribute__((aligned(16))) unsigned char smem[];
   T* lsum = reinterpret_cast<T*>(smem);
   uint32_t* lcnt = reinterpret_cast<uint32_t*>(smem + a.cnt_off);
-  const epa::MathTabs mt = epa::build_math_tabs(smem + a.tab_off);
-  const double* tab = mt.exp2_tab;
+  const double* tab = epa::build_exp2_tab(smem + a.tab_off);
   constexpr bool NL_LDS = RMAX || sizeof(T) == 8;
   __shared__ T col_nL[NL_LDS ? kChunk : 1];
   constexpr bool SRA_LDS = (RMAX || std::is_same<RawT, int16_t>::value) && sizeof(T) == 8;
@@ -323,6 +323,22 @@
     long long dcur = 0x7ff8dead00000001ll, racur = 0x7ff8dead00000002ll;
     uint32_t n_clean = 0u;
     bool plain = false;
+    if (coltab) {
+      const T* __restrict__ tc = coltab + (size_t)c * S;
+      const T2 nan2 = {epa::M<T>::nan(), epa::M<T>::nan()};
+      const T2 tA = *reinterpret_cast<const T2*>(tc + sA);
+      const T2 tB = hasB ? *reinterpret_cast<const T2*>(tc + sB) : nan2;
+      const T nl[VEC] = {tA.x, tA.y, tB.x, tB.y};
+      bool fin = true;
+#pragma unroll
+      for (int j = 0; j < VEC; ++j) {
+        if (NL_LDS) col_nL[eA + (j < 2 ? 0 : 128) + (j & 1)] = nl[j];
+        else col[j].nL = nl[j];
+        fin = fin & ((j >= 2 && !hasB) | (fabs(nl[j]) < (T)__builtin_inf()));
+      }
+      plain = __ballot(!fin) == 0ull;
+      dcur = __double_as_longlong(rowp0[0].d);
+    }
     const int s4 = chunk0 + wave * 256 + 4 * lane;
     PingLoad<RawT> nxt;
     epa::CoefRow nxtR = rowp0[pb < pe ? pb : 0];
@@ -351,19 +367,26 @@
         nxt.issue(raw_c + row_off + S, sA, sB, hasB, s4, S);
       }
       if (!((__double_as_longlong(r.d) == dcur) & (__double_as_longlong(r.ra) == racur))) {
-        dcur = __double_as_longlong(r.d);
-        racur = __double_as_longlong(r.ra);
-        bool fin = true;
-        for (int j = 0; j < VEC; ++j) {
-          const double sj = (double)((j < 2 ? sA : sB) + (j & 1));
-          const T nl = nspread * log10_slow<T>((T)(sj - r.d));
-          if (NL_LDS) col_nL[eA + (j < 2 ? 0 : 128) + (j & 1)] = nl;
-          else col[j].nL = nl;
-          if (SRA_LDS) col_sra[eA + (j < 2 ? 0 : 128) + (j & 1)] = sj * r.ra;
-          else col[j].sra = sj * r.ra;
-          fin = fin & ((j >= 2 && !hasB) | (fabs(nl) < (T)__builtin_inf()));
+        if (__double_as_longlong(r.d) != dcur) {
+          dcur = __double_as_longlong(r.d);
+          bool fin = true;
+          for (int j = 0; j < VEC; ++j) {
+            const double sj = (double)((j < 2 ? sA : sB) + (j & 1));
+            const T nl = nspread * log10_slow<T>((T)(sj - r.d));
+            if (NL_LDS) col_nL[eA + (j < 2 ? 0 : 128) + (j & 1)] = nl;
+            else col[j].nL = nl;
+            fin = fin & ((j >= 2 && !hasB) | (fabs(nl) < (T)__builtin_inf()));
+          }
+          plain = __ballot(!fin) == 0ull;
         }
-        plain = __ballot(!fin) == 0ull;
+        if (__double_as_longlong(r.ra) != racur) {
+          racur = __double_as_longlong(r.ra);
+          for (int j = 0; j < VEC; ++j) {
+            const double sj = (double)((j < 2 ? sA : sB) + (j & 1));
+            if (SRA_LDS) col_sra[eA + (j < 2 ? 0 : 128) + (j & 1)] = sj * r.ra;
+            else col[j].sra = sj * r.ra;
+          }
+        }
       }
       const T g = (T)r.g, a2 = (T)r.alpha2;
       T A0 = (T)r.A0;
@@ -448,14 +471,35 @@
   }
 }
 
+template <typename T>
+__global__ __launch_bounds__(epa::kBlock) void coltab_kernel(const epa::CoefRow* __restrict__ coef, int P, int S,
+                                                             T nspread, T* __restrict__ tab) {
+  const int c = blockIdx.y, s = blockIdx.x * epa::kBlock + threadIdx.x;
+  if (s >= S) return;
+  const double d = coef[(size_t)c * P].d;
+  tab[(size_t)c * S + s] = nspread * log10_slow<T>((T)((double)s - d));
+}
+
+inline bool coltab_enabled() {
+  const char* e = getenv("EPA_FUSED_COLTAB");
+  return !(e && e[0] == '0');
+}
+
 template <typename T, typename RawT>
 int launch(Args& a, const RawT* raw, const int32_t* n_valid, const double* coef, const int32_t* bin_start,
            void* sv_out, void* mvbs_out, void* sum_out, uint32_t* cnt_out, int C, size_t lds_bytes,
-           hipStream_t st) {
+           void* coltab_ws, hipStream_t st) {
   const dim3 grid((unsigned)a.n_tbins + 1u, (unsigned)C);
   a.tab_off = (unsigned)((lds_bytes + 15) & ~(size_t)15);
   lds_bytes = a.tab_off + epa::kMathTabBytes;
   a.xcd_map = epa::xcd_map_enabled() ? 1 : 0;
+  const T* coltab = coltab_enabled() ? reinterpret_cast<const T*>(coltab_ws) : nullptr;
+  if (coltab) {
+    hipLaunchKernelGGL(coltab_kernel<T>, dim3((unsigned)((a.S + epa::kBlock - 1) / epa::kBlock), (unsigned)C),
+                       dim3(epa::kBlock), 0, st, reinterpret_cast<const epa::CoefRow*>(coef), a.P, a.S, (T)a.nspread,
+                       reinterpret_cast<T*>(coltab_ws));
+    if (int rc = epa::check_launch("coltab_kernel")) return rc;
+  }
 #define EPA_FL(W, R) EPA_FLD(W, R, 0)
 #define EPA_FLD(W, R, D)                                                                       \
   do {                                                                                         \
@@ -466,7 +510,7 @@
                                         (int)lds_bytes));                                      \
     hipLaunchKernelGGL(kern, grid, dim3(epa::kBlock), lds_bytes, st, raw, n_valid,             \
                        reinterpret_cast<const epa::CoefRow*>(coef), bin_start, (T*)sv_out,     \
-                       (T*)mvbs_out, (T*)sum_out, cnt_out, a.dscale, a.doffset, a);            \
+                       (T*)mvbs_out, (T*)sum_out, cnt_out, a.dscale, a.doffset, coltab, a);    \
   } while (0)
   if (a.dscale) {
     if constexpr (std::is_same<RawT, float>::value) {
@@ -587,8 +631,7 @@
   extern __shared__ __attribute__((aligned(16))) unsigned char smem[];
   T* lsum = reinterpret_cast<T*>(smem);
   uint32_t* lcnt = reinterpret_cast<uint32_t*>(smem + a.cnt_off);
-  const epa::MathTabs mt = epa::build_math_tabs(smem + a.tab_off);
-  const double* tab = mt.exp2_tab;
+  const double* tab = epa::build_exp2_tab(smem + a.tab_off);
   __shared__ int differs;
   __shared__ unsigned long long rb_lo_key, rb_hi_key;
   const int c = blockIdx.y, tb = a.xcd_map ? epa::xcd_contiguous(blockIdx.x, a.n_tbins) : (int)blockIdx.x;
@@ -726,8 +769,7 @@
   extern __shared__ __attribute__((aligned(16))) unsigned char smem[];
   T* lsum = reinterpret_cast<T*>(smem);
   uint32_t* lcnt = reinterpret_cast<uint32_t*>(smem + a.cnt_off);
-  const epa::MathTabs mt = epa::build_math_tabs(smem + a.tab_off);
-  const double* tab = mt.exp2_tab;
+  const double* tab = epa::build_exp2_tab(smem + a.tab_off);
   const int c = blockIdx.y, tb = a.xcd_map ? epa::xcd_contiguous(blockIdx.x, a.n_tbins) : (int)blockIdx.x;
   const int S = a.S, n_rbins = a.n_rbins;
   if (a.flagged_only && !left_to_rows(mvbs_out + ((size_t)c * a.n_tbins + tb) * n_rbins)) return;
@@ -878,7 +920,7 @@
                         void* mvbs_out, void* sum_out, uint32_t* cnt_out, int dtype,
                         size_t lds_bytes, unsigned cnt_off, unsigned long long* rmax_key,
                         unsigned long long* rstat, const double* dscale, const double* doffset, void* depth_out,
-                        hipStream_t st) {
+                        void* coltab_ws, hipStream_t st) {
   epa_fused::Args a{};
   a.dscale = dscale; a.doffset = doffset; a.depth_out = dscale ? depth_out : nullptr;
   a.rmax_key = rmax_key;
@@ -893,7 +935,7 @@
   a.cnt_off = cnt_off;
 #define EPA_GO(T, RawT)                                                                           \
   return epa_fused::launch<T, RawT>(a, reinterpret_cast<const RawT*>(raw), n_valid, coef, bin_start, \
-                                    sv_out, mvbs_out, sum_out, cnt_out, C, lds_bytes, st)
+                                    sv_out, mvbs_out, sum_out, cnt_out, C, lds_bytes, coltab_ws, st)
   if (raw_is_i16) {
     if (dtype == EPA_F64) EPA_GO(double, int16_t);
     EPA_GO(float, int16_t);
diff --git a/echopype_amd/ops.py b/echopype_amd/ops.py
--- a/echopype_amd/ops.py
+++ b/echopype_amd/ops.py
@@ -337,6 +337,10 @@
     return C * n_tbins < 1024 or lds > 128 * 1024
 
 
+def _coltab_ws(C, S, dtype, dev):
+    return torch.empty(C * S, dtype=dtype, device=dev)
+
+
 def sv_mvbs_fused(raw, coef, bin_start, n_tbins, range_bin, n_rbins, *, cal_type="Sv",
                   cal_flags=_lib.FLAG_GUARD_POS | _lib.FLAG_MASK_RANGE, skipna=True, closed="left",
                   fill_value=float("nan"), dtype=torch.float64, want_sv=True, want_range=False,
@@ -356,11 +360,11 @@
         cnt = torch.empty((C, n_tbins, n_rbins), dtype=torch.int32, device=dev)
     rmax = torch.empty(1, dtype=torch.float64, device=dev) if want_range_max or want_range_stats else None
     rstats = torch.empty(3, dtype=torch.float64, device=dev) if want_range_stats else None
-    call("epa_sv_mvbs_fused", _p(raw), _p(coef), C, P, S,
+    call("epa_sv_mvbs_fused_tab", _p(raw), _p(coef), C, P, S,
          _lib.CAL_SV if cal_type == "Sv" else _lib.CAL_TS, cal_flags, _p(bin_start), _p(ping_perm),
          int(n_tbins), float(range_bin), int(n_rbins), _bin_flags(skipna, closed), float(fill_value),
          _p(sv_out) if want_sv else None, _p(range_out) if want_range else None, _p(mvbs_out),
-         _p(ssum), _p(cnt), _p(rmax), _p(rstats), _DT[dtype], _stream())
+         _p(ssum), _p(cnt), _p(rmax), _p(rstats), _DT[dtype], _p(_coltab_ws(C, S, dtype, dev)), _stream())
     return dict(Sv=sv_out if want_sv else None, echo_range=range_out if want_range else None,
                 MVBS=mvbs_out, sum=ssum, cnt=cnt, range_max=rmax, range_stats=rstats,
                 range_stats_filled=bool(_lib.lib.epa_last_range_stats_filled()) if want_range_stats else False)
@@ -381,10 +385,10 @@
         ssum = torch.empty((C, n_tbins, n_rbins), dtype=dtype, device=dev)
         cnt = torch.empty((C, n_tbins, n_rbins), dtype=torch.int32, device=dev)
     rstats = torch.empty(64, dtype=torch.float64, device=dev)
-    call("epa_sv_mvbs_fused_depth", _p(raw), _p(coef), _p(depth_scale), _p(depth_offset), C, P, S,
+    call("epa_sv_mvbs_fused_depth_tab", _p(raw), _p(coef), _p(depth_scale), _p(depth_offset), C, P, S,
          _lib.CAL_SV if cal_type == "Sv" else _lib.CAL_TS, _p(bin_start), int(n_tbins), float(range_bin), int(n_rbins),
          float(fill_value), _p(sv_out) if want_sv else None, _p(depth_out), _p(mvbs_out), _p(ssum), _p(cnt), _p(rstats),
-         _DT[dtype], _stream())
+         _DT[dtype], _p(_coltab_ws(C, S, dtype, dev)), _stream())
     return dict(Sv=sv_out if want_sv else None, depth=depth_out, MVBS=mvbs_out, sum=ssum, cnt=cnt,
                 range_stats=rstats[:3], range_stats_filled=True)
 
@@ -405,10 +409,10 @@
         ssum = torch.empty((C, n_tbins, n_rbins), dtype=dtype, device=dev)
         cnt = torch.empty((C, n_tbins, n_rbins), dtype=torch.int32, device=dev)
     rmax = torch.empty(1, dtype=torch.float64, device=dev) if want_range_max else None
-    call("epa_sv_mvbs_fused_i16", _p(raw_i16), _p(n_valid), _p(coef), C, P, S,
+    call("epa_sv_mvbs_fused_i16_tab", _p(raw_i16), _p(n_valid), _p(coef), C, P, S,
          _lib.CAL_SV if cal_type == "Sv" else _lib.CAL_TS, _p(bin_start), int(n_tbins), float(range_bin),
          int(n_rbins), float(fill_value), _p(sv_out) if want_sv else None, _p(mvbs_out), _p(ssum), _p(cnt),
-         _p(rmax), _DT[dtype], _stream())
+         _p(rmax), _DT[dtype], _p(_coltab_ws(C, S, dtype, dev)), _stream())
     return dict(Sv=sv_out if want_sv else None, MVBS=mvbs_out, sum=ssum, cnt=cnt, range_max=rmax)
 
 
diff --git a/include/echopype_amd.h b/include/echopype_amd.h
--- a/include/echopype_amd.h
+++ b/include/echopype_amd.h
@@ -90,6 +90,24 @@
                             void* depth_out, void* mvbs_out, void* sum_out, uint32_t* cnt_out, double* depth_stats_out,
                             int dtype, epa_stream_t stream);
 
+int epa_sv_mvbs_fused_tab(const float* raw, const double* coef, int C, int P, int S, int cal_type,
+                          unsigned cal_flags, const int32_t* bin_start, const int32_t* ping_perm,
+                          int n_tbins, double range_bin, int n_rbins, unsigned bin_flags,
+                          double fill_value, void* sv_out, void* range_out, void* mvbs_out,
+                          void* sum_out, uint32_t* cnt_out, double* range_max_out, double* range_stats_out,
+                          int dtype, void* coltab_ws, epa_stream_t stream);
+int epa_sv_mvbs_fused_i16_tab(const int16_t* raw, const int32_t* n_valid, const double* coef, int C, int P,
+                              int S, int cal_type, const int32_t* bin_start, int n_tbins, double range_bin,
+                              int n_rbins, double fill_value, void* sv_out, void* mvbs_out, void* sum_out,
+                              uint32_t* cnt_out, double* range_max_out, int dtype, void* coltab_ws,
+                              epa_stream_t stream);
+int epa_sv_mvbs_fused_depth_tab(const float* raw, const double* coef, const double* depth_scale,
+                                const double* depth_offset, int C, int P, int S, int cal_type,
+                                const int32_t* bin_start, int n_tbins, double range_bin, int n_rbins,
+                                double fill_value, void* sv_out, void* depth_out, void* mvbs_out, void* sum_out,
+                                uint32_t* cnt_out, double* depth_stats_out, int dtype, void* coltab_ws,
+                                epa_stream_t stream);
+
 int epa_mvbs(const void* sv, const void* range, const double* coef, int C, int P, int S,
              const int32_t* bin_start, const int32_t* ping_perm, int n_tbins, double range_bin,
              int n_rbins, unsigned bin_flags, double fill_value, void* mvbs_out, void* sum_out,
```

New measurement: 487.4 billion range-samples/s. -1.3%, worse.
